# AIS-Bonn/lattice_net

Hardware: AMD Instinct MI355X
Metric: Mpoints/sec splat+conv+slice fwd+bwd on 120k-pt SemanticKITTI scan (higher is better)
Workload: dtype f32 (convolution products bf16x3-emulated)

## Files before the change

include/latticenet_hip.h:

```cpp
#ifndef LATTICENET_HIP_H
#define LATTICENET_HIP_H

#include <stddef.h>

#ifdef __cplusplus
extern "C" {
#endif

#define LN_OK 0
#define LN_ERR_ARG (-1)
#define LN_ERR_UNSUPPORTED (-2)
#define LN_ERR_LAUNCH (-3)
#define LN_ERR_WORKSPACE (-4)

#define LN_STATUS_TABLE_FULL 1
#define LN_STATUS_KEY_RANGE 2
#define LN_STATUS_BUCKET_OVERFLOW 4
#define LN_STATUS_CLOUD_BAND 8
#define LN_STATUS_CLOUD_STARTS 16

#define LN_MAX_POS_DIM 6
#define LN_SLOT_MAP_INTS 32
#define LN_KEYS_RAW 0
#define LN_KEYS_LATTICE 1
#define LN_NOT_VISITED (-2)

typedef struct LnTable {
    int capacity;
    int pos_dim;
    unsigned long long* slot_keys;
    unsigned int* slot_tok;
    int* slot_cnt;
    int* entries;
    int* keys;
    int* nr_filled;
    int* status;
    int* host_counters;
    int host_seq;
    int key_format;
    int row_limit;
    const int* slot_map;
    int bucket_slots_max;
    int batch_points;
    int batch_key_step;
    int* row_regions;
} LnTable;

#define LN_BATCH_POINT_STARTS (-1)
typedef struct LnTableClouds {
    LnTable table;
    const int* batch_point_starts;
    int batch_clouds;
} LnTableClouds;

#define LN_XCD_GROUPS 8
typedef struct LnCsr {
    int* grp_start;
    int* csr_tok;
    int* seg_desc;
    int* seg_count;
    long long seg_region;
    const int* planes;
    int dense;
} LnCsr;

const char* ln_last_error_string(void);
const char* ln_version(void);
const char* ln_abi_hash(void);

const char* ln_kernel_names(void);
int ln_profile_begin(const char* kernel_names, int max_samples);
int ln_profile_end(double* total_ms, int* launches);
int ln_profile_end_table(char* out, int out_bytes);

int ln_table_clear(const LnTable* t, float* values, long long values_elems, void* stream);

int ln_arena_init(int* arena, long long words, long long minus_begin, long long minus_end, void* stream);

int ln_table_bucket_count(int capacity);

size_t ln_build_workspace_bytes(long long tokens, int capacity);

#define LN_BUILD_WRITE_IDX 1
#define LN_BUILD_CLEAR_FIRST 2
#define LN_BUILD_ATOMIC_PATH 4
#define LN_BUILD_CANONICAL_ROWS 8
#define LN_BUILD_SORTED_CSR 16
#define LN_BUILD_OVERLAPPED 32
int ln_build_splat(const LnTable* t, const float* positions_raw, const float* sigmas_host, int n, int* idx, float* w,
                   int flags, const LnCsr* csr, void* workspace, size_t workspace_bytes, float* clear_values,
                   long long clear_values_elems, void* stream);

int ln_canonicalize(const LnTable* t, int* idx, long long tokens, const LnCsr* csr, void* workspace, size_t workspace_bytes, void* stream);

int ln_rehash(const LnTable* t, void* stream);

int ln_splat_accumulate(float* table_values, const float* vals, const int* idx, const float* w, int n, int pos_dim,
                        int val_dim, void* stream);

long long ln_csr_max_segments(long long tokens, int groups_upper);
size_t ln_csr_workspace_bytes(long long tokens, int groups_upper);
int ln_csr_build(const int* idx, long long tokens, int groups_upper, const LnCsr* csr, void* workspace, size_t workspace_bytes,
                 void* stream);
int ln_csr_reduce_rows(const LnCsr* csr, const int* grp_row, long long max_segments, const float* src, const float* w, int val_dim,
                       int src_div, int src_stride, float* dst, void* stream);
int ln_csr_sort(const LnCsr* csr, int groups_upper, void* workspace, size_t workspace_bytes, long long tokens, void* stream);

int ln_splat_accumulate_and_neighbours(const LnCsr* csr, const int* grp_row, long long max_segments, const float* src, const float* w,
                                       int val_dim, int src_div, int src_stride, float* dst, const LnTable* table, int query_rows_upper,
                                       int* nbr, void* stream);

int ln_csr_segment_max(const LnCsr* csr, const int* grp_row, long long max_segments, const float* src, int channels, int rows,
                       void* packed_ws, float* out_max, int* out_arg, void* stream);
int ln_csr_group_sizes(const LnCsr* csr, const int* grp_row, int groups_upper, int rows, int* counts, void* stream);

int ln_distribute(const LnTable* t, const float* positions_raw, const float* sigmas_host, const float* vals, int n,
                  int val_dim, int* idx, float* w, float* distributed, int flags, const LnCsr* csr, void* workspace,
                  size_t workspace_bytes, float* clear_values, long long clear_values_elems, void* stream);

int ln_coarsen(const LnTable* fine, int fine_rows_upper, const LnTable* coarse, const LnCsr* csr, void* workspace,
               size_t workspace_bytes, void* stream);

int ln_neighbours(const LnTable* query, int query_rows_upper, const LnTable* neigh, int lvl_query, int lvl_neigh,
                  int dilation, int flip, int* nbr, void* stream);

int ln_im2row(const int* nbr, const float* values_neigh, int m, int filter_extent, int val_dim, float* out, void* stream);
int ln_im2rowindices(const int* nbr, int m, int filter_extent, int val_dim, int* out, void* stream);
int ln_row2im(const int* nbr, const float* rowified, int m, int filter_extent, int val_dim, float* out, void* stream);

#define LN_CONV_FLIP_NEIGHBOURS 1
#define LN_CONV_TRANSPOSED_FILTER 2
#define LN_CONV_BANK_READY 4
#define LN_CONV_OVERLAPPED 8
int ln_conv_forward(const int* nbr, const float* values_neigh, const float* filter, int m, int filter_extent, int val_dim,
                    int nr_filters, int flags, float* out, void* stream);
size_t ln_conv_bank_workspace_bytes(int m, int filter_extent, int val_dim, int nr_filters);
size_t ln_conv_forward_workspace_bytes(int m, int filter_extent, int val_dim, int nr_filters);
int ln_conv_forward_ws(const int* nbr, const float* values_neigh, const float* filter, int m, int filter_extent, int val_dim,
                       int nr_filters, int flags, float* out, void* workspace, size_t workspace_bytes, const int* row_partition, void* stream);
size_t ln_conv_grad_filter_workspace_bytes(int m, int filter_extent, int val_dim, int nr_filters);
int ln_conv_grad_filter(const int* nbr, const float* values_neigh, const float* grad_out, int m, int filter_extent,
                        int val_dim, int nr_filters, float* grad_filter, void* workspace, size_t workspace_bytes,
                        void* stream);

int ln_slice_forward(const float* values, const int* idx, const float* w, int n, int pos_dim, int val_dim, float* out,
                     void* stream);
int ln_slice_forward_prepare_backward(const float* values, const int* idx, const float* w, int n, int pos_dim, int val_dim, float* out,
                                      float* grad_accumulator, long long grad_accumulator_elems, void* stream);
int ln_slice_forward_ordered(const LnTable* t, const LnCsr* csr, const float* values, const int* idx, const float* w, int n, int val_dim,
                             float* out, float* grad_accumulator, long long grad_accumulator_elems, void* stream);

int ln_slice_no_precomputation(const LnTable* t, const float* values, const float* positions_raw, const float* sigmas_host,
                               int n, int val_dim, float* out, int* idx, float* w, void* stream);
int ln_slice_backward(const float* grad_sliced, const int* idx, const float* w, int n, int pos_dim, int val_dim,
                      float* grad_values, void* stream);

int ln_gather_forward(const float* values, const int* idx, const float* w, int n, int pos_dim, int val_dim, float* out,
                      void* stream);
int ln_gather_backward(const float* grad_gathered, const int* idx, const float* w, int n, int pos_dim, int val_dim,
                       float* grad_values, void* stream);

int ln_slice_classify_forward(const float* values, const float* delta_w, const float* lin_w, const float* lin_b,
                              const int* idx, const float* w, int n, int pos_dim, int val_dim, int nr_classes,
                              float* logits, void* stream);
size_t ln_slice_classify_backward_workspace_bytes(int n, int pos_dim, int val_dim, int nr_classes);
int ln_slice_classify_backward(const float* grad_logits, const float* values, const float* delta_w, const float* lin_w,
                               const int* idx, const float* w, int n, int pos_dim, int val_dim, int nr_classes,
                               float* g_values, float* g_delta_w, float* g_lin_w, float* g_lin_b, float* grad_sliced,
                               float* w_eff, void* workspace, size_t workspace_bytes, void* stream);

size_t ln_conv_backward_workspace_bytes(int mq, int mn, int filter_extent, int val_dim, int nr_filters);
int ln_conv_backward(const int* nbr_q, const int* nbr_n, const float* values_neigh, const float* grad_out, const float* filter, int mq, int mn,
                     int filter_extent, int val_dim, int nr_filters, float* grad_values, float* grad_filter, void* workspace,
                     size_t workspace_bytes, const int* row_partition, void* stream);
int ln_conv_backward_flags(const int* nbr_q, const int* nbr_n, const float* values_neigh, const float* grad_out, const float* filter, int mq,
                           int mn, int filter_extent, int val_dim, int nr_filters, int flags, float* grad_values, float* grad_filter,
                           void* workspace, size_t workspace_bytes, const int* row_partition, void* stream);

int ln_csr_reduce_rows_f16(const LnCsr* csr, const int* grp_row, long long max_segments, const void* src_f16, const float* w, int val_dim,
                           int src_div, int src_stride, float* dst, void* stream);
int ln_splat_accumulate_and_neighbours_f16(const LnCsr* csr, const int* grp_row, long long max_segments, const void* src_f16, const float* w,
                                           int val_dim, int src_div, int src_stride, float* dst, const LnTable* table, int query_rows_upper,
                                           int* nbr, void* stream);
int ln_slice_forward_f16(const void* values_f16, const int* idx, const float* w, int n, int pos_dim, int val_dim, void* out_f16, void* stream);
int ln_slice_forward_f16_prepare_backward(const void* values_f16, const int* idx, const float* w, int n, int pos_dim, int val_dim, void* out_f16,
                                          float* grad_accumulator, long long grad_accumulator_elems, void* stream);

int ln_conv_forward_f16(const int* nbr, const void* values_neigh, const void* filter, int m, int filter_extent, int val_dim,
                        int nr_filters, int flags, void* out, void* stream);
size_t ln_conv_grad_filter_f16_workspace_bytes(int m, int filter_extent, int val_dim, int nr_filters);
int ln_conv_grad_filter_f16(const int* nbr, const void* values_neigh, const void* grad_out, int m, int filter_extent, int val_dim,
                            int nr_filters, float* grad_filter, void* workspace, size_t workspace_bytes, void* stream);

int ln_linear_act_forward(const float* x, const float* w, const float* b, long long rows, int cin, int cout, float slope, float* y,
                          void* stream);
size_t ln_linear_act_backward_workspace_bytes(int cin, int cout);
int ln_linear_act_backward(const float* x, const float* w, const float* y, const float* grad_y, long long rows, int cin, int cout,
                           float slope, float* grad_x, float* grad_w, float* grad_b, void* workspace, size_t workspace_bytes, void* stream);

size_t ln_group_norm_workspace_bytes(int channels);
int ln_group_norm_forward(const float* x, const float* gamma, const float* beta, int m, int channels, int groups, float eps, int relu,
                          float* y, float* mean_rstd, float* scale_shift, void* workspace, size_t workspace_bytes, void* next_workspace,
                          size_t next_workspace_bytes, void* stream);
int ln_group_norm_backward(const float* x, const float* grad_y, const float* gamma, const float* mean_rstd, const float* scale_shift, int m,
                           int channels, int groups, int relu, float* grad_x, float* grad_gamma, float* grad_beta, void* workspace,
                           size_t workspace_bytes, void* next_workspace, size_t next_workspace_bytes, void* stream);
int ln_group_norm_forward_rows(const float* x, const float* gamma, const float* beta, int m, int channels, int groups, float eps, int relu,
                               float* y, float* mean_rstd, float* scale_shift, void* workspace, size_t workspace_bytes, void* next_workspace,
                               size_t next_workspace_bytes, const int* rows_device, void* stream);
int ln_group_norm_backward_rows(const float* x, const float* grad_y, const float* gamma, const float* mean_rstd, const float* scale_shift, int m,
                                int channels, int groups, int relu, float* grad_x, float* grad_gamma, float* grad_beta, void* workspace,
                                size_t workspace_bytes, void* next_workspace, size_t next_workspace_bytes, const int* rows_device, void* stream);

int ln_cloud_row_starts(const LnTable* t, int rows_upper, int clouds, int* row_starts, int* order_flag, void* stream);
int ln_cloud_row_starts_many(const LnTable* t, int rows_upper, int clouds, int* row_starts, int* order_flag, void* stream);
size_t ln_group_norm_segments_workspace_bytes(int channels, int segments);
int ln_group_norm_forward_segments(const float* x, const float* gamma, const float* beta, int m, int channels, int groups, float eps, int relu,
                                   float* y, float* mean_rstd, float* scale_shift, void* workspace, size_t workspace_bytes, void* next_workspace,
                                   size_t next_workspace_bytes, const int* rows_device, const int* row_starts, int segments, void* stream);
int ln_group_norm_backward_segments(const float* x, const float* grad_y, const float* gamma, const float* mean_rstd, const float* scale_shift,
                                    int m, int channels, int groups, int relu, float* grad_x, float* grad_gamma, float* grad_beta, void* workspace,
                                    size_t workspace_bytes, void* next_workspace, size_t next_workspace_bytes, const int* rows_device,
                                    const int* row_starts, int segments, void* stream);
int ln_group_norm_forward_many_segments(const float* x, const float* gamma, const float* beta, int m, int channels, int groups, float eps,
                                        int relu, float* y, float* mean_rstd, float* scale_shift, void* workspace, size_t workspace_bytes,
                                        void* next_workspace, size_t next_workspace_bytes, const int* rows_device, const int* row_starts,
                                        int segments, void* stream);
int ln_group_norm_backward_many_segments(const float* x, const float* grad_y, const float* gamma, const float* mean_rstd,
                                         const float* scale_shift, int m, int channels, int groups, int relu, float* grad_x, float* grad_gamma,
                                         float* grad_beta, void* workspace, size_t workspace_bytes, void* next_workspace,
                                         size_t next_workspace_bytes, const int* rows_device, const int* row_starts, int segments, void* stream);

int ln_group_norm_forward_segments_f16(const void* x, const float* gamma, const float* beta, int m, int channels, int groups, float eps, int relu,
                                       void* y, float* mean_rstd, float* scale_shift, void* workspace, size_t workspace_bytes,
                                       void* next_workspace, size_t next_workspace_bytes, const int* rows_device, const int* row_starts,
                                       int segments, void* stream);
int ln_group_norm_backward_segments_f16(const void* x, const void* grad_y, const float* gamma, const float* mean_rstd, const float* scale_shift,
                                        int m, int channels, int groups, int relu, void* grad_x, float* grad_gamma, float* grad_beta,
                                        void* workspace, size_t workspace_bytes, void* next_workspace, size_t next_workspace_bytes,
                                        const int* rows_device, const int* row_starts, int segments, void* stream);

size_t ln_batch_norm_workspace_bytes(int channels);
int ln_batch_norm_forward(const float* x, const float* gamma, const float* beta, float* running_mean, float* running_var, int m, int channels,
                          float eps, double momentum, int training, int relu, float* y, float* mean_rstd, float* scale_shift, void* workspace,
                          size_t workspace_bytes, void* next_workspace, size_t next_workspace_bytes, const int* rows_device, void* stream);
int ln_batch_norm_backward(const float* x, const float* grad_y, const float* gamma, const float* mean_rstd, const float* scale_shift, int m,
                           int channels, int training, int relu, float* grad_x, float* grad_gamma, float* grad_beta, void* workspace,
                           size_t workspace_bytes, void* next_workspace, size_t next_workspace_bytes, const int* rows_device, void* stream);

int ln_max_centre_forward(const float* x, const float* gamma, const float* beta, long long n, int k, int c, float* out,
                          float* max_vals, unsigned char* arg_max, void* stream);
size_t ln_max_centre_backward_workspace_bytes(long long n, int k, int c);
int ln_max_centre_backward(const float* grad_out, const float* max_vals, const unsigned char* arg_max, const float* gamma,
                           long long n, int k, int c, float* grad_x, float* grad_gamma_beta, void* workspace,
                           size_t workspace_bytes, void* stream);

size_t ln_linear_backward_workspace_bytes(int rows, int cin, int cout);
int ln_linear_backward(const int* ident, const float* x, const float* grad_y, const float* w, int rows, int cin, int cout, float* grad_x,
                       float* grad_w, void* workspace, size_t workspace_bytes, void* stream);

int ln_weight_norm_forward(const float* v, const float* g, int rows, int cols, int g_dim, float* w, float* norm, void* stream);
int ln_weight_norm_backward(const float* v, const float* g, const float* grad_w, const float* norm, int rows, int cols, int g_dim,
                            float* grad_v, float* grad_g, void* stream);

int ln_distribute_centre(const float* distributed, const int* splat_idx, const float* position_sums, const int* counts, long long tokens,
                         int width, int pos_dim, float* out, void* stream);
int ln_distribute_centre_clouds(const float* distributed, const int* splat_idx, const float* position_sums, const int* counts,
                                long long tokens, int width, int pos_dim, long long tokens_per_cloud, const int* row_starts, int clouds,
                                float* out, void* stream);
int ln_distribute_centre_cloud_starts(const float* distributed, const int* splat_idx, const float* position_sums, const int* counts,
                                      long long tokens, int width, int pos_dim, int tokens_per_point, const int* point_starts,
                                      const int* row_starts, int clouds, float* out, void* stream);
int ln_distribute_centre_many_clouds(const float* distributed, const int* splat_idx, const float* position_sums, const int* counts,
                                     long long tokens, int width, int pos_dim, long long tokens_per_cloud, const int* row_starts, int clouds,
                                     float* out, void* stream);
int ln_distribute_centre_many_cloud_starts(const float* distributed, const int* splat_idx, const float* position_sums, const int* counts,
                                           long long tokens, int width, int pos_dim, int tokens_per_point, const int* point_starts,
                                           const int* row_starts, int clouds, float* out, void* stream);

size_t ln_pointnet_reduce_workspace_bytes(int rows, int channels);
int ln_pointnet_reduce_forward(const LnCsr* csr, const int* grp_row, long long max_segments, const float* src, int channels,
                               const float* bary, int bary_stride, int rows, int min_points, void* workspace, size_t workspace_bytes,
                               float* out, int* out_arg, void* stream);
int ln_pointnet_reduce_forward_clouds(const LnCsr* csr, const int* grp_row, long long max_segments, const float* src, int channels,
                                      const float* bary, int bary_stride, int rows, int min_points, void* workspace, size_t workspace_bytes,
                                      float* out, int* out_arg, const int* row_starts, int clouds, void* stream);
int ln_pointnet_reduce_forward_many_clouds(const LnCsr* csr, const int* grp_row, long long max_segments, const float* src, int channels,
                                           const float* bary, int bary_stride, int rows, int min_points, void* workspace,
                                           size_t workspace_bytes, float* out, int* out_arg, const int* row_starts, int clouds, void* stream);
int ln_pointnet_reduce_backward(const float* grad_out, int grad_stride, const int* out_arg, const int* splat_idx, long long tokens,
                                int channels, float* grad_src, void* stream);

size_t ln_nll_workspace_bytes(void);
int ln_nll_forward(const float* log_probs, const long long* target, long long n, int classes, long long ignore_index, void* workspace,
                   size_t workspace_bytes, float* loss_count, void* stream);
int ln_nll_backward(const long long* target, const float* grad_loss, const float* loss_count, long long n, int classes,
                    long long ignore_index, float* grad_log_probs, void* stream);

size_t ln_lovasz_workspace_bytes(long long n, int classes);
int ln_lovasz_forward(const float* log_probs, const long long* target, long long n, int classes, long long ignore_index, int reduction,
                      void* workspace, size_t workspace_bytes, float* loss, float* per_class, float* dloss_dlogp, void* stream);
int ln_lovasz_backward(const float* dloss_dlogp, const float* grad_loss, long long n, int classes, float* grad_log_probs, void* stream);

size_t ln_lovasz_clouds_workspace_bytes(long long n, long long points_per_cloud, int classes);
int ln_lovasz_forward_clouds(const float* log_probs, const long long* target, long long n, long long points_per_cloud, int classes,
                             long long ignore_index, int reduction, void* workspace, size_t workspace_bytes, float* loss, float* per_cloud,
                             float* per_class, float* dloss_dlogp, void* stream);

size_t ln_iou_counts_clouds_workspace_bytes(long long n, long long points_per_cloud, int classes);
int ln_iou_counts_clouds(const float* scores, const long long* target, long long n, long long points_per_cloud, int classes,
                         long long unlabeled_index, void* workspace, size_t workspace_bytes, long long* intersection, long long* union_,
                         void* stream);

size_t ln_dice_workspace_bytes(long long n, long long points_per_cloud, int classes);
int ln_dice_forward(const float* log_probs, const long long* target, long long n, long long points_per_cloud, int classes,
                    long long ignore_index, void* workspace, size_t workspace_bytes, float* loss, float* per_cloud, float* stats, float* coef,
                    void* stream);
int ln_dice_backward(const float* log_probs, const long long* target, const float* coef, const float* grad_loss, long long n,
                     long long points_per_cloud, int classes, float* grad_log_probs, void* stream);

size_t ln_nll_clouds_workspace_bytes(long long n, long long points_per_cloud);
int ln_nll_forward_clouds(const float* log_probs, const long long* target, long long n, long long points_per_cloud, int classes,
                          long long ignore_index, const float* class_weight, void* workspace, size_t workspace_bytes, float* loss,
                          float* per_cloud, float* weight_sum, void* stream);
int ln_nll_backward_clouds(const long long* target, const float* grad_loss, const float* weight_sum, long long n, long long points_per_cloud,
                           int classes, long long ignore_index, const float* class_weight, float* grad_log_probs, void* stream);

size_t ln_nll_ranges_workspace_bytes(long long n, int clouds, long long longest);
int ln_nll_forward_ranges(const float* log_probs, const long long* target, long long n, const int* point_starts, int clouds, long long longest,
                          int classes, long long ignore_index, const float* class_weight, void* workspace, size_t workspace_bytes, float* loss,
// ... 24 lines not shown
```

lattice_net_amd/_lib.py:

```python
from __future__ import annotations

import ctypes as C
import os

import torch

_PKG = os.path.dirname(os.path.abspath(__file__))
LIB_PATH = os.environ.get("LATTICE_NET_LIB") or os.path.join(_PKG, "liblatticenet_hip.so")

LN_STATUS_TABLE_FULL = 1
LN_STATUS_KEY_RANGE = 2
LN_STATUS_BUCKET_OVERFLOW = 4
LN_STATUS_CLOUD_BAND = 8
LN_STATUS_CLOUD_STARTS = 16
LN_BUILD_WRITE_IDX = 1
LN_BUILD_CLEAR_FIRST = 2
LN_BUILD_ATOMIC_PATH = 4
LN_BUILD_CANONICAL_ROWS = 8
LN_BUILD_SORTED_CSR = 16
LN_BUILD_OVERLAPPED = 32
LN_NOT_VISITED = -2
LN_CONV_FLIP_NEIGHBOURS = 1
LN_CONV_TRANSPOSED_FILTER = 2
LN_CONV_BANK_READY = 4
LN_CONV_OVERLAPPED = 8
LN_MAX_POS_DIM = 6
LN_KEYS_RAW = 0
LN_KEYS_LATTICE = 1
LN_XCD_GROUPS = 8
LN_SLOT_MAP_INTS = 32


class LnTable(C.Structure):

    _fields_ = [
        ("capacity", C.c_int),
        ("pos_dim", C.c_int),
        ("slot_keys", C.c_void_p),
        ("slot_tok", C.c_void_p),
        ("slot_cnt", C.c_void_p),
        ("entries", C.c_void_p),
        ("keys", C.c_void_p),
        ("nr_filled", C.c_void_p),
        ("status", C.c_void_p),
        ("host_counters", C.c_void_p),
        ("host_seq", C.c_int),
        ("key_format", C.c_int),
        ("row_limit", C.c_int),
        ("slot_map", C.c_void_p),
        ("bucket_slots_max", C.c_int),
        ("batch_points", C.c_int),
        ("batch_key_step", C.c_int),
        ("row_regions", C.c_void_p),
    ]


LN_BATCH_POINT_STARTS = -1


class LnTableClouds(C.Structure):

    _fields_ = [
        ("table", LnTable),
        ("batch_point_starts", C.c_void_p),
        ("batch_clouds", C.c_int),
    ]

    def __init__(self, table_fields=(), batch_point_starts=None, batch_clouds=0):
        super().__init__(LnTable(*table_fields), batch_point_starts, batch_clouds)
        self.table.batch_points = LN_BATCH_POINT_STARTS


class LnCsr(C.Structure):

    _fields_ = [
        ("grp_start", C.c_void_p),
        ("csr_tok", C.c_void_p),
        ("seg_desc", C.c_void_p),
        ("seg_count", C.c_void_p),
        ("seg_region", C.c_longlong),
        ("planes", C.c_void_p),
        ("dense", C.c_int),
    ]


class LatticeNetHipError(RuntimeError):
    pass


_vp, _i, _ll, _sz = C.c_void_p, C.c_int, C.c_longlong, C.c_size_t
_T = C.POINTER(LnTable)
_CSR = C.POINTER(LnCsr)

SIGNATURES = {
    "ln_last_error_string": (C.c_char_p, []),
    "ln_version": (C.c_char_p, []),
    "ln_abi_hash": (C.c_char_p, []),
    "ln_kernel_names": (C.c_char_p, []),
    "ln_profile_begin": (_i, [C.c_char_p, _i]),
    "ln_profile_end": (_i, [C.POINTER(C.c_double), C.POINTER(_i)]),
    "ln_profile_end_table": (_i, [C.c_char_p, _i]),
    "ln_table_clear": (_i, [_T, _vp, _ll, _vp]),
    "ln_build_workspace_bytes": (_sz, [_ll, _i]),
    "ln_table_bucket_count": (_i, [_i]),
    "ln_build_splat": (_i, [_T, _vp, _vp, _i, _vp, _vp, _i, _CSR, _vp, _sz, _vp, _ll, _vp]),
    "ln_rehash": (_i, [_T, _vp]),
    "ln_canonicalize": (_i, [_T, _vp, _ll, _CSR, _vp, _sz, _vp]),
    "ln_splat_accumulate": (_i, [_vp, _vp, _vp, _vp, _i, _i, _i, _vp]),
    "ln_csr_workspace_bytes": (_sz, [_ll, _i]),
    "ln_csr_max_segments": (_ll, [_ll, _i]),
    "ln_csr_build": (_i, [_vp, _ll, _i, _CSR, _vp, _sz, _vp]),
    "ln_csr_reduce_rows": (_i, [_CSR, _vp, _ll, _vp, _vp, _i, _i, _i, _vp, _vp]),
    "ln_csr_sort": (_i, [_CSR, _i, _vp, _sz, _ll, _vp]),
    "ln_splat_accumulate_and_neighbours": (_i, [_CSR, _vp, _ll, _vp, _vp, _i, _i, _i, _vp, _T, _i, _vp, _vp]),
    "ln_csr_segment_max": (_i, [_CSR, _vp, _ll, _vp, _i, _i, _vp, _vp, _vp, _vp]),
    "ln_csr_group_sizes": (_i, [_CSR, _vp, _i, _i, _vp, _vp]),
    "ln_distribute": (_i, [_T, _vp, _vp, _vp, _i, _i, _vp, _vp, _vp, _i, _CSR, _vp, _sz, _vp, _ll, _vp]),
    "ln_coarsen": (_i, [_T, _i, _T, _CSR, _vp, _sz, _vp]),
    "ln_neighbours": (_i, [_T, _i, _T, _i, _i, _i, _i, _vp, _vp]),
    "ln_im2row": (_i, [_vp, _vp, _i, _i, _i, _vp, _vp]),
    "ln_im2rowindices": (_i, [_vp, _i, _i, _i, _vp, _vp]),
    "ln_row2im": (_i, [_vp, _vp, _i, _i, _i, _vp, _vp]),
    "ln_conv_forward": (_i, [_vp, _vp, _vp, _i, _i, _i, _i, _i, _vp, _vp]),
    "ln_conv_forward_workspace_bytes": (_sz, [_i, _i, _i, _i]),
    "ln_conv_bank_workspace_bytes": (_sz, [_i, _i, _i, _i]),
    "ln_conv_forward_ws": (_i, [_vp, _vp, _vp, _i, _i, _i, _i, _i, _vp, _vp, _sz, _vp, _vp]),
    "ln_conv_grad_filter_workspace_bytes": (_sz, [_i, _i, _i, _i]),
    "ln_conv_grad_filter": (_i, [_vp, _vp, _vp, _i, _i, _i, _i, _vp, _vp, _sz, _vp]),
    "ln_slice_forward": (_i, [_vp, _vp, _vp, _i, _i, _i, _vp, _vp]),
    "ln_slice_forward_prepare_backward": (_i, [_vp, _vp, _vp, _i, _i, _i, _vp, _vp, _ll, _vp]),
    "ln_slice_forward_ordered": (_i, [_T, _CSR, _vp, _vp, _vp, _i, _i, _vp, _vp, _ll, _vp]),
    "ln_slice_no_precomputation": (_i, [_T, _vp, _vp, _vp, _i, _i, _vp, _vp, _vp, _vp]),
    "ln_slice_backward": (_i, [_vp, _vp, _vp, _i, _i, _i, _vp, _vp]),
    "ln_gather_forward": (_i, [_vp, _vp, _vp, _i, _i, _i, _vp, _vp]),
    "ln_gather_backward": (_i, [_vp, _vp, _vp, _i, _i, _i, _vp, _vp]),
    "ln_slice_classify_forward": (_i, [_vp, _vp, _vp, _vp, _vp, _vp, _i, _i, _i, _i, _vp, _vp]),
    "ln_csr_reduce_rows_f16": (_i, [_CSR, _vp, _ll, _vp, _vp, _i, _i, _i, _vp, _vp]),
    "ln_splat_accumulate_and_neighbours_f16": (_i, [_CSR, _vp, _ll, _vp, _vp, _i, _i, _i, _vp, _T, _i, _vp, _vp]),
    "ln_slice_forward_f16": (_i, [_vp, _vp, _vp, _i, _i, _i, _vp, _vp]),
    "ln_slice_forward_f16_prepare_backward": (_i, [_vp, _vp, _vp, _i, _i, _i, _vp, _vp, _ll, _vp]),
    "ln_conv_backward_workspace_bytes": (_sz, [_i, _i, _i, _i, _i]),
    "ln_conv_backward": (_i, [_vp, _vp, _vp, _vp, _vp, _i, _i, _i, _i, _i, _vp, _vp, _vp, _sz, _vp, _vp]),
    "ln_conv_backward_flags": (_i, [_vp, _vp, _vp, _vp, _vp, _i, _i, _i, _i, _i, _i, _vp, _vp, _vp, _sz, _vp, _vp]),
    "ln_conv_forward_f16": (_i, [_vp, _vp, _vp, _i, _i, _i, _i, _i, _vp, _vp]),
    "ln_conv_grad_filter_f16_workspace_bytes": (_sz, [_i, _i, _i, _i]),
    "ln_conv_grad_filter_f16": (_i, [_vp, _vp, _vp, _i, _i, _i, _i, _vp, _vp, _sz, _vp]),
    "ln_linear_act_forward": (_i, [_vp, _vp, _vp, _ll, _i, _i, C.c_float, _vp, _vp]),
    "ln_linear_act_backward_workspace_bytes": (_sz, [_i, _i]),
    "ln_linear_act_backward": (_i, [_vp, _vp, _vp, _vp, _ll, _i, _i, C.c_float, _vp, _vp, _vp, _vp, _sz, _vp]),
    "ln_arena_init": (_i, [_vp, _ll, _ll, _ll, _vp]),
    "ln_weight_norm_forward": (_i, [_vp, _vp, _i, _i, _i, _vp, _vp, _vp]),
    "ln_weight_norm_backward": (_i, [_vp, _vp, _vp, _vp, _i, _i, _i, _vp, _vp, _vp]),
    "ln_distribute_centre": (_i, [_vp, _vp, _vp, _vp, _ll, _i, _i, _vp, _vp]),
    "ln_distribute_centre_clouds": (_i, [_vp, _vp, _vp, _vp, _ll, _i, _i, _ll, _vp, _i, _vp, _vp]),
    "ln_distribute_centre_many_clouds": (_i, [_vp, _vp, _vp, _vp, _ll, _i, _i, _ll, _vp, _i, _vp, _vp]),
    "ln_distribute_centre_cloud_starts": (_i, [_vp, _vp, _vp, _vp, _ll, _i, _i, _i, _vp, _vp, _i, _vp, _vp]),
    "ln_distribute_centre_many_cloud_starts": (_i, [_vp, _vp, _vp, _vp, _ll, _i, _i, _i, _vp, _vp, _i, _vp, _vp]),
    "ln_pointnet_reduce_workspace_bytes": (_sz, [_i, _i]),
    "ln_pointnet_reduce_forward": (_i, [_CSR, _vp, _ll, _vp, _i, _vp, _i, _i, _i, _vp, _sz, _vp, _vp, _vp]),
    "ln_pointnet_reduce_forward_clouds": (_i, [_CSR, _vp, _ll, _vp, _i, _vp, _i, _i, _i, _vp, _sz, _vp, _vp, _vp, _i, _vp]),
    "ln_pointnet_reduce_forward_many_clouds": (_i, [_CSR, _vp, _ll, _vp, _i, _vp, _i, _i, _i, _vp, _sz, _vp, _vp, _vp, _i, _vp]),
    "ln_pointnet_reduce_backward": (_i, [_vp, _i, _vp, _vp, _ll, _i, _vp, _vp]),
    "ln_linear_backward_workspace_bytes": (_sz, [_i, _i, _i]),
    "ln_linear_backward": (_i, [_vp, _vp, _vp, _vp, _i, _i, _i, _vp, _vp, _vp, _sz, _vp]),
    "ln_nll_workspace_bytes": (_sz, []),
    "ln_nll_forward": (_i, [_vp, _vp, _ll, _i, _ll, _vp, _sz, _vp, _vp]),
    "ln_nll_backward": (_i, [_vp, _vp, _vp, _ll, _i, _ll, _vp, _vp]),
    "ln_nll_clouds_workspace_bytes": (_sz, [_ll, _ll]),
    "ln_nll_forward_clouds": (_i, [_vp, _vp, _ll, _ll, _i, _ll, _vp, _vp, _sz, _vp, _vp, _vp, _vp]),
    "ln_nll_backward_clouds": (_i, [_vp, _vp, _vp, _ll, _ll, _i, _ll, _vp, _vp, _vp]),
    "ln_lovasz_workspace_bytes": (_sz, [_ll, _i]),
    "ln_lovasz_forward": (_i, [_vp, _vp, _ll, _i, _ll, _i, _vp, _sz, _vp, _vp, _vp, _vp]),
    "ln_lovasz_backward": (_i, [_vp, _vp, _ll, _i, _vp, _vp]),
    "ln_lovasz_clouds_workspace_bytes": (_sz, [_ll, _ll, _i]),
    "ln_lovasz_forward_clouds": (_i, [_vp, _vp, _ll, _ll, _i, _ll, _i, _vp, _sz, _vp, _vp, _vp, _vp, _vp]),
    "ln_iou_counts_clouds_workspace_bytes": (_sz, [_ll, _ll, _i]),
    "ln_iou_counts_clouds": (_i, [_vp, _vp, _ll, _ll, _i, _ll, _vp, _sz, _vp, _vp, _vp]),
    "ln_dice_workspace_bytes": (_sz, [_ll, _ll, _i]),
    "ln_dice_forward": (_i, [_vp, _vp, _ll, _ll, _i, _ll, _vp, _sz, _vp, _vp, _vp, _vp, _vp]),
    "ln_dice_backward": (_i, [_vp, _vp, _vp, _vp, _ll, _ll, _i, _vp, _vp]),
    "ln_nll_ranges_workspace_bytes": (_sz, [_ll, _i, _ll]),
    "ln_nll_forward_ranges": (_i, [_vp, _vp, _ll, _vp, _i, _ll, _i, _ll, _vp, _vp, _sz, _vp, _vp, _vp, _vp]),
    "ln_nll_backward_ranges": (_i, [_vp, _vp, _vp, _ll, _vp, _i, _ll, _i, _ll, _vp, _vp, _vp]),
    "ln_dice_ranges_workspace_bytes": (_sz, [_ll, _i, _ll, _i]),
    "ln_dice_forward_ranges": (_i, [_vp, _vp, _ll, _vp, _i, _ll, _i, _ll, _vp, _sz, _vp, _vp, _vp, _vp, _vp]),
    "ln_dice_backward_ranges": (_i, [_vp, _vp, _vp, _vp, _ll, _vp, _i, _ll, _i, _vp, _vp]),
    "ln_lovasz_ranges_workspace_bytes": (_sz, [_ll, _i, _ll, _i]),
    "ln_lovasz_forward_ranges": (_i, [_vp, _vp, _ll, _vp, _i, _ll, _i, _ll, _i, _vp, _sz, _vp, _vp, _vp, _vp, _vp]),
    "ln_max_centre_forward": (_i, [_vp, _vp, _vp, _ll, _i, _i, _vp, _vp, _vp, _vp]),
    "ln_max_centre_backward_workspace_bytes": (_sz, [_ll, _i, _i]),
    "ln_max_centre_backward": (_i, [_vp, _vp, _vp, _vp, _ll, _i, _i, _vp, _vp, _vp, _sz, _vp]),
    "ln_group_norm_workspace_bytes": (_sz, [_i]),
    "ln_group_norm_forward": (_i, [_vp, _vp, _vp, _i, _i, _i, C.c_float, _i, _vp, _vp, _vp, _vp, _sz, _vp, _sz, _vp]),
    "ln_group_norm_backward": (_i, [_vp, _vp, _vp, _vp, _vp, _i, _i, _i, _i, _vp, _vp, _vp, _vp, _sz, _vp, _sz, _vp]),
    "ln_group_norm_forward_rows": (_i, [_vp, _vp, _vp, _i, _i, _i, C.c_float, _i, _vp, _vp, _vp, _vp, _sz, _vp, _sz, _vp, _vp]),
    "ln_group_norm_backward_rows": (_i, [_vp, _vp, _vp, _vp, _vp, _i, _i, _i, _i, _vp, _vp, _vp, _vp, _sz, _vp, _sz, _vp, _vp]),
    "ln_cloud_row_starts": (_i, [_T, _i, _i, _vp, _vp, _vp]),
    "ln_cloud_row_starts_many": (_i, [_T, _i, _i, _vp, _vp, _vp]),
    "ln_group_norm_segments_workspace_bytes": (_sz, [_i, _i]),
    "ln_group_norm_forward_segments": (_i, [_vp, _vp, _vp, _i, _i, _i, C.c_float, _i, _vp, _vp, _vp, _vp, _sz, _vp, _sz, _vp, _vp, _i, _vp]),
    "ln_group_norm_forward_many_segments": (_i, [_vp, _vp, _vp, _i, _i, _i, C.c_float, _i, _vp, _vp, _vp, _vp, _sz, _vp, _sz, _vp, _vp, _i, _vp]),
    "ln_group_norm_backward_segments": (_i, [_vp, _vp, _vp, _vp, _vp, _i, _i, _i, _i, _vp, _vp, _vp, _vp, _sz, _vp, _sz, _vp, _vp, _i, _vp]),
    "ln_group_norm_backward_many_segments": (_i, [_vp, _vp, _vp, _vp, _vp, _i, _i, _i, _i, _vp, _vp, _vp, _vp, _sz, _vp, _sz, _vp, _vp, _i, _vp]),
    "ln_group_norm_forward_segments_f16": (_i, [_vp, _vp, _vp, _i, _i, _i, C.c_float, _i, _vp, _vp, _vp, _vp, _sz, _vp, _sz, _vp, _vp, _i, _vp]),
    "ln_group_norm_backward_segments_f16": (_i, [_vp, _vp, _vp, _vp, _vp, _i, _i, _i, _i, _vp, _vp, _vp, _vp, _sz, _vp, _sz, _vp, _vp, _i, _vp]),
    "ln_batch_norm_workspace_bytes": (_sz, [_i]),
    "ln_batch_norm_forward": (_i, [_vp, _vp, _vp, _vp, _vp, _i, _i, C.c_float, C.c_double, _i, _i, _vp, _vp, _vp, _vp, _sz, _vp, _sz, _vp, _vp]),
    "ln_batch_norm_backward": (_i, [_vp, _vp, _vp, _vp, _vp, _i, _i, _i, _i, _vp, _vp, _vp, _vp, _sz, _vp, _sz, _vp, _vp]),
    "ln_cloud_key_extents": (_i, [_T, _vp, _vp, _i, _i, _vp, _vp, _vp]),
    "ln_cloud_point_starts_check": (_i, [_vp, _i, _i, _vp, _vp]),
    "ln_slice_classify_backward_workspace_bytes": (_sz, [_i, _i, _i, _i]),
    "ln_slice_classify_backward": (_i, [_vp, _vp, _vp, _vp, _vp, _vp, _i, _i, _i, _i, _vp, _vp, _vp, _vp, _vp, _vp, _vp, _sz, _vp]),
}

_lib = None


def load():
    global _lib
    if _lib is not None:
        return _lib
    if not os.path.exists(LIB_PATH):
        raise LatticeNetHipError(
            f"{LIB_PATH} is missing: the HIP extension is not built. Run `python -c 'import __graft_entry__ as g; g.build()'` "
            "(or `python lattice_net_amd/build_ext.py`). There is no CPU fallback."
        )
    lib = C.CDLL(LIB_PATH)
    for name, (res, args) in SIGNATURES.items():
        fn = getattr(lib, name)
        fn.restype = res
        fn.argtypes = args
    from . import build_ext
    try:
        want = build_ext.abi_hash()
    except OSError:
        want = None
    have = lib.ln_abi_hash().decode()
    if want is not None and have != want:
        raise LatticeNetHipError(f"{LIB_PATH} was built from a different include/latticenet_hip.h (library {have}, header {want}): "
                                 "rebuild it with `python lattice_net_amd/build_ext.py`")
    _lib = lib
    return lib


def check(rc: int, what: str = ""):
    if rc != 0:
        msg = load().ln_last_error_string().decode("utf-8", "replace")
        raise LatticeNetHipError(f"{what or 'latticenet_hip'} failed (code {rc}): {msg}")


def ptr(t):
    return None if t is None else t.data_ptr()


def stream_ptr(device) -> int:
    cur = torch.cuda.current_device()
    idx = device.index if device.index is not None else cur
    if idx != cur:
        raise LatticeNetHipError(f"lattice tensors live on cuda:{idx} but the current device is cuda:{cur}; wrap the call in "
                                 f"`with torch.cuda.device({idx}):` (or torch.cuda.set_device) — one process drives one GPU")
    return torch._C._cuda_getCurrentRawStream(idx)


def host_floats(values):
    arr = (C.c_float * len(values))(*[float(v) for v in values])
    return arr
```

lattice_net_amd/csrc/ln_conv.hip:

```cpp
#include "ln_common.h"
#include <stdlib.h>

#include "ln_bf16x3.h"

#include "ln_conv_plan.h"
#include <type_traits>

#ifdef LN_STAMPS
__device__ unsigned long long* g_ln_stamps_conv = nullptr;
extern "C" int ln_debug_set_stamps_conv(void* buffer) {
    unsigned long long* p = static_cast<unsigned long long*>(buffer);
    return hipMemcpyToSymbol(HIP_SYMBOL(g_ln_stamps_conv), &p, sizeof(p)) == hipSuccess ? 0 : -1;
}
#define LN_CSTAMP(slot)                                                                                                  \
    do {                                                                                                                 \
        if (g_ln_stamps_conv && threadIdx.x == 0) g_ln_stamps_conv[(size_t)blockIdx.x * 8 + (slot)] = wall_clock64(); \
    } while (0)
#else
#define LN_CSTAMP(slot) do { } while (0)
#endif

template <int KQ>
__device__ __forceinline__ void ln_load_quarter(const float* __restrict__ src, float* a) {
    if constexpr (KQ % 4 == 0) {
// ... 811 lines not shown
                }
            }
        }
    }
}

template <int V, int NT, int E, bool FLIP, bool WT>
__global__ void __launch_bounds__(256)
    k_conv_mfma_full(const int* __restrict__ nbr, const float* __restrict__ values, const float* __restrict__ filter, int m,
                     float* __restrict__ out, int conv_blocks, const float* __restrict__ slab_partial, int nslabs, int slab_total,
                     float* __restrict__ slab_out) {
    if (slab_out != nullptr && (int)blockIdx.x >= conv_blocks) {
        ln_sum_slabs_body<false>(blockIdx.x - conv_blocks, slab_partial, nslabs, slab_total, slab_total, slab_out);
        return;
    }
    constexpr int F = 16 * NT;
    constexpr int KQ = V / 4;
    static_assert(E * V * F * 4 <= 64 * 1024, "filter bank must fit 64 KiB of LDS");
    __shared__ __attribute__((aligned(16))) float s_b[E * V * F];
    const int tid = threadIdx.x;
    const int lane = tid & 63;
    const int wave = tid >> 6;
    const int i = lane & 15;
    const int q = lane >> 4;
    const int m0 = blockIdx.x * 64 + wave * 16;
    const int my_row = m0 + i;

    LN_CSTAMP(0);
    constexpr int N4 = E * V * F / 4;
    constexpr int NST = (N4 + 255) / 256;
    float4 wv[NST];
#pragma unroll
    for (int s = 0; s < NST; ++s) {
        const int x4 = tid + s * 256;
        wv[s] = (x4 < N4) ? reinterpret_cast<const float4*>(filter)[x4] : make_float4(0.f, 0.f, 0.f, 0.f);
    }
    int nb[E];
#pragma unroll
    for (int e = 0; e < E; ++e) nb[e] = (my_row < m) ? nbr[(size_t)my_row * E + ((FLIP && e < E - 1) ? (e ^ 1) : e)] : -1;
    float a[E][KQ];
#pragma unroll
    for (int e = 0; e < E; ++e) ln_load_quarter<KQ>(values + (size_t)(nb[e] >= 0 ? nb[e] : 0) * V + q * KQ, a[e]);
#pragma unroll
    for (int s = 0; s < NST; ++s) {
        const int x4 = tid + s * 256;
        if (x4 < N4) {
            const int x = x4 * 4;
            if constexpr (!WT) {
                const int ek = x / F;
                const int f = x - ek * F;
                const int e = ek / V;
                const int k = ek - e * V;
                const int qq = k / KQ;
                const int kk = k - qq * KQ;
                float* dst = s_b + (((e * KQ + kk) * NT + (f >> 4)) * 64 + qq * 16 + (f & 15));
                *reinterpret_cast<float4*>(dst) = wv[s];
            } else {
                const int ef = x / V;
                const int k0 = x - ef * V;
                const int e = ef / F;
                const int f = ef - e * F;
                const float vals4[4] = {wv[s].x, wv[s].y, wv[s].z, wv[s].w};
#pragma unroll
                for (int j = 0; j < 4; ++j) {
                    const int k = k0 + j;
                    const int qq = k / KQ;
                    const int kk = k - qq * KQ;
                    s_b[((e * KQ + kk) * NT + (f >> 4)) * 64 + qq * 16 + (f & 15)] = vals4[j];
                }
            }
        }
    }
    __syncthreads();
    LN_CSTAMP(1);
    floatx4 acc[NT];
#pragma unroll
    for (int nt = 0; nt < NT; ++nt) acc[nt] = floatx4{0.f, 0.f, 0.f, 0.f};
#pragma unroll
    for (int e = 0; e < E; ++e) {
#pragma unroll
        for (int kk = 0; kk < KQ; ++kk) {
            const float av = nb[e] >= 0 ? a[e][kk] : 0.f;
#pragma unroll
            for (int nt = 0; nt < NT; ++nt) {
                const float b = s_b[((e * KQ + kk) * NT + nt) * 64 + lane];
                acc[nt] = __builtin_amdgcn_mfma_f32_16x16x4f32(av, b, acc[nt], 0, 0, 0);
            }
        }
    }
    LN_CSTAMP(2);
#pragma unroll
    for (int nt = 0; nt < NT; ++nt) {
#pragma unroll
        for (int r = 0; r < 4; ++r) {
            const int row = m0 + q * 4 + r;
            if (row < m) out[(size_t)row * F + nt * 16 + i] = acc[nt][r];
        }
    }
    LN_CSTAMP(3);
}

__global__ void __launch_bounds__(256)
    k_conv_generic(const int* __restrict__ nbr, const float* __restrict__ values, const float* __restrict__ filter, long long work,
                   int E, int V, int F, int flip, int wt, float* __restrict__ out) {
    const long long g = (long long)blockIdx.x * blockDim.x + threadIdx.x;
    if (g >= work) return;
    const long long mrow = g / F;
    const int f = int(g - mrow * F);
    float acc = 0.0f;
    for (int e = 0; e < E; ++e) {
        const int nb = nbr[mrow * E + ((flip && e < E - 1) ? (e ^ 1) : e)];
        if (nb < 0) continue;
        const float* vr = values + (size_t)nb * V;
        if (wt) {
            const float* wr = filter + ((size_t)e * F + f) * V;
            for (int v = 0; v < V; ++v) acc = fmaf(vr[v], wr[v], acc);
        } else {
            const float* wr = filter + (size_t)e * V * F + f;
            for (int v = 0; v < V; ++v) acc = fmaf(vr[v], wr[(size_t)v * F], acc);
        }
    }
    out[g] = acc;
}

__global__ void __launch_bounds__(256) ln_k_sum_partials(const float* __restrict__ partial, int nslabs, long long total4, float* __restrict__ out) {
    const long long i = (long long)blockIdx.x * 256 + threadIdx.x;
    if (i >= total4) return;
    float4 acc = reinterpret_cast<const float4*>(partial)[i];
    for (int sl = 1; sl < nslabs; ++sl) {
        const float4 v = reinterpret_cast<const float4*>(partial)[(long long)sl * total4 + i];
        acc.x += v.x; acc.y += v.y; acc.z += v.z; acc.w += v.w;
    }
    reinterpret_cast<float4*>(out)[i] = acc;
}

static bool ln_conv_b3_enabled() {
    static int v = -1;
    if (v < 0) {
        const char* e = getenv("LN_CONV_EXACT_F32");
        v = (e && e[0] == '1') ? 0 : 1;
    }
    return v == 1;
}
static bool ln_aligned16(const void* p) { return (reinterpret_cast<uintptr_t>(p) & 15) == 0; }

extern "C" size_t ln_conv_bank_workspace_bytes(int m, int filter_extent, int val_dim, int nr_filters) {
    return ln_conv_bank_query(m, filter_extent, val_dim, nr_filters, ln_conv_b3_enabled());
}

extern "C" size_t ln_conv_forward_workspace_bytes(int m, int filter_extent, int val_dim, int nr_filters) {
    return ln_conv_forward_query(m, filter_extent, val_dim, nr_filters, ln_conv_b3_enabled());
}

template <int T>
__global__ void __launch_bounds__(256 * T) __attribute__((amdgpu_waves_per_eu(T, T)))
    k_conv_forward_b3(const int* __restrict__ nbr, const float* __restrict__ values, const float* __restrict__ filter, int m,
                      float* __restrict__ out, const int* __restrict__ row_part) {
    constexpr int V = 32, F = 32, E = 9, KQ = 8, NT = 2;
    constexpr int THREADS = 256 * T;
    constexpr int FRAG16 = E * NT * 3 * 64;
    __shared__ __attribute__((aligned(16))) unsigned char s_raw[FRAG16 * 16];
    const u32x4* s_frag = reinterpret_cast<const u32x4*>(s_raw);
    __shared__ __attribute__((aligned(16))) floatx4 s_x[4 * T][16 * 8];
    __shared__ int s_nbr[64 * T * E];
    const int tid = threadIdx.x;
    const int lane = tid & 63;
    const int i = lane & 15;
    const int q = lane >> 4;
    const int bx = ln_partition_tile(blockIdx.x, gridDim.x, row_part, 64 * T);
    const int m0 = bx * (64 * T) + (tid >> 6) * 16;
    const int my_row = m0 + i;
    constexpr int ITEMS = E * (V / 8) * F;
    constexpr int NIT = (ITEMS + THREADS - 1) / THREADS;
    float wv[NIT][8];
#pragma unroll
    for (int s = 0; s < NIT; ++s) {
        const int x = min(tid + s * THREADS, ITEMS - 1);
        const int f = x % F;
        const int ev8 = x / F;
#pragma unroll
        for (int j = 0; j < 8; ++j) wv[s][j] = filter[(ev8 * 8 + j) * F + f];
    }
    {
        const size_t g0 = (size_t)bx * (64 * T) * E, g_end = (size_t)m * E;
        for (int x = tid; x < 64 * T * E; x += THREADS) s_nbr[x] = (g0 + x < g_end) ? nbr[g0 + x] : -1;
    }
    {
        bool any = false;
        for (int x = tid; x < 64 * T * E; x += THREADS) any |= s_nbr[x] >= 0;
        if (!__syncthreads_or(any)) {
            for (int x = tid; x < 64 * T * (F / 4); x += THREADS) {
                const int row = bx * (64 * T) + x / (F / 4);
                if (row < m) *reinterpret_cast<float4*>(out + (size_t)row * F + (x % (F / 4)) * 4) = make_float4(0.f, 0.f, 0.f, 0.f);
            }
            return;
        }
    }
    const int wv_ = tid >> 6;
    const int lr = lane >> 3;
    int nb[2][E];
#pragma unroll
    for (int j = 0; j < 2; ++j)
#pragma unroll
        for (int e = 0; e < E; ++e) nb[j][e] = s_nbr[(wv_ * 16 + 8 * j + lr) * E + e];
    auto fsw = [](int r) -> int { return ((r >> 1) & 7) ^ (((r >> 2) & 1) << 1); };
    floatx4* xw[2];
#pragma unroll
    for (int j = 0; j < 2; ++j) xw[j] = &s_x[wv_][(8 * j + lr) * 8 + ((lane & 7) ^ fsw(8 * j + lr))];
    const floatx4* xr0 = &s_x[wv_][i * 8 + ((2 * q) ^ fsw(i))];
    const floatx4* xr1 = &s_x[wv_][i * 8 + ((2 * q + 1) ^ fsw(i))];
#ifndef LN_FWD_DEPTH
#define LN_FWD_DEPTH 4
#endif
    constexpr int DEPTH = LN_FWD_DEPTH;
    floatx4 a[DEPTH][2];
    auto gather = [&](int e, floatx4 (&dst)[2]) {
#pragma unroll
        for (int j = 0; j < 2; ++j)
            dst[j] = *reinterpret_cast<const floatx4*>(values + (size_t)(nb[j][e] >= 0 ? nb[j][e] : 0) * V + (lane & 7) * 4);
    };
#pragma unroll
    for (int k = 0; k < DEPTH - 1 && k < E; ++k) gather(k, a[k]);
    u32x4* s_frag_w = reinterpret_cast<u32x4*>(s_raw);
#pragma unroll
    for (int s = 0; s < NIT; ++s) {
        const int x = tid + s * THREADS;
        if (x < ITEMS) {
            const int f = x % F;
            const int ev8 = x / F;
            const int e = ev8 / (V / 8);
            const int vo = ev8 - e * (V / 8);
            unsigned int h[8], md[8], lo[8];
#pragma unroll
            for (int j = 0; j < 8; ++j) ln_split3_bits(wv[s][j], h[j], md[j], lo[j]);
            const int unit = ((e * NT + (f >> 4)) * 3) * 64 + vo * 16 + (f & 15);
            s_frag_w[unit] = u32x4{ln_pack_hi(h[0], h[1]), ln_pack_hi(h[2], h[3]), ln_pack_hi(h[4], h[5]), ln_pack_hi(h[6], h[7])};
            s_frag_w[unit + 64] = u32x4{ln_pack_hi(md[0], md[1]), ln_pack_hi(md[2], md[3]), ln_pack_hi(md[4], md[5]), ln_pack_hi(md[6], md[7])};
            s_frag_w[unit + 128] = u32x4{ln_pack_hi(lo[0], lo[1]), ln_pack_hi(lo[2], lo[3]), ln_pack_hi(lo[4], lo[5]), ln_pack_hi(lo[6], lo[7])};
        }
    }
    floatx4 acc[NT];
#pragma unroll
    for (int nt = 0; nt < NT; ++nt) acc[nt] = floatx4{0.f, 0.f, 0.f, 0.f};
    __syncthreads();
#pragma unroll
    for (int e = 0; e < E; ++e) {
        if (e + DEPTH - 1 < E) gather(e + DEPTH - 1, a[(e + DEPTH - 1) % DEPTH]);
#pragma unroll
        for (int j = 0; j < 2; ++j) *xw[j] = (nb[j][e] >= 0) ? a[e % DEPTH][j] : floatx4{0.f, 0.f, 0.f, 0.f};
        __builtin_amdgcn_fence(__ATOMIC_RELEASE, "wavefront");
        __builtin_amdgcn_wave_barrier();
        __builtin_amdgcn_fence(__ATOMIC_ACQUIRE, "wavefront");
        const floatx4 lo4 = *xr0, hi4 = *xr1;
        __builtin_amdgcn_fence(__ATOMIC_RELEASE, "wavefront");
        __builtin_amdgcn_wave_barrier();
        __builtin_amdgcn_fence(__ATOMIC_ACQUIRE, "wavefront");
        const float ae[KQ] = {lo4[0], lo4[1], lo4[2], lo4[3], hi4[0], hi4[1], hi4[2], hi4[3]};
        u32x4 p[3];
        ln_split3_pack8(ae, 0, p);
        const bf16x8 ap[3] = {__builtin_bit_cast(bf16x8, p[0]), __builtin_bit_cast(bf16x8, p[1]), __builtin_bit_cast(bf16x8, p[2])};
#pragma unroll
        for (int nt = 0; nt < NT; ++nt) {
            const u32x4* pb = s_frag + ((e * NT + nt) * 3) * 64 + lane;
            const bf16x8 bp[3] = {__builtin_bit_cast(bf16x8, pb[0]), __builtin_bit_cast(bf16x8, pb[64]), __builtin_bit_cast(bf16x8, pb[128])};
            ln_b3_mfma16(ap, bp, acc[nt]);
        }
    }
#pragma unroll
    for (int nt = 0; nt < NT; ++nt)
#pragma unroll
        for (int r = 0; r < 4; ++r) {
            const int row = m0 + q * 4 + r;
            if (row < m) out[(size_t)row * F + nt * 16 + i] = acc[nt][r];
        }
}

template <int T, int C>
__global__ void __launch_bounds__(256 * T) __attribute__((amdgpu_waves_per_eu(T, T)))
    k_conv_forward_b3_rows(const int* __restrict__ nbr, const float* __restrict__ values, const float* __restrict__ filter, int m,
                      float* __restrict__ out, const int* __restrict__ row_part) {
    constexpr int V = 32, F = 32, E = 9, KQ = 8, NT = 2;
    constexpr int THREADS = 256 * T;
    constexpr int FRAG16 = E * NT * 3 * 64;
    __shared__ __attribute__((aligned(16))) unsigned char s_raw[FRAG16 * 16];
    const u32x4* s_frag = reinterpret_cast<const u32x4*>(s_raw);
    __shared__ __attribute__((aligned(16))) floatx4 s_x[4 * T][16 * 8];
    __shared__ int s_nbr[64 * T * E];
    const int tid = threadIdx.x;
    const int lane = tid & 63;
    const int i = lane & 15;
    const int q = lane >> 4;
    const int bx0 = ln_partition_tile(blockIdx.x, gridDim.x, row_part, 64 * T * C) * C;
    const int m00 = bx0 * (64 * T) + (tid >> 6) * 16;
    constexpr int ITEMS = E * (V / 8) * F;
    constexpr int NIT = (ITEMS + THREADS - 1) / THREADS;
    float wv[NIT][8];
#pragma unroll
    for (int s = 0; s < NIT; ++s) {
        const int x = min(tid + s * THREADS, ITEMS - 1);
        const int f = x % F;
        const int ev8 = x / F;
#pragma unroll
        for (int j = 0; j < 8; ++j) wv[s][j] = filter[(ev8 * 8 + j) * F + f];
    }
    bool staged = false;
#pragma unroll
    for (int c = 0; c < C; ++c) {
    const int bx = bx0 + c;
    const int m0 = m00 + c * (64 * T);
    {
        const size_t g0 = (size_t)bx * (64 * T) * E, g_end = (size_t)m * E;
        for (int x = tid; x < 64 * T * E; x += THREADS) s_nbr[x] = (g0 + x < g_end) ? nbr[g0 + x] : -1;
    }
    {
        bool any = false;
        for (int x = tid; x < 64 * T * E; x += THREADS) any |= s_nbr[x] >= 0;
        if (!__syncthreads_or(any)) {
            for (int x = tid; x < 64 * T * (F / 4); x += THREADS) {
                const int row = bx * (64 * T) + x / (F / 4);
                if (row < m) *reinterpret_cast<float4*>(out + (size_t)row * F + (x % (F / 4)) * 4) = make_float4(0.f, 0.f, 0.f, 0.f);
            }
            if constexpr (C == 1) return;
            else continue;
        }
    }
    const int wv_ = tid >> 6;
    const int lr = lane >> 3;
    int nb[2][E];
#pragma unroll
    for (int j = 0; j < 2; ++j)
#pragma unroll
        for (int e = 0; e < E; ++e) nb[j][e] = s_nbr[(wv_ * 16 + 8 * j + lr) * E + e];
    auto fsw = [](int r) -> int { return ((r >> 1) & 7) ^ (((r >> 2) & 1) << 1); };
    floatx4* xw[2];
#pragma unroll
    for (int j = 0; j < 2; ++j) xw[j] = &s_x[wv_][(8 * j + lr) * 8 + ((lane & 7) ^ fsw(8 * j + lr))];
    const floatx4* xr0 = &s_x[wv_][i * 8 + ((2 * q) ^ fsw(i))];
    const floatx4* xr1 = &s_x[wv_][i * 8 + ((2 * q + 1) ^ fsw(i))];
#ifndef LN_FWD_DEPTH
#define LN_FWD_DEPTH 4
#endif
    constexpr int DEPTH = LN_FWD_DEPTH;
    floatx4 a[DEPTH][2];
    auto gather = [&](int e, floatx4 (&dst)[2]) {
#pragma unroll
        for (int j = 0; j < 2; ++j)
            dst[j] = *reinterpret_cast<const floatx4*>(values + (size_t)(nb[j][e] >= 0 ? nb[j][e] : 0) * V + (lane & 7) * 4);
    };
#pragma unroll
    for (int k = 0; k < DEPTH - 1 && k < E; ++k) gather(k, a[k]);
    u32x4* s_frag_w = reinterpret_cast<u32x4*>(s_raw);
    if (!staged) {
    staged = true;
#pragma unroll
    for (int s = 0; s < NIT; ++s) {
        const int x = tid + s * THREADS;
        if (x < ITEMS) {
            const int f = x % F;
            const int ev8 = x / F;
            const int e = ev8 / (V / 8);
            const int vo = ev8 - e * (V / 8);
            unsigned int h[8], md[8], lo[8];
#pragma unroll
            for (int j = 0; j < 8; ++j) ln_split3_bits(wv[s][j], h[j], md[j], lo[j]);
            const int unit = ((e * NT + (f >> 4)) * 3) * 64 + vo * 16 + (f & 15);
            s_frag_w[unit] = u32x4{ln_pack_hi(h[0], h[1]), ln_pack_hi(h[2], h[3]), ln_pack_hi(h[4], h[5]), ln_pack_hi(h[6], h[7])};
            s_frag_w[unit + 64] = u32x4{ln_pack_hi(md[0], md[1]), ln_pack_hi(md[2], md[3]), ln_pack_hi(md[4], md[5]), ln_pack_hi(md[6], md[7])};
            s_frag_w[unit + 128] = u32x4{ln_pack_hi(lo[0], lo[1]), ln_pack_hi(lo[2], lo[3]), ln_pack_hi(lo[4], lo[5]), ln_pack_hi(lo[6], lo[7])};
        }
    }
    }
    floatx4 acc[NT];
#pragma unroll
    for (int nt = 0; nt < NT; ++nt) acc[nt] = floatx4{0.f, 0.f, 0.f, 0.f};
    __syncthreads();
#pragma unroll
    for (int e = 0; e < E; ++e) {
        if (e + DEPTH - 1 < E) gather(e + DEPTH - 1, a[(e + DEPTH - 1) % DEPTH]);
#pragma unroll
        for (int j = 0; j < 2; ++j) *xw[j] = (nb[j][e] >= 0) ? a[e % DEPTH][j] : floatx4{0.f, 0.f, 0.f, 0.f};
        __builtin_amdgcn_fence(__ATOMIC_RELEASE, "wavefront");
        __builtin_amdgcn_wave_barrier();
        __builtin_amdgcn_fence(__ATOMIC_ACQUIRE, "wavefront");
        const floatx4 lo4 = *xr0, hi4 = *xr1;
        __builtin_amdgcn_fence(__ATOMIC_RELEASE, "wavefront");
        __builtin_amdgcn_wave_barrier();
        __builtin_amdgcn_fence(__ATOMIC_ACQUIRE, "wavefront");
        const float ae[KQ] = {lo4[0], lo4[1], lo4[2], lo4[3], hi4[0], hi4[1], hi4[2], hi4[3]};
        u32x4 p[3];
        ln_split3_pack8(ae, 0, p);
        const bf16x8 ap[3] = {__builtin_bit_cast(bf16x8, p[0]), __builtin_bit_cast(bf16x8, p[1]), __builtin_bit_cast(bf16x8, p[2])};
#pragma unroll
        for (int nt = 0; nt < NT; ++nt) {
            const u32x4* pb = s_frag + ((e * NT + nt) * 3) * 64 + lane;
            const bf16x8 bp[3] = {__builtin_bit_cast(bf16x8, pb[0]), __builtin_bit_cast(bf16x8, pb[64]), __builtin_bit_cast(bf16x8, pb[128])};
            ln_b3_mfma16(ap, bp, acc[nt]);
        }
    }
#pragma unroll
    for (int nt = 0; nt < NT; ++nt)
#pragma unroll
        for (int r = 0; r < 4; ++r) {
            const int row = m0 + q * 4 + r;
            if (row < m) out[(size_t)row * F + nt * 16 + i] = acc[nt][r];
        }
    }
}

template <bool FLIP, bool WT>
struct LnConvCall {
    const int* nbr;
    const float *values, *filter;
    int m, E, V, F;
    float* out;
    unsigned short* bank;
    float* dst;
    int e_per;
    LnSlabSum sum;
    const int* row_partition;
    hipStream_t st;
};

template <bool FLIP, bool WT>
static void ln_conv_launch_full(int V, int NT, dim3 grid, hipStream_t st, const int* nbr, const float* values, const float* filter, int m,
                                float* out, int conv_blocks, const float* partial, int chunks, int total, float* grad_filter) {
    auto go = [&](auto v, auto nt) {
        constexpr int VV = decltype(v)::value, NN = decltype(nt)::value;
        static_assert(ln_conv_full_shape(VV, 16 * NN), "not a small-filter shape");
        LN_LAUNCH("k_conv_mfma", (k_conv_mfma_full<VV, NN, 9, FLIP, WT>), grid, dim3(256), 0, st, nbr, values, filter, m, out, conv_blocks, partial,
                  chunks, total, grad_filter);
    };
    using std::integral_constant;
    switch (V * 16 + NT) {
        case 32 * 16 + 2: go(integral_constant<int, 32>{}, integral_constant<int, 2>{}); break;
        case 32 * 16 + 1: go(integral_constant<int, 32>{}, integral_constant<int, 1>{}); break;
        case 16 * 16 + 1: go(integral_constant<int, 16>{}, integral_constant<int, 1>{}); break;
        case 16 * 16 + 2: go(integral_constant<int, 16>{}, integral_constant<int, 2>{}); break;
        case 16 * 16 + 4: go(integral_constant<int, 16>{}, integral_constant<int, 4>{}); break;
        case 8 * 16 + 1: go(integral_constant<int, 8>{}, integral_constant<int, 1>{}); break;
        case 8 * 16 + 2: go(integral_constant<int, 8>{}, integral_constant<int, 2>{}); break;
        case 8 * 16 + 4: go(integral_constant<int, 8>{}, integral_constant<int, 4>{}); break;
        case 8 * 16 + 8: go(integral_constant<int, 8>{}, integral_constant<int, 8>{}); break;
        default: break;
    }
}

template <bool FLIP, bool WT>
struct LnConvEntry {
    const LnConvLaunch& l;
    const LnConvCall<FLIP, WT>& c;
    dim3 grid() const { return dim3(l.grid[0], l.grid[1], l.grid[2]); }
    unsigned short* bank() const { return c.bank + l.bank_off; }
    const u32x4* frags() const { return reinterpret_cast<const u32x4*>(bank()); }
    LnSlabSum ride() const { return l.carries_sum ? c.sum : LnSlabSum{nullptr, 0, 0, nullptr}; }
};
template <int V, int NT, bool FLIP, bool WT>
static void ln_conv_run_wide(const LnConvEntry<FLIP, WT>& e) {
    const LnConvLaunch& l = e.l;
    const LnConvCall<FLIP, WT>& c = e.c;
    if constexpr (ln_conv_wide_built(V, NT)) {
        if (l.kernel == LN_K_SPLIT_BANK32) {
            LN_LAUNCH("k_conv_split_bank", (k_conv_split_bank32<V, NT, WT>), e.grid(), dim3(l.block), 0, c.st, c.filter, c.F, l.f_off, e.bank(), l.split_x,
                      e.ride());
            return;
        }
        if constexpr (NT == 3) {
            if (l.kernel == LN_K_ROWS32SK) {
                LN_LAUNCH("k_conv_mfma", (k_conv_rows32sk_b3<V, NT, LN_CONV_R32SK_RT, FLIP>), e.grid(), dim3(l.block), 0, c.st, c.nbr, c.values, e.frags(),
                          c.m, c.E, c.dst, c.F, l.f_off, c.e_per);
                return;
            }
        }
        LN_LAUNCH("k_conv_mfma", (k_conv_rows32_b3<V, ln_conv_r32_ntw(NT), ln_conv_r32_ch(NT), ln_conv_r32_rt(NT), FLIP>), e.grid(), dim3(l.block), 0, c.st,
                  c.nbr, c.values, e.frags(), c.m, c.E, c.dst, c.F, l.f_off, c.e_per);
    }
}
template <int V, int NT, bool FLIP, bool WT>
static void ln_conv_run_chunk(const LnConvEntry<FLIP, WT>& e) {
    const LnConvLaunch& l = e.l;
    const LnConvCall<FLIP, WT>& c = e.c;
    if constexpr (ln_conv_chunk_fits(V, NT)) {
        if constexpr (ln_conv_chunk_b3(V, NT)) {
            if (l.kernel == LN_K_SPLIT_BANK) {
                LN_LAUNCH("k_conv_split_bank", (k_conv_split_bank<V, NT, WT>), e.grid(), dim3(l.block), 0, c.st, c.filter, c.F, l.f_off, e.bank(), l.split_x,
                          e.ride());
                return;
            }
            if (l.kernel == LN_K_MFMA_B3) {
                if (l.t == 3) {
                    if constexpr (ln_conv_b3_three_subtiles(V))
                        LN_LAUNCH("k_conv_mfma", (k_conv_mfma_b3<V, NT, FLIP, 3>), e.grid(), dim3(l.block), 0, c.st, c.nbr, c.values, e.frags(), c.m, c.E,
                                  c.dst, c.F, l.f_off, c.e_per);
                } else {
                    LN_LAUNCH("k_conv_mfma", (k_conv_mfma_b3<V, NT, FLIP, 1>), e.grid(), dim3(l.block), 0, c.st, c.nbr, c.values, e.frags(), c.m, c.E, c.dst,
                              c.F, l.f_off, c.e_per);
                }
                return;
            }
        }
        LN_LAUNCH("k_conv_mfma", (k_conv_mfma<V, NT, FLIP, WT>), e.grid(), dim3(l.block), 0, c.st, c.nbr, c.values, c.filter, c.m, c.E, c.dst, c.F, l.f_off,
                  c.e_per);
    }
}

template <int V, bool FLIP, bool WT>
static void ln_conv_run_v(const LnConvLaunch& l, const LnConvCall<FLIP, WT>& c) {
    const LnConvEntry<FLIP, WT> e = {l, c};
    if (l.kernel == LN_K_SPLIT_BANK32 || l.kernel == LN_K_ROWS32 || l.kernel == LN_K_ROWS32SK) {
        switch (l.nt) {
            case 4: ln_conv_run_wide<V, 4>(e); break;
            case 3: ln_conv_run_wide<V, 3>(e); break;
            case 2: ln_conv_run_wide<V, 2>(e); break;
            case 1: ln_conv_run_wide<V, 1>(e); break;
            default: break;
        }
    } else {
        switch (l.nt) {
            case 8: ln_conv_run_chunk<V, 8>(e); break;
            case 4: ln_conv_run_chunk<V, 4>(e); break;
            case 2: ln_conv_run_chunk<V, 2>(e); break;
            case 1: ln_conv_run_chunk<V, 1>(e); break;
            default: break;
        }
    }
}

template <bool FLIP, bool WT>
static void ln_conv_run(const LnConvPlan& p, const LnConvCall<FLIP, WT>& c) {
    for (int k = 0; k < p.n; ++k) {
        const LnConvLaunch& l = p.launch[k];
        const dim3 grid(l.grid[0], l.grid[1], l.grid[2]), block(l.block);
        switch (l.kernel) {
            case LN_K_FORWARD_B3:
                if constexpr (!FLIP && !WT) {
                    if (l.c > 1)
                        LN_LAUNCH("k_conv_mfma", (k_conv_forward_b3_rows<LN_CONV_OVL_T, LN_CONV_OVL_C>), grid, block, 0, c.st, c.nbr, c.values, c.filter, c.m, c.out,
                                  c.row_partition);
                    else if (l.t == 1) LN_LAUNCH("k_conv_mfma", (k_conv_forward_b3<1>), grid, block, 0, c.st, c.nbr, c.values, c.filter, c.m, c.out, c.row_partition);
                    else if (l.t == 2) LN_LAUNCH("k_conv_mfma", (k_conv_forward_b3<2>), grid, block, 0, c.st, c.nbr, c.values, c.filter, c.m, c.out, c.row_partition);
                    else LN_LAUNCH("k_conv_mfma", (k_conv_forward_b3<3>), grid, block, 0, c.st, c.nbr, c.values, c.filter, c.m, c.out, c.row_partition);
                }
                break;
            case LN_K_FULL:
                ln_conv_launch_full<FLIP, WT>(c.V, l.nt, grid, c.st, c.nbr, c.values, c.filter, c.m, c.out, l.grid[0], nullptr, 0, 0, nullptr);
                break;
            case LN_K_SUM_PARTIALS:
                LN_LAUNCH("k_conv_sum_partials", ln_k_sum_partials, grid, block, 0, c.st, (const float*)c.dst, p.nsplit, (long long)c.m * c.F / 4, c.out);
                break;
            case LN_K_GENERIC:
                LN_LAUNCH("k_conv_generic", k_conv_generic, grid, block, 0, c.st, c.nbr, c.values, c.filter, (long long)c.m * c.F, c.E, c.V, c.F,
                          FLIP ? 1 : 0, WT ? 1 : 0, c.out);
                break;
            default:
                switch (c.V) {
                    case 8: ln_conv_run_v<8>(l, c); break;
                    case 16: ln_conv_run_v<16>(l, c); break;
                    case 32: ln_conv_run_v<32>(l, c); break;
                    case 48: ln_conv_run_v<48>(l, c); break;
                    case 64: ln_conv_run_v<64>(l, c); break;
                    case 96: ln_conv_run_v<96>(l, c); break;
                    case 128: ln_conv_run_v<128>(l, c); break;
                    case 192: ln_conv_run_v<192>(l, c); break;
                    case 256: ln_conv_run_v<256>(l, c); break;
                    default: break;
                }
        }
    }
}

template <bool FLIP, bool WT>
static void ln_conv_plan_and_run(LnConvPlanIn in, const int* nbr, const float* values, const float* filter, float* out, void* ws,
                                 const LnSlabSum& sum, bool* sum_left, const int* row_partition, hipStream_t st) {
    in.flip = FLIP;
    in.wt = WT;
    const LnConvPlan p = ln_conv_plan(in);
    char* slabs = static_cast<char*>(ws) + p.bank_bytes;
    ln_conv_run<FLIP, WT>(p, LnConvCall<FLIP, WT>{nbr, values, filter, in.m, in.E, in.V, in.F, out, static_cast<unsigned short*>(ws),
                                                 p.nsplit > 1 ? reinterpret_cast<float*>(slabs) : out, p.e_per, sum, row_partition, st});
    *sum_left = p.sum_left;
}

static int ln_conv_forward_riding(const int* nbr, const float* values_neigh, const float* filter, int m, int filter_extent, int val_dim,
                                  int nr_filters, int flags, float* out, void* workspace, size_t workspace_bytes, const int* row_partition,
                                  void* stream, const LnSlabSum& sum) {
    hipStream_t st = (hipStream_t)stream;
    bool sum_left = sum.partial != nullptr;
    const int rc = [&]() -> int {
        LN_REQUIRE(m >= 0 && filter_extent >= 1 && val_dim >= 1 && nr_filters >= 1, LN_ERR_ARG, "ln_conv_forward: bad sizes");
        LN_REQUIRE(m == 0 || (nbr && values_neigh && filter && out), LN_ERR_ARG, "ln_conv_forward: null buffer");
        LN_REQUIRE((flags & ~15) == 0, LN_ERR_ARG, "ln_conv_forward: unknown flags %d", flags);
        if (m == 0) return LN_OK;
        LnConvPlanIn in = {};
        in.m = m, in.E = filter_extent, in.V = val_dim, in.F = nr_filters;
        in.b3_enabled = ln_conv_b3_enabled();
        in.values_aligned = ln_aligned16(values_neigh);
        in.filter_aligned = ln_aligned16(filter);
        in.ws_aligned = workspace && (reinterpret_cast<uintptr_t>(workspace) & 255) == 0;
        in.ws_bytes = workspace_bytes;
        in.bank_ready = (flags & LN_CONV_BANK_READY) != 0 && workspace != nullptr;
        in.riding_total = sum.partial ? sum.total : 0;
        in.overlapped = (flags & LN_CONV_OVERLAPPED) != 0;
        switch (flags & 3) {
            case 0: ln_conv_plan_and_run<false, false>(in, nbr, values_neigh, filter, out, workspace, sum, &sum_left, row_partition, st); break;
            case LN_CONV_FLIP_NEIGHBOURS: ln_conv_plan_and_run<true, false>(in, nbr, values_neigh, filter, out, workspace, sum, &sum_left, row_partition, st); break;
            case LN_CONV_TRANSPOSED_FILTER: ln_conv_plan_and_run<false, true>(in, nbr, values_neigh, filter, out, workspace, sum, &sum_left, row_partition, st); break;
            default: ln_conv_plan_and_run<true, true>(in, nbr, values_neigh, filter, out, workspace, sum, &sum_left, row_partition, st); break;
        }
        return ln_check_launch("ln_conv_forward");
    }();
    if (sum_left) (void)ln_reduce_slabs_async(sum.partial, sum.nslabs, sum.total, sum.out, st);
    return rc;
}

extern "C" int ln_conv_forward_ws(const int* nbr, const float* values_neigh, const float* filter, int m, int filter_extent, int val_dim,
                                  int nr_filters, int flags, float* out, void* workspace, size_t workspace_bytes, const int* row_partition,
                                  void* stream) {
    return ln_conv_forward_riding(nbr, values_neigh, filter, m, filter_extent, val_dim, nr_filters, flags, out, workspace, workspace_bytes,
                                  row_partition, stream, LnSlabSum{nullptr, 0, 0, nullptr});
}

extern "C" int ln_conv_forward(const int* nbr, const float* values_neigh, const float* filter, int m, int filter_extent,
                               int val_dim, int nr_filters, int flags, float* out, void* stream) {
    return ln_conv_forward_ws(nbr, values_neigh, filter, m, filter_extent, val_dim, nr_filters, flags, out, nullptr, 0, nullptr, stream);
}

#define LN_GF_SUB 64

template <int VT, int FT>
__global__ void __launch_bounds__(256)
    k_grad_filter_mfma(const int* __restrict__ nbr, const float* __restrict__ values, const float* __restrict__ grad_out, int m,
                       int E, float* __restrict__ partial, int v_total, int v_off, int f_total, int f_off) {
    if (gridDim.z > 1) {
        const int col_tiles = f_total / (16 * FT);
        v_off = (blockIdx.z / col_tiles) * 16 * VT;
        f_off = (blockIdx.z % col_tiles) * 16 * FT;
    }
    constexpr int V = VT * 16;
    constexpr int F = FT * 16;
    constexpr int SA = V + 16;
    constexpr int SG = F + 16;
    constexpr int TILES = VT * FT;
    constexpr int TPW = (TILES + 3) / 4;
    constexpr int A4 = LN_GF_SUB * V / 4 / 256;
    constexpr int G4 = LN_GF_SUB * F / 4 / 256;
    static_assert(A4 >= 1 && G4 >= 1, "tile too small for 256 staging threads");
    __shared__ __attribute__((aligned(16))) float s_a[LN_GF_SUB * SA];
    __shared__ __attribute__((aligned(16))) float s_g[LN_GF_SUB * SG];
    const int tid = threadIdx.x;
    const int lane = tid & 63;
    const int wave = tid >> 6;
    const int i = lane & 15;
    const int q = lane >> 4;
    const int e = blockIdx.y;
    const int chunk_begin = blockIdx.x * LN_GF_ROWS;
    const int chunk_end = min(chunk_begin + LN_GF_ROWS, m);

    floatx4 acc[TPW][2];
#pragma unroll
    for (int t = 0; t < TPW; ++t) {
        acc[t][0] = floatx4{0.f, 0.f, 0.f, 0.f};
        acc[t][1] = floatx4{0.f, 0.f, 0.f, 0.f};
    }
    float4 ra[A4], rg[G4];
    auto issue_loads = [&](int sub_begin) {
#pragma unroll
        for (int s = 0; s < A4; ++s) {
            const int x4 = tid + s * 256;
            const int r = x4 / (V / 4);
            const int c = x4 - r * (V / 4);
            const int row = sub_begin + r;
            const int nb = (row < chunk_end) ? nbr[(size_t)row * E + e] : -1;
            ra[s] = *reinterpret_cast<const float4*>(values + (size_t)(nb >= 0 ? nb : 0) * v_total + v_off + c * 4);
            if (nb < 0) ra[s] = make_float4(0.f, 0.f, 0.f, 0.f);
        }
#pragma unroll
        for (int s = 0; s < G4; ++s) {
            const int x4 = tid + s * 256;
            const int r = x4 / (F / 4);
            const int c = x4 - r * (F / 4);
            const int row = sub_begin + r;
            rg[s] = (row < chunk_end) ? *reinterpret_cast<const float4*>(grad_out + (size_t)row * f_total + f_off + c * 4)
                                      : make_float4(0.f, 0.f, 0.f, 0.f);
        }
    };
    if (chunk_begin < chunk_end) issue_loads(chunk_begin);
    for (int sub = chunk_begin; sub < chunk_end; sub += LN_GF_SUB) {
        __syncthreads();
#pragma unroll
        for (int s = 0; s < A4; ++s) {
            const int x4 = tid + s * 256;
            const int r = x4 / (V / 4);
            const int c = x4 - r * (V / 4);
            *reinterpret_cast<float4*>(s_a + r * SA + c * 4) = ra[s];
        }
#pragma unroll
        for (int s = 0; s < G4; ++s) {
            const int x4 = tid + s * 256;
            const int r = x4 / (F / 4);
            const int c = x4 - r * (F / 4);
            *reinterpret_cast<float4*>(s_g + r * SG + c * 4) = rg[s];
        }
        __syncthreads();
        if (sub + LN_GF_SUB < chunk_end) issue_loads(sub + LN_GF_SUB);
#pragma unroll
        for (int t = 0; t < TPW; ++t) {
            const int tile = wave + 4 * t;
            if (tile < TILES) {
                const int vt = tile / FT;
                const int ft = tile - vt * FT;
                const float* pa = s_a + q * SA + vt * 16 + i;
                const float* pg = s_g + q * SG + ft * 16 + i;
#pragma unroll 8
                for (int k = 0; k < LN_GF_SUB / 4; k += 2) {
                    acc[t][0] = __builtin_amdgcn_mfma_f32_16x16x4f32(pa[(k * 4) * SA], pg[(k * 4) * SG], acc[t][0], 0, 0, 0);
                    acc[t][1] = __builtin_amdgcn_mfma_f32_16x16x4f32(pa[(k * 4 + 4) * SA], pg[(k * 4 + 4) * SG], acc[t][1], 0, 0, 0);
                }
            }
        }
    }
    float* dst = partial + ((size_t)blockIdx.x * E + e) * ((size_t)v_total * f_total) + (size_t)v_off * f_total + f_off;
#pragma unroll
    for (int t = 0; t < TPW; ++t) {
        const int tile = wave + 4 * t;
        if (tile < TILES) {
            const int vt = tile / FT;
            const int ft = tile - vt * FT;
#pragma unroll
            for (int r = 0; r < 4; ++r) dst[(size_t)(vt * 16 + q * 4 + r) * f_total + ft * 16 + i] = acc[t][0][r] + acc[t][1][r];
        }
    }
}

__global__ void __launch_bounds__(256)
    k_grad_filter_generic(const int* __restrict__ nbr, const float* __restrict__ values, const float* __restrict__ grad_out, int m,
                          int E, int V, int F, float* __restrict__ grad_filter) {
    const int g = blockIdx.x * blockDim.x + threadIdx.x;
    if (g >= E * V * F) return;
    const int f = g % F;
    const int ev = g / F;
    const int v = ev % V;
    const int e = ev / V;
    float acc = 0.0f;
    for (int row = 0; row < m; ++row) {
        const int nb = nbr[(size_t)row * E + e];
        if (nb >= 0) acc = fmaf(values[(size_t)nb * V + v], grad_out[(size_t)row * F + f], acc);
    }
    grad_filter[g] = acc;
}

__global__ void __launch_bounds__(256) k_reduce_slabs4(const float* __restrict__ partial, int nslabs, int total, float* __restrict__ out) {
    ln_reduce_slabs4_block(blockIdx.x, partial, nslabs, total, out);
}

int ln_reduce_slabs_async(const float* partial, int nslabs, int total, float* out, hipStream_t st) {
    if (total % 64 == 0 && ((reinterpret_cast<uintptr_t>(out) | reinterpret_cast<uintptr_t>(partial)) & 15) == 0)
        LN_LAUNCH("k_reduce_slabs", k_reduce_slabs4, dim3(total / 64), dim3(256), 0, st, partial, nslabs, total, out);
    else
        LN_LAUNCH("k_reduce_slabs", ln_k_sum_slabs<false>, dim3(ln_div_up(total, 16)), dim3(256), 0, st, partial, nslabs, (long long)total, total, out);
    return LN_OK;
}

typedef short gf_short4 __attribute__((ext_vector_type(4)));
#ifndef LN_GFB_WAVES
#define LN_GFB_WAVES 2
#endif
template <int VT, int FT, int E, int WV, int WF>
__global__ void __launch_bounds__(64 * WV * WF, (WV * WF) > 8 ? 1 : LN_GFB_WAVES)
    k_grad_filter_b3(const int* __restrict__ nbr, const float* __restrict__ values, const float* __restrict__ grad_out, int m, int rows_per_wg,
                     float* __restrict__ partial, int v_total, int f_total) {
    constexpr int V = VT * 16, F = FT * 16;
    constexpr int EG = LN_GFB_EG;
// ... 217 lines not shown
extern "C" int ln_conv_grad_filter(const int* nbr, const float* values_neigh, const float* grad_out, int m, int filter_extent,
                                   int val_dim, int nr_filters, float* grad_filter, void* workspace, size_t workspace_bytes,
                                   void* stream) {
    return ln_conv_grad_filter_impl(nbr, values_neigh, grad_out, m, filter_extent, val_dim, nr_filters, grad_filter, workspace, workspace_bytes,
                                    stream, nullptr);
}

template <int V, int F, int E, int T>
__global__ void __launch_bounds__(256 * T) __attribute__((amdgpu_waves_per_eu(T, T)))
    k_conv_backward_fused(const int* __restrict__ nbr, const float* __restrict__ values, const float* __restrict__ grad_out,
                          const float* __restrict__ filter, int m, float* __restrict__ grad_values, float* __restrict__ slabs) {
    constexpr int KQ = F / 4;
    constexpr int NT = V / 16;
    constexpr int VT = V / 16, FT = F / 16;
    static_assert(VT * FT == 4, "one filter-gradient tile per wave of a sub-tile");
    static_assert(E * V * F * 4 <= 64 * 1024, "filter bank must fit 64 KiB of LDS");
    constexpr int SG = F + 16;
    constexpr int THREADS = 256 * T;
    constexpr int BANK = E * V * F;
    constexpr int STAGE = 2 * 64 * SG;
    constexpr int LDS_FLOATS = (BANK + T * STAGE) > (T - 1) * BANK ? (BANK + T * STAGE) : (T - 1) * BANK;
    __shared__ __attribute__((aligned(16))) float s_all[LDS_FLOATS];
    float* s_b = s_all;
    const int tid = threadIdx.x;
    const int sub = tid >> 8;
    const int t256 = tid & 255;
    const int lane = tid & 63;
    const int wave = t256 >> 6;
    const int i = lane & 15;
    const int q = lane >> 4;
    const int sub0 = blockIdx.x * (64 * T) + sub * 64;
    const int m0 = sub0 + wave * 16;
    const int my_row = m0 + i;

    LN_CSTAMP(0);
    constexpr int N4 = E * V * F / 4;
    constexpr int NST = (N4 + THREADS - 1) / THREADS;
    float4 wv[NST];
#pragma unroll
    for (int s = 0; s < NST; ++s) {
        const int x4 = tid + s * THREADS;
        wv[s] = (x4 < N4) ? reinterpret_cast<const float4*>(filter)[x4] : make_float4(0.f, 0.f, 0.f, 0.f);
    }
    int nb[E];
#pragma unroll
    for (int e = 0; e < E; ++e) nb[e] = (my_row < m) ? nbr[(size_t)my_row * E + (e < E - 1 ? (e ^ 1) : e)] : -1;
    const int vt = wave / FT, ft = wave % FT;
    float vT[16];
#pragma unroll
    for (int st = 0; st < 16; ++st) {
        const int row = sub0 + 4 * st + q;
        vT[st] = (row < m) ? values[(size_t)row * V + vt * 16 + i] : 0.f;
    }
    constexpr int DEPTH = 3;
    auto slot_of = [](int k) { return k == 0 ? E - 1 : k - 1; };
    float a[DEPTH + 1][KQ];
    ln_load_quarter<KQ>(grad_out + (size_t)(my_row < m ? my_row : 0) * F + q * KQ, a[0]);
#pragma unroll
    for (int k = 1; k < DEPTH && k < E; ++k)
        ln_load_quarter<KQ>(grad_out + (size_t)(nb[slot_of(k)] >= 0 ? nb[slot_of(k)] : 0) * F + q * KQ, a[k % (DEPTH + 1)]);
#pragma unroll
    for (int s = 0; s < NST; ++s) {
        const int x4 = tid + s * THREADS;
        if (x4 < N4) {
            const int x = x4 * 4;
            const int ev = x / F;
            const int k0 = x - ev * F;
            const int e = ev / V;
            const int v = ev - e * V;
            const float vals4[4] = {wv[s].x, wv[s].y, wv[s].z, wv[s].w};
#pragma unroll
            for (int j = 0; j < 4; ++j) {
                const int k = k0 + j;
                const int qq = k / KQ;
                const int kk = k - qq * KQ;
                s_b[((e * KQ + kk) * NT + (v >> 4)) * 64 + qq * 16 + (v & 15)] = vals4[j];
            }
        }
    }
    floatx4 acc_v[NT];
#pragma unroll
    for (int nt = 0; nt < NT; ++nt) acc_v[nt] = floatx4{0.f, 0.f, 0.f, 0.f};
    floatx4 acc_w[E];
#pragma unroll
    for (int e = 0; e < E; ++e) acc_w[e] = floatx4{0.f, 0.f, 0.f, 0.f};
#pragma unroll
    for (int k = 0; k < E; ++k) {
        const int e = slot_of(k);
        float* sg = s_all + BANK + sub * STAGE + (k & 1) * (64 * SG);
        float (&ae)[KQ] = a[k % (DEPTH + 1)];
        if (k + DEPTH < E)
            ln_load_quarter<KQ>(grad_out + (size_t)(nb[slot_of(k + DEPTH)] >= 0 ? nb[slot_of(k + DEPTH)] : 0) * F + q * KQ, a[(k + DEPTH) % (DEPTH + 1)]);
        {
            float* dst = sg + (wave * 16 + i) * SG + q * KQ;
#pragma unroll
            for (int c = 0; c < KQ; c += 4)
                *reinterpret_cast<float4*>(dst + c) = nb[e] >= 0 ? make_float4(ae[c], ae[c + 1], ae[c + 2], ae[c + 3]) : make_float4(0.f, 0.f, 0.f, 0.f);
        }
        __syncthreads();
        if (k == 0) LN_CSTAMP(1);
        if (k == 1) LN_CSTAMP(4);
        if (k == 8) LN_CSTAMP(5);
#pragma unroll
        for (int kk = 0; kk < KQ; ++kk) {
            const float av = nb[e] >= 0 ? ae[kk] : 0.f;
#pragma unroll
            for (int nt = 0; nt < NT; ++nt)
                acc_v[nt] = __builtin_amdgcn_mfma_f32_16x16x4f32(av, s_b[((e * KQ + kk) * NT + nt) * 64 + lane], acc_v[nt], 0, 0, 0);
        }
        const float* pg = sg + q * SG + ft * 16 + i;
        floatx4 w0 = floatx4{0.f, 0.f, 0.f, 0.f}, w1 = floatx4{0.f, 0.f, 0.f, 0.f};
#pragma unroll
        for (int st = 0; st < 16; st += 2) {
            w0 = __builtin_amdgcn_mfma_f32_16x16x4f32(vT[st], pg[(4 * st) * SG], w0, 0, 0, 0);
            w1 = __builtin_amdgcn_mfma_f32_16x16x4f32(vT[st + 1], pg[(4 * st + 4) * SG], w1, 0, 0, 0);
        }
        acc_w[e] = w0 + w1;
    }
    LN_CSTAMP(2);
#pragma unroll
    for (int nt = 0; nt < NT; ++nt) {
#pragma unroll
        for (int r = 0; r < 4; ++r) {
            const int row = m0 + q * 4 + r;
            if (row < m) grad_values[(size_t)row * V + nt * 16 + i] = acc_v[nt][r];
        }
    }
    __syncthreads();
    if (sub > 0) {
        float* park = s_all + (size_t)(sub - 1) * BANK;
#pragma unroll
        for (int e = 0; e < E; ++e)
#pragma unroll
            for (int r = 0; r < 4; ++r) park[(e * V + vt * 16 + q * 4 + r) * F + ft * 16 + i] = acc_w[e][r];
    }
    if constexpr (T > 1) __syncthreads();
    if (sub == 0) {
        float* dst = slabs + (size_t)blockIdx.x * BANK;
#pragma unroll
        for (int e = 0; e < E; ++e)
#pragma unroll
            for (int r = 0; r < 4; ++r) {
                const int o = (e * V + vt * 16 + q * 4 + r) * F + ft * 16 + i;
                float sum = acc_w[e][r];
#pragma unroll
                for (int k = 1; k < T; ++k) sum += s_all[(size_t)(k - 1) * BANK + o];
                dst[o] = sum;
            }
    }
    LN_CSTAMP(3);
}

typedef short short4v __attribute__((ext_vector_type(4)));
template <int T>
__global__ void __launch_bounds__(256 * T) __attribute__((amdgpu_waves_per_eu(T, T)))
    k_conv_backward_fused_b3(const int* __restrict__ nbr, const float* __restrict__ values, const float* __restrict__ grad_out,
                             const float* __restrict__ filter, int m, float* __restrict__ grad_values, float* __restrict__ slabs,
                             const int* __restrict__ row_part) {
    constexpr int V = 32, F = 32, E = 9, KQ = 8, NT = 2, FT = 2;
    constexpr int THREADS = 256 * T;
    constexpr int BANK = E * V * F;
    constexpr int FRAG16 = E * NT * 3 * 64;
    constexpr int RS = 32;
    auto swz = [](int r) { return (0x78 >> (2 * ((r >> 2) & 3))) & 3; };
    constexpr int PART = 64 * RS;
    constexpr int STAGE = 2 * 3 * PART;
    constexpr int LDS_BYTES_A = FRAG16 * 16 + T * STAGE * 2;
    constexpr int LDS_BYTES_B = (T - 1) * BANK * 4;
    constexpr int LDS_BYTES = LDS_BYTES_A > LDS_BYTES_B ? LDS_BYTES_A : LDS_BYTES_B;
    __shared__ __attribute__((aligned(16))) unsigned char s_raw[LDS_BYTES];
    u32x4* s_frag = reinterpret_cast<u32x4*>(s_raw);
    unsigned short* s_fh = reinterpret_cast<unsigned short*>(s_raw);
    unsigned short* s_stage = reinterpret_cast<unsigned short*>(s_raw + FRAG16 * 16);
    const int tid = threadIdx.x;
    const int sub = tid >> 8;
    const int t256 = tid & 255;
    const int lane = tid & 63;
    const int wave = t256 >> 6;
    const int i = lane & 15;
    const int q = lane >> 4;
    const int bx = ln_partition_tile(blockIdx.x, gridDim.x, row_part, 64 * T);
    const int sub0 = bx * (64 * T) + sub * 64;
    const int m0 = sub0 + wave * 16;
    const int my_row = m0 + i;

    constexpr int N4 = E * V * F / 4;
    constexpr int NST = (N4 + THREADS - 1) / THREADS;
    float4 wv[NST];
#pragma unroll
    for (int s = 0; s < NST; ++s) {
        const int x4 = tid + s * THREADS;
        wv[s] = (N4 % THREADS == 0 || x4 < N4) ? reinterpret_cast<const float4*>(filter)[x4] : make_float4(0.f, 0.f, 0.f, 0.f);
    }
    const int vt = wave / FT, ft = wave % FT;
    u32x4 va[2][3];
#pragma unroll
    for (int st = 0; st < 2; ++st) {
        float x[8];
#pragma unroll
        for (int j = 0; j < 8; ++j) {
            const int row = sub0 + 32 * st + 8 * q + j;
            const float xv = values[(size_t)min(row, m - 1) * V + vt * 16 + i];
            x[j] = (row < m) ? xv : 0.f;
        }
#pragma unroll
        for (int j = 0; j < 4; ++j) {
            unsigned int h0, m0_, l0, h1, m1_, l1;
            ln_split3_bits(x[2 * j], h0, m0_, l0);
            ln_split3_bits(x[2 * j + 1], h1, m1_, l1);
            va[st][0][j] = ln_pack_hi(h0, h1);
            va[st][1][j] = ln_pack_hi(m0_, m1_);
            va[st][2][j] = ln_pack_hi(l0, l1);
        }
    }
#ifndef LN_BWD_DEPTH
#define LN_BWD_DEPTH 2
#endif
    constexpr int DEPTH = LN_BWD_DEPTH;
    auto slot_of = [](int k) { return k == 0 ? E - 1 : k - 1; };
    const int lr = lane >> 3, c8 = lane & 7;
    int nb2[2][E];
#pragma unroll
    for (int j = 0; j < 2; ++j)
#pragma unroll
        for (int e = 0; e < E; ++e) {
            const int id = nbr[(size_t)min(m0 + 8 * j + lr, m - 1) * E + (e < E - 1 ? (e ^ 1) : e)];
            nb2[j][e] = (m0 + 8 * j + lr < m) ? id : -1;
        }
    floatx4 a[DEPTH + 1][2];
    auto gather = [&](int e, floatx4 (&dst)[2]) {
#pragma unroll
        for (int j = 0; j < 2; ++j) dst[j] = *reinterpret_cast<const floatx4*>(grad_out + (size_t)(nb2[j][e] >= 0 ? nb2[j][e] : 0) * F + c8 * 4);
    };
#pragma unroll
    for (int j = 0; j < 2; ++j)
        a[0][j] = *reinterpret_cast<const floatx4*>(grad_out + (size_t)(m0 + 8 * j + lr < m ? m0 + 8 * j + lr : 0) * F + c8 * 4);
#pragma unroll
    for (int k = 1; k < DEPTH && k < E; ++k) gather(slot_of(k), a[k % (DEPTH + 1)]);
#pragma unroll
    for (int s = 0; s < NST; ++s) {
        const int x4 = tid + s * THREADS;
        if (N4 % THREADS == 0 || x4 < N4) {
            const int x = x4 * 4;
            const int ev = x / F;
            const int f0 = x - ev * F;
            const int e = ev / V;
            const int v = ev - e * V;
            const float v4[4] = {wv[s].x, wv[s].y, wv[s].z, wv[s].w};
            unsigned int h[4], md[4], lo[4];
#pragma unroll
            for (int j = 0; j < 4; ++j) ln_split3_bits(v4[j], h[j], md[j], lo[j]);
            const int fr = (((e * NT + (v >> 4)) * 3) * 64 + (f0 >> 3) * 16 + ((v & 15) ^ (2 * (f0 >> 3)))) * 8 + (f0 & 7);
            *reinterpret_cast<uint2*>(s_fh + fr) = make_uint2(ln_pack_hi(h[0], h[1]), ln_pack_hi(h[2], h[3]));
            *reinterpret_cast<uint2*>(s_fh + fr + 64 * 8) = make_uint2(ln_pack_hi(md[0], md[1]), ln_pack_hi(md[2], md[3]));
            *reinterpret_cast<uint2*>(s_fh + fr + 2 * 64 * 8) = make_uint2(ln_pack_hi(lo[0], lo[1]), ln_pack_hi(lo[2], lo[3]));
        }
    }
    floatx4 acc_v[NT];
#pragma unroll
    for (int nt = 0; nt < NT; ++nt) acc_v[nt] = floatx4{0.f, 0.f, 0.f, 0.f};
    floatx4 acc_w[E];
#pragma unroll
    for (int e = 0; e < E; ++e) acc_w[e] = floatx4{0.f, 0.f, 0.f, 0.f};
#pragma unroll
    for (int k = 0; k < E; ++k) {
        const int e = slot_of(k);
        unsigned short* sg = s_stage + (size_t)sub * STAGE + (k & 1) * (3 * PART);
        if (k + DEPTH < E) gather(slot_of(k + DEPTH), a[(k + DEPTH) % (DEPTH + 1)]);
#pragma unroll
        for (int j = 0; j < 2; ++j) {
            const floatx4 x = a[k % (DEPTH + 1)][j];
            const bool there = nb2[j][e] >= 0;
            unsigned int h[4], md[4], lo[4];
#pragma unroll
            for (int c = 0; c < 4; ++c) ln_split3_bits(there ? x[c] : 0.f, h[c], md[c], lo[c]);
            const int row = wave * 16 + 8 * j + lr;
            unsigned short* dst = sg + row * RS + (((c8 >> 1) ^ swz(row)) * 8 + (c8 & 1) * 4);
            *reinterpret_cast<uint2*>(dst) = make_uint2(ln_pack_hi(h[0], h[1]), ln_pack_hi(h[2], h[3]));
            *reinterpret_cast<uint2*>(dst + PART) = make_uint2(ln_pack_hi(md[0], md[1]), ln_pack_hi(md[2], md[3]));
            *reinterpret_cast<uint2*>(dst + 2 * PART) = make_uint2(ln_pack_hi(lo[0], lo[1]), ln_pack_hi(lo[2], lo[3]));
        }
        __syncthreads();
        u32x4 p1, p2, p3;
        {
            const unsigned short* src = sg + (wave * 16 + i) * RS + ((q ^ swz(wave * 16 + i)) * KQ);
            p1 = *reinterpret_cast<const u32x4*>(src);
            p2 = *reinterpret_cast<const u32x4*>(src + PART);
            p3 = *reinterpret_cast<const u32x4*>(src + 2 * PART);
        }
        const bf16x8 a1 = __builtin_bit_cast(bf16x8, p1), a2 = __builtin_bit_cast(bf16x8, p2), a3 = __builtin_bit_cast(bf16x8, p3);
#pragma unroll
        for (int nt = 0; nt < NT; ++nt) {
            const u32x4* pb = s_frag + ((e * NT + nt) * 3) * 64 + q * 16 + (i ^ (2 * q));
            const bf16x8 b1 = __builtin_bit_cast(bf16x8, pb[0]), b2 = __builtin_bit_cast(bf16x8, pb[64]), b3 = __builtin_bit_cast(bf16x8, pb[128]);
            acc_v[nt] = __builtin_amdgcn_mfma_f32_16x16x32_bf16(a3, b1, acc_v[nt], 0, 0, 0);
            acc_v[nt] = __builtin_amdgcn_mfma_f32_16x16x32_bf16(a1, b3, acc_v[nt], 0, 0, 0);
            acc_v[nt] = __builtin_amdgcn_mfma_f32_16x16x32_bf16(a2, b2, acc_v[nt], 0, 0, 0);
            acc_v[nt] = __builtin_amdgcn_mfma_f32_16x16x32_bf16(a2, b1, acc_v[nt], 0, 0, 0);
            acc_v[nt] = __builtin_amdgcn_mfma_f32_16x16x32_bf16(a1, b2, acc_v[nt], 0, 0, 0);
            acc_v[nt] = __builtin_amdgcn_mfma_f32_16x16x32_bf16(a1, b1, acc_v[nt], 0, 0, 0);
        }
        floatx4 w0 = floatx4{0.f, 0.f, 0.f, 0.f}, w1 = floatx4{0.f, 0.f, 0.f, 0.f};
#pragma unroll
        for (int st = 0; st < 2; ++st) {
            bf16x8 b[3];
#pragma unroll
            for (int part = 0; part < 3; ++part) {
                const int r_lo = 32 * st + 8 * q + (i >> 2), r_hi = r_lo + 4;
                const int piece = ft * 2 + ((i & 3) >> 1), inner = (i & 1) * 4;
                const unsigned short* base = sg + part * PART + r_lo * RS + (piece ^ swz(r_lo)) * 8 + inner;
                const unsigned short* base_hi = sg + part * PART + r_hi * RS + (piece ^ swz(r_hi)) * 8 + inner;
                const short4v lo4 = __builtin_amdgcn_ds_read_tr16_b64_v4i16((short4v __attribute__((address_space(3)))*)(base));
                const short4v hi4 = __builtin_amdgcn_ds_read_tr16_b64_v4i16((short4v __attribute__((address_space(3)))*)(base_hi));
                u32x4 packed;
                packed[0] = (unsigned int)(unsigned short)lo4[0] | ((unsigned int)(unsigned short)lo4[1] << 16);
                packed[1] = (unsigned int)(unsigned short)lo4[2] | ((unsigned int)(unsigned short)lo4[3] << 16);
                packed[2] = (unsigned int)(unsigned short)hi4[0] | ((unsigned int)(unsigned short)hi4[1] << 16);
                packed[3] = (unsigned int)(unsigned short)hi4[2] | ((unsigned int)(unsigned short)hi4[3] << 16);
                b[part] = __builtin_bit_cast(bf16x8, packed);
            }
            const bf16x8 v1 = __builtin_bit_cast(bf16x8, va[st][0]), v2 = __builtin_bit_cast(bf16x8, va[st][1]), v3 = __builtin_bit_cast(bf16x8, va[st][2]);
            floatx4& acc = st ? w1 : w0;
            acc = __builtin_amdgcn_mfma_f32_16x16x32_bf16(v3, b[0], acc, 0, 0, 0);
            acc = __builtin_amdgcn_mfma_f32_16x16x32_bf16(v1, b[2], acc, 0, 0, 0);
            acc = __builtin_amdgcn_mfma_f32_16x16x32_bf16(v2, b[1], acc, 0, 0, 0);
            acc = __builtin_amdgcn_mfma_f32_16x16x32_bf16(v2, b[0], acc, 0, 0, 0);
            acc = __builtin_amdgcn_mfma_f32_16x16x32_bf16(v1, b[1], acc, 0, 0, 0);
            acc = __builtin_amdgcn_mfma_f32_16x16x32_bf16(v1, b[0], acc, 0, 0, 0);
        }
        acc_w[e] = w0 + w1;
    }
#pragma unroll
    for (int nt = 0; nt < NT; ++nt) {
#pragma unroll
        for (int r = 0; r < 4; ++r) {
            const int row = m0 + q * 4 + r;
            if (row < m) grad_values[(size_t)row * V + nt * 16 + i] = acc_v[nt][r];
        }
    }
    __syncthreads();
    float* park_all = reinterpret_cast<float*>(s_raw);
    const int colp = (ft * 16 + i) ^ ((q & 1) << 4);
    if (sub > 0) {
        float* park = park_all + (size_t)(sub - 1) * BANK;
#pragma unroll
        for (int e = 0; e < E; ++e)
#pragma unroll
            for (int r = 0; r < 4; ++r) park[(e * V + vt * 16 + q * 4 + r) * F + colp] = acc_w[e][r];
    }
    if constexpr (T > 1) __syncthreads();
    if (sub == 0) {
        float* dst = slabs + (size_t)blockIdx.x * BANK;
#pragma unroll
        for (int e = 0; e < E; ++e)
#pragma unroll
            for (int r = 0; r < 4; ++r) {
                const int o = (e * V + vt * 16 + q * 4 + r) * F + ft * 16 + i;
                float sum = acc_w[e][r];
#pragma unroll
                for (int k2 = 1; k2 < T; ++k2) sum += park_all[(k2 - 1) * BANK + (e * V + vt * 16 + q * 4 + r) * F + colp];
                dst[o] = sum;
            }
    }
}

template <int T, int C>
__global__ void __launch_bounds__(256 * T) __attribute__((amdgpu_waves_per_eu(T, T)))
    k_conv_backward_fused_b3_rows(const int* __restrict__ nbr, const float* __restrict__ values, const float* __restrict__ grad_out,
                             const float* __restrict__ filter, int m, float* __restrict__ grad_values, float* __restrict__ slabs,
                             const int* __restrict__ row_part) {
    constexpr int V = 32, F = 32, E = 9, KQ = 8, NT = 2, FT = 2;
    constexpr int THREADS = 256 * T;
    constexpr int BANK = E * V * F;
    constexpr int FRAG16 = E * NT * 3 * 64;
    constexpr int RS = 32;
    auto swz = [](int r) { return (0x78 >> (2 * ((r >> 2) & 3))) & 3; };
    constexpr int PART = 64 * RS;
    constexpr int STAGE = 2 * 3 * PART;
    constexpr int LDS_BYTES_A = FRAG16 * 16 + T * STAGE * 2;
    constexpr int LDS_BYTES_B = (T - 1) * BANK * 4;
    constexpr int LDS_BYTES = LDS_BYTES_A > LDS_BYTES_B ? LDS_BYTES_A : LDS_BYTES_B;
    __shared__ __attribute__((aligned(16))) unsigned char s_raw[LDS_BYTES];
    u32x4* s_frag = reinterpret_cast<u32x4*>(s_raw);
    unsigned short* s_fh = reinterpret_cast<unsigned short*>(s_raw);
    unsigned short* s_stage = reinterpret_cast<unsigned short*>(s_raw + FRAG16 * 16);
    const int tid = threadIdx.x;
    const int sub = tid >> 8;
    const int t256 = tid & 255;
    const int lane = tid & 63;
    const int wave = t256 >> 6;
    const int i = lane & 15;
    const int q = lane >> 4;
    const int bx0 = ln_partition_tile(blockIdx.x, gridDim.x, row_part, 64 * T * C) * C;
    const int sub00 = bx0 * (64 * T) + sub * 64;
    const int m00 = sub00 + wave * 16;

    constexpr int N4 = E * V * F / 4;
    constexpr int NST = (N4 + THREADS - 1) / THREADS;
    float4 wv[NST];
#pragma unroll
    for (int s = 0; s < NST; ++s) {
        const int x4 = tid + s * THREADS;
        wv[s] = (N4 % THREADS == 0 || x4 < N4) ? reinterpret_cast<const float4*>(filter)[x4] : make_float4(0.f, 0.f, 0.f, 0.f);
    }
    const int vt = wave / FT, ft = wave % FT;
    floatx4 acc_w[E];
#pragma unroll
    for (int c = 0; c < C; ++c) {
    const int sub0 = sub00 + c * (64 * T);
    const int m0 = m00 + c * (64 * T);
    if (c > 0 && (bx0 + c) * (64 * T) >= m) break;
    u32x4 va[2][3];
#pragma unroll
    for (int st = 0; st < 2; ++st) {
        float x[8];
#pragma unroll
        for (int j = 0; j < 8; ++j) {
            const int row = sub0 + 32 * st + 8 * q + j;
            const float xv = values[(size_t)min(row, m - 1) * V + vt * 16 + i];
            x[j] = (row < m) ? xv : 0.f;
        }
#pragma unroll
        for (int j = 0; j < 4; ++j) {
            unsigned int h0, m0_, l0, h1, m1_, l1;
            ln_split3_bits(x[2 * j], h0, m0_, l0);
            ln_split3_bits(x[2 * j + 1], h1, m1_, l1);
            va[st][0][j] = ln_pack_hi(h0, h1);
            va[st][1][j] = ln_pack_hi(m0_, m1_);
            va[st][2][j] = ln_pack_hi(l0, l1);
        }
    }
#ifndef LN_BWD_DEPTH
#define LN_BWD_DEPTH 2
#endif
    constexpr int DEPTH = LN_BWD_DEPTH;
    auto slot_of = [](int k) { return k == 0 ? E - 1 : k - 1; };
    const int lr = lane >> 3, c8 = lane & 7;
    int nb2[2][E];
#pragma unroll
    for (int j = 0; j < 2; ++j)
#pragma unroll
        for (int e = 0; e < E; ++e) {
            const int id = nbr[(size_t)min(m0 + 8 * j + lr, m - 1) * E + (e < E - 1 ? (e ^ 1) : e)];
            nb2[j][e] = (m0 + 8 * j + lr < m) ? id : -1;
        }
    floatx4 a[DEPTH + 1][2];
    auto gather = [&](int e, floatx4 (&dst)[2]) {
#pragma unroll
        for (int j = 0; j < 2; ++j) dst[j] = *reinterpret_cast<const floatx4*>(grad_out + (size_t)(nb2[j][e] >= 0 ? nb2[j][e] : 0) * F + c8 * 4);
    };
#pragma unroll
    for (int j = 0; j < 2; ++j)
        a[0][j] = *reinterpret_cast<const floatx4*>(grad_out + (size_t)(m0 + 8 * j + lr < m ? m0 + 8 * j + lr : 0) * F + c8 * 4);
#pragma unroll
    for (int k = 1; k < DEPTH && k < E; ++k) gather(slot_of(k), a[k % (DEPTH + 1)]);
    if (c == 0) {
#pragma unroll
    for (int s = 0; s < NST; ++s) {
        const int x4 = tid + s * THREADS;
        if (N4 % THREADS == 0 || x4 < N4) {
            const int x = x4 * 4;
            const int ev = x / F;
            const int f0 = x - ev * F;
            const int e = ev / V;
            const int v = ev - e * V;
            const float v4[4] = {wv[s].x, wv[s].y, wv[s].z, wv[s].w};
            unsigned int h[4], md[4], lo[4];
#pragma unroll
            for (int j = 0; j < 4; ++j) ln_split3_bits(v4[j], h[j], md[j], lo[j]);
            const int fr = (((e * NT + (v >> 4)) * 3) * 64 + (f0 >> 3) * 16 + ((v & 15) ^ (2 * (f0 >> 3)))) * 8 + (f0 & 7);
            *reinterpret_cast<uint2*>(s_fh + fr) = make_uint2(ln_pack_hi(h[0], h[1]), ln_pack_hi(h[2], h[3]));
            *reinterpret_cast<uint2*>(s_fh + fr + 64 * 8) = make_uint2(ln_pack_hi(md[0], md[1]), ln_pack_hi(md[2], md[3]));
            *reinterpret_cast<uint2*>(s_fh + fr + 2 * 64 * 8) = make_uint2(ln_pack_hi(lo[0], lo[1]), ln_pack_hi(lo[2], lo[3]));
        }
    }
    }
    floatx4 acc_v[NT];
#pragma unroll
    for (int nt = 0; nt < NT; ++nt) acc_v[nt] = floatx4{0.f, 0.f, 0.f, 0.f};
#pragma unroll
    for (int k = 0; k < E; ++k) {
        const int e = slot_of(k);
        unsigned short* sg = s_stage + (size_t)sub * STAGE + ((c * E + k) & 1) * (3 * PART);
        if (k + DEPTH < E) gather(slot_of(k + DEPTH), a[(k + DEPTH) % (DEPTH + 1)]);
#pragma unroll
        for (int j = 0; j < 2; ++j) {
            const floatx4 x = a[k % (DEPTH + 1)][j];
            const bool there = nb2[j][e] >= 0;
            unsigned int h[4], md[4], lo[4];
#pragma unroll
            for (int cc = 0; cc < 4; ++cc) ln_split3_bits(there ? x[cc] : 0.f, h[cc], md[cc], lo[cc]);
            const int row = wave * 16 + 8 * j + lr;
            unsigned short* dst = sg + row * RS + (((c8 >> 1) ^ swz(row)) * 8 + (c8 & 1) * 4);
            *reinterpret_cast<uint2*>(dst) = make_uint2(ln_pack_hi(h[0], h[1]), ln_pack_hi(h[2], h[3]));
            *reinterpret_cast<uint2*>(dst + PART) = make_uint2(ln_pack_hi(md[0], md[1]), ln_pack_hi(md[2], md[3]));
            *reinterpret_cast<uint2*>(dst + 2 * PART) = make_uint2(ln_pack_hi(lo[0], lo[1]), ln_pack_hi(lo[2], lo[3]));
        }
        __syncthreads();
        u32x4 p1, p2, p3;
        {
            const unsigned short* src = sg + (wave * 16 + i) * RS + ((q ^ swz(wave * 16 + i)) * KQ);
            p1 = *reinterpret_cast<const u32x4*>(src);
            p2 = *reinterpret_cast<const u32x4*>(src + PART);
            p3 = *reinterpret_cast<const u32x4*>(src + 2 * PART);
        }
        const bf16x8 a1 = __builtin_bit_cast(bf16x8, p1), a2 = __builtin_bit_cast(bf16x8, p2), a3 = __builtin_bit_cast(bf16x8, p3);
#pragma unroll
        for (int nt = 0; nt < NT; ++nt) {
            const u32x4* pb = s_frag + ((e * NT + nt) * 3) * 64 + q * 16 + (i ^ (2 * q));
            const bf16x8 b1 = __builtin_bit_cast(bf16x8, pb[0]), b2 = __builtin_bit_cast(bf16x8, pb[64]), b3 = __builtin_bit_cast(bf16x8, pb[128]);
            acc_v[nt] = __builtin_amdgcn_mfma_f32_16x16x32_bf16(a3, b1, acc_v[nt], 0, 0, 0);
            acc_v[nt] = __builtin_amdgcn_mfma_f32_16x16x32_bf16(a1, b3, acc_v[nt], 0, 0, 0);
            acc_v[nt] = __builtin_amdgcn_mfma_f32_16x16x32_bf16(a2, b2, acc_v[nt], 0, 0, 0);
            acc_v[nt] = __builtin_amdgcn_mfma_f32_16x16x32_bf16(a2, b1, acc_v[nt], 0, 0, 0);
            acc_v[nt] = __builtin_amdgcn_mfma_f32_16x16x32_bf16(a1, b2, acc_v[nt], 0, 0, 0);
            acc_v[nt] = __builtin_amdgcn_mfma_f32_16x16x32_bf16(a1, b1, acc_v[nt], 0, 0, 0);
        }
        floatx4 w0 = floatx4{0.f, 0.f, 0.f, 0.f}, w1 = floatx4{0.f, 0.f, 0.f, 0.f};
#pragma unroll
        for (int st = 0; st < 2; ++st) {
            bf16x8 b[3];
#pragma unroll
            for (int part = 0; part < 3; ++part) {
                const int r_lo = 32 * st + 8 * q + (i >> 2), r_hi = r_lo + 4;
                const int piece = ft * 2 + ((i & 3) >> 1), inner = (i & 1) * 4;
                const unsigned short* base = sg + part * PART + r_lo * RS + (piece ^ swz(r_lo)) * 8 + inner;
                const unsigned short* base_hi = sg + part * PART + r_hi * RS + (piece ^ swz(r_hi)) * 8 + inner;
                const short4v lo4 = __builtin_amdgcn_ds_read_tr16_b64_v4i16((short4v __attribute__((address_space(3)))*)(base));
                const short4v hi4 = __builtin_amdgcn_ds_read_tr16_b64_v4i16((short4v __attribute__((address_space(3)))*)(base_hi));
                u32x4 packed;
                packed[0] = (unsigned int)(unsigned short)lo4[0] | ((unsigned int)(unsigned short)lo4[1] << 16);
                packed[1] = (unsigned int)(unsigned short)lo4[2] | ((unsigned int)(unsigned short)lo4[3] << 16);
                packed[2] = (unsigned int)(unsigned short)hi4[0] | ((unsigned int)(unsigned short)hi4[1] << 16);
                packed[3] = (unsigned int)(unsigned short)hi4[2] | ((unsigned int)(unsigned short)hi4[3] << 16);
                b[part] = __builtin_bit_cast(bf16x8, packed);
            }
            const bf16x8 v1 = __builtin_bit_cast(bf16x8, va[st][0]), v2 = __builtin_bit_cast(bf16x8, va[st][1]), v3 = __builtin_bit_cast(bf16x8, va[st][2]);
            floatx4& acc = st ? w1 : w0;
            acc = __builtin_amdgcn_mfma_f32_16x16x32_bf16(v3, b[0], acc, 0, 0, 0);
            acc = __builtin_amdgcn_mfma_f32_16x16x32_bf16(v1, b[2], acc, 0, 0, 0);
            acc = __builtin_amdgcn_mfma_f32_16x16x32_bf16(v2, b[1], acc, 0, 0, 0);
            acc = __builtin_amdgcn_mfma_f32_16x16x32_bf16(v2, b[0], acc, 0, 0, 0);
            acc = __builtin_amdgcn_mfma_f32_16x16x32_bf16(v1, b[1], acc, 0, 0, 0);
            acc = __builtin_amdgcn_mfma_f32_16x16x32_bf16(v1, b[0], acc, 0, 0, 0);
        }
        if (c == 0) acc_w[e] = w0 + w1;
        else acc_w[e] += w0 + w1;
    }
#pragma unroll
    for (int nt = 0; nt < NT; ++nt) {
#pragma unroll
        for (int r = 0; r < 4; ++r) {
            const int row = m0 + q * 4 + r;
            if (row < m) grad_values[(size_t)row * V + nt * 16 + i] = acc_v[nt][r];
        }
    }
    }
    __syncthreads();
    float* park_all = reinterpret_cast<float*>(s_raw);
    const int colp = (ft * 16 + i) ^ ((q & 1) << 4);
    if (sub > 0) {
        float* park = park_all + (size_t)(sub - 1) * BANK;
#pragma unroll
        for (int e = 0; e < E; ++e)
#pragma unroll
            for (int r = 0; r < 4; ++r) park[(e * V + vt * 16 + q * 4 + r) * F + colp] = acc_w[e][r];
    }
    if constexpr (T > 1) __syncthreads();
    if (sub == 0) {
        float* dst = slabs + (size_t)blockIdx.x * BANK;
#pragma unroll
        for (int e = 0; e < E; ++e)
#pragma unroll
            for (int r = 0; r < 4; ++r) {
                const int o = (e * V + vt * 16 + q * 4 + r) * F + ft * 16 + i;
                float sum = acc_w[e][r];
#pragma unroll
                for (int k2 = 1; k2 < T; ++k2) sum += park_all[(k2 - 1) * BANK + (e * V + vt * 16 + q * 4 + r) * F + colp];
                dst[o] = sum;
            }
    }
}

template <int T>
static void ln_bwd_launch_fused(const LnBwdPlan& p, const int* nbr, const float* values, const float* grad_out, const float* filter, int m,
                                float* grad_values, float* partial, const int* row_partition, hipStream_t st) {
    if constexpr (T <= LN_BWD_B3_MAX_T) {
        if (p.form == LN_BWD_FUSED_B3) {
            if constexpr (T == LN_CONV_OVL_T) {
                if (p.c > 1) {
                    LN_LAUNCH("k_conv_backward_fused", (k_conv_backward_fused_b3_rows<T, LN_CONV_OVL_C>), dim3(p.grid), dim3(p.block), 0, st, nbr, values, grad_out,
                              filter, m, grad_values, partial, row_partition);
                    return;
                }
            }
            LN_LAUNCH("k_conv_backward_fused", (k_conv_backward_fused_b3<T>), dim3(p.grid), dim3(p.block), 0, st, nbr, values, grad_out, filter, m,
                      grad_values, partial, row_partition);
            return;
        }
    }
    LN_LAUNCH("k_conv_backward_fused", (k_conv_backward_fused<32, 32, 9, T>), dim3(p.grid), dim3(p.block), 0, st, nbr, values, grad_out, filter, m,
              grad_values, partial);
}

extern "C" size_t ln_conv_backward_workspace_bytes(int mq, int mn, int filter_extent, int val_dim, int nr_filters) {
    return ln_conv_backward_query(mq, mn, filter_extent, val_dim, nr_filters, ln_conv_b3_enabled());
}

extern "C" int ln_conv_backward_flags(const int* nbr_q, const int* nbr_n, const float* values_neigh, const float* grad_out, const float* filter,
                                      int mq, int mn, int filter_extent, int val_dim, int nr_filters, int flags, float* grad_values,
                                      float* grad_filter, void* workspace, size_t workspace_bytes, const int* row_partition, void* stream) {
    hipStream_t st = (hipStream_t)stream;
    LN_REQUIRE((flags & ~LN_CONV_OVERLAPPED) == 0, LN_ERR_ARG, "ln_conv_backward: unknown flags %d", flags);
    const LnBwdPlan p = ln_conv_backward_plan(LnBwdPlanIn{
        mq, mn, filter_extent, val_dim, nr_filters, nbr_q == nbr_n,
        nbr_q && nbr_n && values_neigh && grad_out && filter && grad_values && grad_filter, workspace ? workspace_bytes : 0,
        ln_aligned16(values_neigh) && ln_aligned16(grad_out) && ln_aligned16(filter), ln_conv_b3_enabled(), (flags & LN_CONV_OVERLAPPED) != 0});
    float* partial = static_cast<float*>(workspace);
    const int total = filter_extent * val_dim * nr_filters;
    if (p.form == LN_BWD_FUSED_B3 || p.form == LN_BWD_FUSED_F32) {
        switch (p.t) {
            case 1: ln_bwd_launch_fused<1>(p, nbr_n, values_neigh, grad_out, filter, mn, grad_values, partial, row_partition, st); break;
            case 2: ln_bwd_launch_fused<2>(p, nbr_n, values_neigh, grad_out, filter, mn, grad_values, partial, row_partition, st); break;
            case 3: ln_bwd_launch_fused<3>(p, nbr_n, values_neigh, grad_out, filter, mn, grad_values, partial, row_partition, st); break;
            default: ln_bwd_launch_fused<4>(p, nbr_n, values_neigh, grad_out, filter, mn, grad_values, partial, row_partition, st); break;
        }
        (void)ln_reduce_slabs_async(partial, p.grid, total, grad_filter, st);
        return ln_check_launch("ln_conv_backward");
    }
    if (p.form == LN_BWD_FULL_SUM) {
        const LnGfPlan gf = ln_gf_plan(mq, filter_extent, val_dim, nr_filters, ln_conv_b3_enabled());
        ln_gf_launch_partials(gf, nbr_q, values_neigh, grad_out, mq, filter_extent, val_dim, nr_filters, partial, st);
        ln_conv_launch_full<true, true>(nr_filters, val_dim / 16, dim3(p.grid), st, nbr_n, grad_out, filter, mn, grad_values, p.conv_blocks,
                                        (const float*)partial, gf.chunks, total, grad_filter);
        return ln_check_launch("ln_conv_backward");
    }
    LnSlabSum sum = {nullptr, 0, 0, nullptr};
    int rc = ln_conv_grad_filter_impl(nbr_q, values_neigh, grad_out, mq, filter_extent, val_dim, nr_filters, grad_filter, workspace, workspace_bytes,
                                      stream, &sum);
    if (rc) return rc;
    const size_t gf_bytes = ln_bwd_gf_bytes(mq, filter_extent, val_dim, nr_filters, ln_conv_b3_enabled());
    char* conv_ws = (workspace && workspace_bytes > gf_bytes) ? static_cast<char*>(workspace) + gf_bytes : nullptr;
    rc = ln_conv_forward_riding(nbr_n, grad_out, filter, mn, filter_extent, nr_filters, val_dim, LN_CONV_FLIP_NEIGHBOURS | LN_CONV_TRANSPOSED_FILTER,
                                grad_values, conv_ws, conv_ws ? workspace_bytes - gf_bytes : 0, row_partition, stream, sum);
    return rc ? rc : ln_check_launch("ln_conv_backward");
}

extern "C" int ln_conv_backward(const int* nbr_q, const int* nbr_n, const float* values_neigh, const float* grad_out, const float* filter, int mq,
                                int mn, int filter_extent, int val_dim, int nr_filters, float* grad_values, float* grad_filter,
                                void* workspace, size_t workspace_bytes, const int* row_partition, void* stream) {
    return ln_conv_backward_flags(nbr_q, nbr_n, values_neigh, grad_out, filter, mq, mn, filter_extent, val_dim, nr_filters, 0, grad_values,
                                  grad_filter, workspace, workspace_bytes, row_partition, stream);
}

extern "C" size_t ln_linear_backward_workspace_bytes(int rows, int cin, int cout) {
    return ln_linear_backward_query(rows, cin, cout, ln_conv_b3_enabled());
}

extern "C" int ln_linear_backward(const int* ident, const float* x, const float* grad_y, const float* w, int rows, int cin, int cout,
                                  float* grad_x, float* grad_w, void* workspace, size_t workspace_bytes, void* stream) {
    LN_REQUIRE(rows >= 0 && cin >= 1 && cout >= 1 && grad_w, LN_ERR_ARG, "ln_linear_backward: bad sizes / null output");
    LN_REQUIRE(workspace && workspace_bytes >= ln_linear_backward_workspace_bytes(rows, cin, cout), LN_ERR_WORKSPACE,
               "ln_linear_backward: workspace too small");
    const size_t gf_bytes = ln_bwd_gf_bytes(rows, 1, cout, cin, ln_conv_b3_enabled());
    const bool conv = grad_x && rows > 0;
    LnSlabSum sum = {nullptr, 0, 0, nullptr};
    int rc = ln_conv_grad_filter_impl(ident, grad_y, x, rows, 1, cout, cin, grad_w, workspace, gf_bytes, stream, conv ? &sum : nullptr);
    if (rc) return rc;
    if (conv)
        rc = ln_conv_forward_riding(ident, grad_y, w, rows, 1, cout, cin, 0, grad_x, static_cast<char*>(workspace) + gf_bytes,
                                    workspace_bytes - gf_bytes, nullptr, stream, sum);
    return rc ? rc : ln_check_launch("ln_linear_backward");
}
```

lattice_net_amd/csrc/ln_conv_plan.h:

```cpp
#pragma once
#include <stddef.h>
#include <stdint.h>

#define LN_BWD_MAX_SUBTILES 4
#define LN_BWD_CUS 256
#ifndef LN_BWD_B3_MAX_T
#define LN_BWD_B3_MAX_T 3
#endif
#ifndef LN_CONV_LDS_E
#define LN_CONV_LDS_E 16
#endif
#define LN_CONV_B3_WAVES(V) ((V) <= 128 ? 3 : 2)
#ifndef LN_CONV_SPLIT_TILES
#define LN_CONV_SPLIT_TILES 512
#endif
#ifndef LN_CONV_WIDE_SPLIT_MIN_V
#define LN_CONV_WIDE_SPLIT_MIN_V 128
#endif
#ifndef LN_CONV_B3_MIN_ROWS
#define LN_CONV_B3_MIN_ROWS 4096
#endif
#ifndef LN_GF_ROWS
#define LN_GF_ROWS 320
#endif
#ifndef LN_GFB_SUB
#define LN_GFB_SUB 64
#endif
#ifndef LN_GFB_EG
#define LN_GFB_EG 3
#endif
#ifndef LN_GFB_W128F
#define LN_GFB_W128F 2
#endif
#define LN_GFB_SLAB_BYTES (24ll << 20)

constexpr int ln_cdiv(long long a, long long b) { return int((a + b - 1) / b); }

constexpr bool ln_conv_per_slot_v(int V) {
    return V == 8 || V == 16 || V == 32 || V == 48 || V == 64 || V == 96 || V == 128 || V == 192 || V == 256;
}
constexpr int ln_conv_nt_max(int V) { return (V * 16 * 8 * 4 <= 32 * 1024) ? 8 : ((V * 16 * 4 * 4 <= 48 * 1024) ? 4 : 2); }
constexpr bool ln_conv_chunk_fits(int V, int NT) { return (NT == 8 || NT == 4 || NT == 2 || NT == 1) && NT <= ln_conv_nt_max(V); }
constexpr bool ln_conv_chunk_b3_spills(int V, int NT) { return V >= 256 && NT > 1; }
constexpr bool ln_conv_chunk_b3(int V, int NT) { return V % 32 == 0 && V * 16 * NT * 6 <= 64 * 1024 && !ln_conv_chunk_b3_spills(V, NT); }
constexpr bool ln_conv_b3_three_subtiles(int V) { return LN_CONV_B3_WAVES(V) == 3; }
constexpr int ln_conv_b3_subtiles(int V, int m, int chunks) {
    return ln_conv_b3_three_subtiles(V) && (long long)ln_cdiv(m, 192) * chunks >= LN_BWD_CUS * 3 / 4 ? 3 : 1;
}
constexpr bool ln_conv_wide_built(int V, int NT) { return V % 32 == 0 && NT >= 1 && NT <= 4; }
constexpr bool ln_conv_wide_shape(int V, int F) { return V % 32 == 0 && V >= 96 && F % 32 == 0; }
constexpr int ln_conv_r32_ntw(int NT) { return NT == 4 ? 2 : (NT == 3 ? 3 : 1); }
constexpr int ln_conv_r32_ch(int NT) { return NT % 2 == 0 ? 2 : 1; }
constexpr int ln_conv_r32_rt(int NT) { return NT % 2 == 0 ? 6 : 4; }
constexpr int LN_CONV_R32SK_RT = 6;
constexpr bool ln_conv_full_shape(int V, int F) {
    return (V == 8 || V == 16 || V == 32) && (F == 16 || F == 32 || F == 64 || F == 128) && V * F <= 1024;
}
constexpr bool ln_conv_small_filter(int E, int V, int F) { return E == 9 && (size_t)E * V * F * 4 <= 64 * 1024 && V <= 32; }
constexpr bool ln_bwd_fused_shape(int E, int V, int F) { return E == 9 && V == 32 && F == 32; }

constexpr int LN_CONV_OVL_T = 2;
constexpr int LN_CONV_OVL_C = 2;
constexpr int LN_CONV_OVL_MAX_ROWS = 2 * 64 * LN_BWD_B3_MAX_T * LN_BWD_CUS;
constexpr bool ln_bwd_narrow(int m, bool b3_enabled, bool overlapped) {
    return overlapped && b3_enabled && m >= LN_CONV_B3_MIN_ROWS && m <= LN_CONV_OVL_MAX_ROWS;
}
constexpr int ln_bwd_subtiles(int m, bool b3_enabled, bool overlapped = false) {
    if (ln_bwd_narrow(m, b3_enabled, overlapped)) return LN_CONV_OVL_T;
    const int max_t = b3_enabled ? LN_BWD_B3_MAX_T : LN_BWD_MAX_SUBTILES;
    const int s = (m + 63) / 64;
    int best = 1, best_cost = 1 << 30;
    for (int t = 1; t <= max_t; ++t) {
        const int wgs = (s + t - 1) / t;
        const int cost = ((wgs + LN_BWD_CUS - 1) / LN_BWD_CUS) * (t + 1);
        if (cost <= best_cost) {
            best = t;
            best_cost = cost;
        }
    }
    return best;
}
constexpr int ln_bwd_chunks(int m, bool b3_enabled, bool overlapped = false) { return ln_bwd_narrow(m, b3_enabled, overlapped) ? LN_CONV_OVL_C : 1; }
static_assert(LN_CONV_OVL_T * LN_CONV_OVL_C >= LN_BWD_B3_MAX_T, "the narrow form would write more slabs than the workspace queries report");
constexpr int ln_bwd_workgroups(int m, bool b3_enabled, bool overlapped = false) {
    return ln_cdiv(m, 64 * ln_bwd_subtiles(m, b3_enabled, overlapped) * ln_bwd_chunks(m, b3_enabled, overlapped));
}

constexpr size_t ln_conv_bank_bytes(int m, int E, int V, int F, bool b3_enabled) {
    if (V % 32 != 0 || F % 16 != 0 || m < LN_CONV_B3_MIN_ROWS || E > LN_CONV_LDS_E || !b3_enabled) return 0;
    return (((size_t)E * V * F * 3 * sizeof(unsigned short)) + 255) & ~size_t(255);
}
constexpr int ln_conv_slots_per_split(int V, int m, int E, int F) {
    if (!ln_conv_per_slot_v(V)) return E;
    const long long tiles = (long long)ln_cdiv(m, 64) * ln_cdiv(F, 16 * ln_conv_nt_max(V));
    if (tiles * 2 > LN_CONV_SPLIT_TILES || E < 2) return E;
    int nsplit = int((LN_CONV_SPLIT_TILES + tiles - 1) / tiles);
    if (nsplit > E) nsplit = E;
    return (E + nsplit - 1) / nsplit;
}
constexpr bool ln_conv_wide_fills_chip(int m, int F) { return (long long)ln_cdiv(m, 192) * ln_cdiv(F, 128) >= LN_BWD_CUS / 2; }
constexpr int ln_conv_wide_split(int V, int m, int E, int F, bool have_bank) {
    if (!have_bank || !ln_conv_per_slot_v(V) || V % 32 != 0 || V < LN_CONV_WIDE_SPLIT_MIN_V || F % 32 != 0 || E < 3 || m < LN_CONV_B3_MIN_ROWS)
        return 0;
    if (ln_conv_wide_fills_chip(m, F)) return 0;
    const long long wgs = (long long)ln_cdiv(m, 192) * (F >= 128 ? F / 128 : 1);
    int best = 1;
    long long best_cost = 1ll << 60;
    for (int n = 2; n <= E; ++n) {
        const long long cost = ((wgs * n + LN_BWD_CUS - 1) / LN_BWD_CUS) * ((E + n - 1) / n);
        if (cost < best_cost) {
            best = n;
            best_cost = cost;
        }
    }
    return best;
}
struct LnConvLayout {
    size_t bank_bytes;
    int wide_split;
    int nsplit, e_per;
};
constexpr LnConvLayout ln_conv_layout(int m, int E, int V, int F, bool b3_enabled, bool have_bank) {
    LnConvLayout l = {ln_conv_bank_bytes(m, E, V, F, b3_enabled), 0, 1, ln_conv_slots_per_split(V, m, E, F)};
    l.wide_split = ln_conv_wide_split(V, m, E, F, l.bank_bytes > 0 && have_bank);
    if (l.wide_split > 1) l.e_per = (E + l.wide_split - 1) / l.wide_split;
    l.nsplit = (E + l.e_per - 1) / l.e_per;
    return l;
}
constexpr size_t ln_conv_slab_bytes(int nsplit, int m, int F) { return nsplit > 1 ? (size_t)nsplit * m * F * sizeof(float) : 0; }
constexpr size_t ln_conv_bank_query(int m, int E, int V, int F, bool b3_enabled) {
    if (m <= 0 || F % 16 != 0 || ln_conv_small_filter(E, V, F)) return 0;
    return ln_conv_bank_bytes(m, E, V, F, b3_enabled);
}
constexpr size_t ln_conv_forward_query(int m, int E, int V, int F, bool b3_enabled) {
    if (m <= 0 || F % 16 != 0) return 256;
    return ln_conv_bank_query(m, E, V, F, b3_enabled) + ln_conv_slab_bytes(ln_conv_layout(m, E, V, F, b3_enabled, true).nsplit, m, F) + 256;
}

enum LnConvKernel : uint8_t {
    LN_K_FORWARD_B3,
    LN_K_FULL,
    LN_K_SPLIT_BANK32,
    LN_K_ROWS32,
    LN_K_ROWS32SK,
    LN_K_SPLIT_BANK,
    LN_K_MFMA_B3,
    LN_K_MFMA,
    LN_K_SUM_PARTIALS,
    LN_K_GENERIC,
};
struct LnConvLaunch {
    uint8_t kernel;
    uint8_t nt, t;
    uint8_t c;
    bool carries_sum;
    int grid[3], block;
    int f_off, cols;
    int split_x;
    size_t bank_off;
    size_t bank_elems;
};
#define LN_CONV_MAX_LAUNCHES 10
struct LnConvPlanIn {
    int m, E, V, F;
    bool flip, wt;
    bool b3_enabled;
    bool values_aligned, filter_aligned;
    bool ws_aligned;
    size_t ws_bytes;
    bool bank_ready;
    int riding_total;
    bool overlapped = false;
};
struct LnConvPlan {
    size_t bank_bytes, slab_bytes;
    int nsplit, e_per;
    bool sum_left;
    int n;
    LnConvLaunch launch[LN_CONV_MAX_LAUNCHES];
};

inline LnConvLaunch* ln_plan_add(LnConvPlan& p, LnConvKernel k, int nt, int t, int gx, int gy, int gz, int block, int f_off, int cols) {
    LnConvLaunch& l = p.launch[p.n++];
    l = LnConvLaunch{uint8_t(k), uint8_t(nt), uint8_t(t), 1, false, {gx, gy, gz}, block, f_off, cols, 0, 0, 0};
    return &l;
}

inline LnConvPlan ln_conv_plan(const LnConvPlanIn& in) {
    const int m = in.m, E = in.E, V = in.V, F = in.F;
    LnConvPlan p = {};
    p.nsplit = 1;
    p.e_per = E;
    p.sum_left = in.riding_total > 0;
    if (E == 9 && in.filter_aligned) {
        if (!in.flip && !in.wt && V == 32 && F == 32 && m >= LN_CONV_B3_MIN_ROWS && in.b3_enabled && in.values_aligned) {
            const int bt = ln_bwd_subtiles(m, true, in.overlapped), t = bt < 3 ? bt : 3, c = ln_bwd_chunks(m, true, in.overlapped);
            ln_plan_add(p, LN_K_FORWARD_B3, 2, t, ln_cdiv(m, 64 * t * c), 1, 1, 256 * t, 0, F)->c = uint8_t(c);
            return p;
        }
        if (ln_conv_full_shape(V, F)) {
            ln_plan_add(p, LN_K_FULL, F / 16, 1, ln_cdiv(m, 64), 1, 1, 256, 0, F);
            return p;
        }
    }
    if (!(F % 16 == 0 && in.values_aligned && in.filter_aligned && ln_conv_per_slot_v(V))) {
        ln_plan_add(p, LN_K_GENERIC, 0, 0, ln_cdiv((long long)m * F, 256), 1, 1, 256, 0, F);
        return p;
    }
    const size_t bank_bytes = ln_conv_bank_bytes(m, E, V, F, in.b3_enabled);
    const bool b3 = bank_bytes > 0 && in.ws_aligned && in.ws_bytes >= bank_bytes;
    const LnConvLayout lay = ln_conv_layout(m, E, V, F, in.b3_enabled, b3);
    p.bank_bytes = b3 ? bank_bytes : 0;
    p.nsplit = lay.nsplit;
    p.e_per = lay.e_per;
    if (p.nsplit > 1 && (!in.ws_aligned || in.ws_bytes - p.bank_bytes < ln_conv_slab_bytes(p.nsplit, m, F))) {
        p.e_per = E;
        p.nsplit = 1;
    }
    p.slab_bytes = ln_conv_slab_bytes(p.nsplit, m, F);
    const int nsplit = p.nsplit;
    int f_off = 0;
    size_t bank_off = 0;
    auto split = [&](LnConvKernel k, int nt, int cnt, int cols_per_chunk) {
        if (in.bank_ready) return;
        const int sx = ln_cdiv(V * cols_per_chunk, 256);
        LnConvLaunch* l = ln_plan_add(p, k, nt, 1, sx, E, cnt, 256, f_off, cnt * cols_per_chunk);
        l->split_x = sx;
        l->bank_off = bank_off;
        l->bank_elems = (size_t)E * cnt * V * cols_per_chunk * 3;
        if (p.sum_left) {
            l->carries_sum = true;
            l->grid[0] += ln_cdiv(in.riding_total / 64, E * cnt);
            p.sum_left = false;
        }
    };
    auto conv = [&](LnConvKernel k, int nt, int t, int rows, int block, int cnt, int cols_per_chunk, bool banked) {
        LnConvLaunch* l = ln_plan_add(p, k, nt, t, ln_cdiv(m, rows), cnt, nsplit, block, f_off, cnt * cols_per_chunk);
        if (banked) {
// ... 162 lines not shown
```

lattice_net_amd/lattice.py:

```python
from __future__ import annotations

import ctypes as C
import itertools
import os
import re
import weakref
from typing import Optional, Sequence

import torch
import torch.utils.weak

from . import _lib

__all__ = ["Lattice", "HashTable", "set_row_order", "get_row_order", "set_hash_capacity_policy", "set_slot_order", "set_bank_cache", "set_deterministic"]


_SIZE_CACHE = {}
_FORCE_ATOMIC_BUILD = os.environ.get("LATTICE_BUILD_PATH", "") == "atomic"

_ROW_ORDER = [os.environ.get("LATTICE_ROW_ORDER", "slot")]


_HASH_POLICY = [os.environ.get("LATTICE_HASH_CAPACITY", "tokens")]
_STATIC_SLOTS_PER_ROW = float(os.environ.get("LATTICE_STATIC_SLOTS_PER_ROW", "2.3"))
# ... 932 lines not shown
            nh.m_values_tensor = torch.zeros((oh.capacity(), oh.val_dim() or v), dtype=torch.float32, device=dev)
            nh._zero_beyond = (weakref.ref(nh.m_values_tensor), 0)
            nh._counters = nh._storage.fresh_counters
            nh.clear(lazy=True)
        else:
            nh._storage = oh._storage.clone()
            nh.m_values_tensor = torch.zeros_like(oh.m_values_tensor)
            nh._counters = oh._counters.clone()
        idx, w = new._build(positions_raw, True, vals=values, distributed=distributed)
        new._after_build(lambda: new._prefetch_neighbours(n * (d + 1)))
        new._trace_level()
        return new, distributed, idx, w

    def expand(self, positions_raw: torch.Tensor, point_multiplier: int, noise_stddev: float, expand_values: bool):
        self._check_positions(positions_raw)
        d = positions_raw.shape[1]
        self._ensure_table(d, 1, positions_raw)
        pos = positions_raw.repeat(point_multiplier, 1)
        pos = pos + torch.randn_like(pos) * noise_stddev
        new = Lattice._clone_of(self)
        new.m_name = "expanded_lattice"
        oh, nh = self.m_hash_table, new.m_hash_table
        nh._storage = oh._storage.clone()
        nh.m_values_tensor = torch.zeros((1, self.val_dim()), dtype=torch.float32, device=self._dev())
        nh._counters = oh._counters.clone()
        new.just_create_verts(pos.contiguous(), False)
        if expand_values:
            diff = new.nr_lattice_vertices() - self.nr_lattice_vertices()
            if diff < 0:
                raise _lib.LatticeNetHipError("expand produced fewer vertices than the source lattice")
            new.set_values(torch.nn.functional.pad(self.values()[: self.nr_lattice_vertices()], (0, 0, 0, diff)))
        return new

    def _accumulate_and_prefetch(self, values, idx, w, dst, val_dim, src_div, tokens):
        ht = self.m_hash_table
        st = ht._storage
        rows_upper = min(ht.capacity(), tokens)
        _, csr, max_seg, grp_row, _ = self._csr(idx)
        if rows_upper <= 0 or max_seg <= 0 or not self.prefetch_neighbours:
            return self._scatter_rows(values, idx, w, dst, val_dim, src_div, val_dim)
        lib = _lib.load()
        nbr = torch.empty((rows_upper, self.get_filter_extent(1)), dtype=torch.int32, device=self._dev())
        t = ht.c_table()
        fn, what = (lib.ln_splat_accumulate_and_neighbours_f16, "ln_splat_accumulate_and_neighbours_f16") if values.dtype == torch.float16 \
            else (lib.ln_splat_accumulate_and_neighbours, "ln_splat_accumulate_and_neighbours")
        csr.dense = self._dense_hint(tokens)
        _lib.check(fn(C.byref(csr), _lib.ptr(grp_row), max_seg, _lib.ptr(values), _lib.ptr(w), val_dim, src_div, val_dim, _lib.ptr(dst),
                      C.byref(t), rows_upper, _lib.ptr(nbr), self._stream()), what)
        st.nbr_cache[("prefetch", st.uid, st.version, self.m_lvl)] = (nbr,)

    def _prefetch_neighbours(self, tokens: int):
        ht = self.m_hash_table
        st = ht._storage
        rows_upper = min(ht.capacity(), tokens)
        if rows_upper <= 0:
            return
        lib = _lib.load()
        E = self.get_filter_extent(1)
        nbr = torch.empty((rows_upper, E), dtype=torch.int32, device=self._dev())
        t = ht.c_table()
        _lib.check(lib.ln_neighbours(C.byref(t), rows_upper, C.byref(t), self.m_lvl, self.m_lvl, 1, 0, _lib.ptr(nbr), self._stream()),
                   "ln_neighbours")
        st.nbr_cache[("prefetch", st.uid, st.version, self.m_lvl)] = (nbr,)


    def neighbours(self, lattice_neighbours: Optional["Lattice"], dilation: int, flip_neighbours: bool) -> torch.Tensor:
        nb = lattice_neighbours if lattice_neighbours is not None else self
        if abs(self.m_lvl - nb.m_lvl) > 1:
            raise ValueError(f"query lvl {self.m_lvl} and neighbours lvl {nb.m_lvl} must differ by at most 1")
        m = self.nr_lattice_vertices()
        if m == 0:
            raise _lib.LatticeNetHipError("this lattice has zero vertices")
        sq, sn = self.m_hash_table._storage, nb.m_hash_table._storage
        key = (sn.uid, sn.version, self.m_lvl, nb.m_lvl, int(dilation), bool(flip_neighbours), m)
        hit = sq.nbr_cache.get(key)
        if hit is not None:
            return hit[0]
        E = self.get_filter_extent(1)
        pre = sq.nbr_cache.get(("prefetch", sn.uid, sn.version, self.m_lvl)) if (sn is sq and not flip_neighbours and dilation == 1 and
                                                                                  nb.m_lvl == self.m_lvl) else None
        if pre is not None and pre[0].shape[0] >= m:
            nbr = pre[0][:m]
            sq.nbr_cache[key] = (nbr,)
            return nbr
        if flip_neighbours:
            base = self.neighbours(nb, dilation, False)
            perm = [e ^ 1 for e in range(E - 1)] + [E - 1]
            nbr = base[:, perm].contiguous()
        else:
            lib = _lib.load()
            nbr = torch.empty((m, E), dtype=torch.int32, device=self._dev())
            tq, tn = self.m_hash_table.c_table(), nb.m_hash_table.c_table()
            _lib.check(lib.ln_neighbours(C.byref(tq), m, C.byref(tn), self.m_lvl, nb.m_lvl, int(dilation), 0, _lib.ptr(nbr),
                                         self._stream()), "ln_neighbours")
        sq.nbr_cache[key] = (nbr,)
        return nbr

    def _row_partition(self):
        st = self.m_hash_table._storage
        if st is None or not st.rows_follow_space or st.row_regions is None:
            return None
        return st.row_regions.data_ptr()

    def _check_filter_extent(self, filter_extent: int):
        if filter_extent != self.get_filter_extent(1):
            raise ValueError(f"filter extent should be {self.get_filter_extent(1)} (1-hop neighbourhood + centre), got {filter_extent}")

    def convolve_im2row_standalone(self, filter_bank: torch.Tensor, dilation: int, lattice_neighbours: Optional["Lattice"],
                                   flip_neighbours: bool, filter_is_transposed: bool = False) -> "Lattice":
        nb = lattice_neighbours if lattice_neighbours is not None else self
        if filter_bank is None or filter_bank.dim() != 2:
            raise ValueError("filter bank should be 2-D: (filter_extent * val_dim) x nr_filters")
        filter_bank = filter_bank.contiguous()
        v = nb.val_dim()
        E = self.get_filter_extent(1)
        if filter_is_transposed:
            if filter_bank.shape[1] != v or filter_bank.shape[0] % E != 0:
                raise ValueError(f"transposed filter bank should be (filter_extent * nr_filters) x val_dim={v}, got {tuple(filter_bank.shape)}")
            nr_filters = int(filter_bank.shape[0]) // E
            filter_extent = E
        else:
            nr_filters = int(filter_bank.shape[1])
            filter_extent = filter_bank.shape[0] // v
            self._check_filter_extent(filter_extent)
            if filter_bank.shape[0] != filter_extent * v:
                raise ValueError("filter bank rows must be filter_extent * val_dim")
        nbr = self.neighbours(nb, dilation, False)
        m = nbr.shape[0]
        vals = nb.values()
        half = vals.dtype == torch.float16
        if filter_bank.dtype != vals.dtype:
            raise ValueError(f"filter bank is {filter_bank.dtype}, lattice values are {vals.dtype}")
        out = torch.empty((m, nr_filters), dtype=vals.dtype, device=self._dev())
        flags = (_lib.LN_CONV_FLIP_NEIGHBOURS if flip_neighbours else 0) | (_lib.LN_CONV_TRANSPOSED_FILTER if filter_is_transposed else 0)
        lib = _lib.load()
        if not half and _SCANS_IN_FLIGHT[0] > 1:
            flags |= _lib.LN_CONV_OVERLAPPED
        if half:
            _lib.check(lib.ln_conv_forward_f16(_lib.ptr(nbr), _lib.ptr(vals), _lib.ptr(filter_bank), m, filter_extent, v, nr_filters, flags,
                                               _lib.ptr(out), self._stream()), "ln_conv_forward_f16")
        else:
            wsb = int(lib.ln_conv_forward_workspace_bytes(m, filter_extent, v, nr_filters))
            ws = None
            key = None
            bank_b = int(lib.ln_conv_bank_workspace_bytes(m, filter_extent, v, nr_filters))
            if bank_b > 0 and wsb == bank_b + 256 and _BANK_CACHE[0] and not filter_bank.requires_grad and \
                    not torch.cuda.is_current_stream_capturing():
                key = (filter_bank.data_ptr(), filter_bank._version, m, filter_extent, v, nr_filters, flags, self._stream())
                hit = _BANK_ENTRIES.get(filter_bank)
                if hit is not None and hit[0] == key:
                    ws, flags = hit[1], flags | _lib.LN_CONV_BANK_READY
            if ws is None and wsb > 256:
                ws = torch.empty((wsb,), dtype=torch.uint8, device=self._dev())
            _lib.check(lib.ln_conv_forward_ws(_lib.ptr(nbr), _lib.ptr(vals), _lib.ptr(filter_bank), m, filter_extent, v, nr_filters, flags,
                                              _lib.ptr(out), _lib.ptr(ws), 0 if ws is None else ws.numel(), self._row_partition(),
                                              self._stream()), "ln_conv_forward")
            if key is not None and not (flags & _lib.LN_CONV_BANK_READY):
                try:
                    _BANK_ENTRIES[filter_bank] = (key, ws)
                except TypeError:
                    pass
        conv = Lattice._clone_of(self)
        conv.m_name = "convolved_lattice"
        conv.m_hash_table.set_values(out)
        return conv

    def convolve_im2row_backward(self, grad_out: torch.Tensor, filter_bank: torch.Tensor, dilation: int,
                                 query: Optional["Lattice"], neighbours: Optional["Lattice"], filter_grad_fp32: bool = False):
        q = query if query is not None else self
        nb = neighbours if neighbours is not None else self
        lib = _lib.load()
        main = self._stream()
        E = q.get_filter_extent(1)
        grad_out = grad_out.contiguous()
        filter_bank = filter_bank.contiguous()
        v = nb.val_dim()
        f = int(filter_bank.shape[1])
        if filter_bank.shape[0] != E * v or grad_out.shape[1] != f:
            raise ValueError("filter bank / gradient shapes do not match the forward convolution")
        nbr_q = q.neighbours(nb, dilation, False)
        mq = nbr_q.shape[0]
        if grad_out.shape[0] != mq:
            raise ValueError(f"grad_out has {grad_out.shape[0]} rows, the query lattice has {mq} vertices")
        dev = self._dev()
        half = grad_out.dtype == torch.float16
        if filter_bank.dtype != grad_out.dtype or nb.values().dtype != grad_out.dtype:
            raise ValueError("grad_out, filter bank and lattice values must share one dtype (float32 or float16)")
        gf = torch.empty((E * v, f), dtype=torch.float32, device=dev)
        ws_bytes = int(lib.ln_conv_grad_filter_f16_workspace_bytes(mq, E, v, f) if half else
                       lib.ln_conv_backward_workspace_bytes(mq, int(nb.nr_lattice_vertices()), E, v, f))
        ws = torch.empty((max(ws_bytes, 256),), dtype=torch.uint8, device=dev)
        nbr_n = nb.neighbours(q, dilation, False)
        mn = nbr_n.shape[0]
        gvals = torch.empty((mn, v), dtype=grad_out.dtype, device=dev)
        if half:
            _lib.check(lib.ln_conv_grad_filter_f16(_lib.ptr(nbr_q), _lib.ptr(nb.values()), _lib.ptr(grad_out), mq, E, v, f, _lib.ptr(gf),
                                                   _lib.ptr(ws), ws.numel(), main), "ln_conv_grad_filter_f16")
            flags = _lib.LN_CONV_FLIP_NEIGHBOURS | _lib.LN_CONV_TRANSPOSED_FILTER
            _lib.check(lib.ln_conv_forward_f16(_lib.ptr(nbr_n), _lib.ptr(grad_out), _lib.ptr(filter_bank), mn, E, f, v, flags, _lib.ptr(gvals),
                                               main), "ln_conv_forward_f16")
            return gvals, (gf if filter_grad_fp32 else gf.to(torch.float16))
        part = nb._row_partition() if q.m_hash_table._storage is nb.m_hash_table._storage else None
        flags = _lib.LN_CONV_OVERLAPPED if _SCANS_IN_FLIGHT[0] > 1 else 0
        _lib.check(lib.ln_conv_backward_flags(_lib.ptr(nbr_q), _lib.ptr(nbr_n), _lib.ptr(nb.values()), _lib.ptr(grad_out), _lib.ptr(filter_bank),
                                              mq, mn, E, v, f, flags, _lib.ptr(gvals), _lib.ptr(gf), _lib.ptr(ws), ws.numel(), part, main),
                   "ln_conv_backward")
        return gvals, gf

    def convolve_im2row_grad_filter(self, grad_out: torch.Tensor, dilation: int, lattice_neighbours: Optional["Lattice"],
                                    filter_extent: int) -> torch.Tensor:
        nb = lattice_neighbours if lattice_neighbours is not None else self
        self._check_filter_extent(filter_extent)
        grad_out = grad_out.contiguous()
        nbr = self.neighbours(nb, dilation, False)
        m = nbr.shape[0]
        v = nb.val_dim()
        f = int(grad_out.shape[1])
        if grad_out.shape[0] != m:
            raise ValueError(f"grad_out has {grad_out.shape[0]} rows, lattice has {m} vertices")
        lib = _lib.load()
        gf = torch.empty((filter_extent * v, f), dtype=torch.float32, device=self._dev())
        ws = self._workspace(lib.ln_conv_grad_filter_workspace_bytes(m, filter_extent, v, f))
        _lib.check(lib.ln_conv_grad_filter(_lib.ptr(nbr), _lib.ptr(nb.values()), _lib.ptr(grad_out), m, filter_extent, v, f,
                                           _lib.ptr(gf), _lib.ptr(ws), ws.numel(), self._stream()), "ln_conv_grad_filter")
        return gf

    def im2row(self, lattice_neighbours: Optional["Lattice"], filter_extent: int, dilation: int, flip_neighbours: bool):
        nb = lattice_neighbours if lattice_neighbours is not None else self
        self._check_filter_extent(filter_extent)
        nbr = self.neighbours(nb, dilation, flip_neighbours)
        m = nbr.shape[0]
        v = nb.val_dim()
        out = torch.empty((m, filter_extent * v), dtype=torch.float32, device=self._dev())
        lib = _lib.load()
        _lib.check(lib.ln_im2row(_lib.ptr(nbr), _lib.ptr(nb.values()), m, filter_extent, v, _lib.ptr(out), self._stream()), "ln_im2row")
        return out

    def im2rowindices(self, lattice_neighbours: Optional["Lattice"], filter_extent: int, dilation: int, flip_neighbours: bool):
        nb = lattice_neighbours if lattice_neighbours is not None else self
        self._check_filter_extent(filter_extent)
        nbr = self.neighbours(nb, dilation, flip_neighbours)
        m = nbr.shape[0]
        v = nb.val_dim()
        out = torch.empty((m, filter_extent * v), dtype=torch.int32, device=self._dev())
        lib = _lib.load()
        _lib.check(lib.ln_im2rowindices(_lib.ptr(nbr), m, filter_extent, v, _lib.ptr(out), self._stream()), "ln_im2rowindices")
        return out

    def row2im(self, lattice_rowified: torch.Tensor, dilation: int, filter_extent: int, nr_filters: int,
               lattice_neighbours: Optional["Lattice"]):
        nb = lattice_neighbours if lattice_neighbours is not None else self
        if not lattice_rowified.is_contiguous():
            raise ValueError("lattice rowified is not contiguous, call .contiguous() on it")
        v = lattice_rowified.shape[1] // filter_extent
        if v != self.val_dim():
            raise ValueError(f"each rowified row should be val_dim*filter_extent long: row {lattice_rowified.shape[1]}, val_dim {self.val_dim()}")
        nbr = self.neighbours(nb, dilation, False)
        m = nbr.shape[0]
        out = torch.empty((m, v), dtype=torch.float32, device=self._dev())
        lib = _lib.load()
        _lib.check(lib.ln_row2im(_lib.ptr(nbr), _lib.ptr(lattice_rowified), m, filter_extent, v, _lib.ptr(out), self._stream()), "ln_row2im")
        self.m_hash_table.m_values_tensor = out
        return out

    def _new_coarse(self) -> "Lattice":
        capacity = self.m_hash_table.capacity()
        d = self.pos_dim()
        dev = self._dev()
        coarse = Lattice._clone_of(self)
        coarse.m_name = "coarse_lattice"
        coarse.m_lvl = self.m_lvl + 1
        coarse.m_sigmas = [s * 2.0 for s in self.m_sigmas]
        coarse._sigmas_tensor = None
        ht = HashTable(capacity)
        bp, step = self.m_hash_table._batch
        ht._batch = (bp, (step // (2 * (d + 1))) * (d + 1)) if bp else (0, 0)
        ht._cloud_lengths, ht._cloud_starts = self.m_hash_table._cloud_lengths, self.m_hash_table._cloud_starts
        ht._per_cloud_norm = self.m_hash_table._per_cloud_norm
        ht._per_cloud_invalid_vertex = self.m_hash_table._per_cloud_invalid_vertex
        ht._many_clouds = self.m_hash_table._many_clouds
        ht._band = self.m_hash_table._band
        ht._storage = _TableStorage(capacity, d, dev, spare_row_width=self.val_dim())
        ht.m_values_tensor = ht._storage.fresh_row if ht._storage.fresh_row is not None else torch.zeros((1, self.val_dim()), dtype=torch.float32, device=dev)
        ht._counters = ht._storage.fresh_counters
        levels = getattr(self.m_hash_table, "_static_levels", None)
        if self.m_hash_table._static_rows is not None:
            if not levels or coarse.m_lvl not in levels:
                raise _lib.LatticeNetHipError(f"static-rows mode: no row bound for lattice level {coarse.m_lvl} "
                                              "(set_static_rows(bound, coarse_bounds=[...]))")
            ht._static_rows = min(int(levels[coarse.m_lvl]), capacity)
        ht._static_levels = levels
        coarse.m_hash_table = ht
        ht.clear(lazy=True)
        return coarse

    def create_coarse_verts(self) -> "Lattice":
        coarse = self._new_coarse()
        coarse.m_hash_table._storage.key_format = _lib.LN_KEYS_RAW
        lib = _lib.load()
        m = self.nr_lattice_vertices()
        tokens = m * (2 * (self.pos_dim() + 1) + 1)
        coarse._choose_hash_capacity(tokens, fresh=True)
        cap = coarse.m_hash_table._storage.hashed()
        ws = self._workspace(_build_sizes(tokens, cap)[0])
        csr_buf, csr, _ = self._alloc_csr(tokens, cap)
        tf, tc = self.m_hash_table.c_table(), coarse.m_hash_table.c_table()
        _lib.check(lib.ln_coarsen(C.byref(tf), m, C.byref(tc), C.byref(csr), _lib.ptr(ws), ws.numel(), self._stream()), "ln_coarsen")
        coarse.m_hash_table._storage.touch()
        coarse.m_hash_table.m_nr_filled_is_dirty = True
        nr = coarse.nr_lattice_vertices()
        coarse.m_hash_table.m_values_tensor = torch.zeros((nr, self.val_dim()), dtype=torch.float32, device=self._dev())
        coarse._trace_level()
        return coarse

    def create_coarse_verts_naive(self, positions_raw: torch.Tensor) -> "Lattice":
        self._check_positions(positions_raw)
        coarse = self._new_coarse()
        coarse.just_create_verts(positions_raw, False)
        coarse._trace_level()
        return coarse

    def _check_slice_inputs(self, positions_raw, idx, w):
        self._check_positions(positions_raw)
        if self.val_dim() <= 0:
            raise ValueError("val_dim is 0: splat something first")
        if positions_raw.shape[1] != self.pos_dim():
            raise ValueError("position dimension does not match the lattice")
        n = positions_raw.shape[0]
        expect = n * (self.pos_dim() + 1)
        if idx is None or w is None or idx.numel() != expect or w.numel() != expect:
            raise ValueError(f"indices / weights must have {expect} elements")
        return n

    def slice_standalone_with_precomputation(self, positions_raw, splatting_indices_tensor, splatting_weights_tensor,
                                             grad_accumulator: Optional[torch.Tensor] = None):
        idx, w = splatting_indices_tensor.contiguous(), splatting_weights_tensor.contiguous()
        n = self._check_slice_inputs(positions_raw, idx, w)
        vals = self.values()
        lib = _lib.load()
        if vals.dtype == torch.float16:
            out = torch.empty((n, self.val_dim()), dtype=torch.float16, device=self._dev())
            if grad_accumulator is None:
                _lib.check(lib.ln_slice_forward_f16(_lib.ptr(vals), _lib.ptr(idx), _lib.ptr(w), n, self.pos_dim(), self.val_dim(), _lib.ptr(out),
                                                    self._stream()), "ln_slice_forward_f16")
            else:
                _lib.check(lib.ln_slice_forward_f16_prepare_backward(_lib.ptr(vals), _lib.ptr(idx), _lib.ptr(w), n, self.pos_dim(), self.val_dim(),
                                                                     _lib.ptr(out), _lib.ptr(grad_accumulator), grad_accumulator.numel(),
                                                                     self._stream()), "ln_slice_forward_f16_prepare_backward")
            return out
        out = torch.empty((n, self.val_dim()), dtype=torch.float32, device=self._dev())
        st = self.m_hash_table._storage
        hit = st.csr_cache.get((idx.data_ptr(), idx._version, idx.numel())) if (st is not None and st.rows_follow_space and _ORDERED_SLICE[0]) else None
        if hit is not None and hit[3] is not None:
            t = self.m_hash_table.c_table()
            _lib.check(lib.ln_slice_forward_ordered(C.byref(t), C.byref(hit[1]), _lib.ptr(vals), _lib.ptr(idx), _lib.ptr(w), n, self.val_dim(),
                                                    _lib.ptr(out), _lib.ptr(grad_accumulator),
                                                    0 if grad_accumulator is None else grad_accumulator.numel(), self._stream()),
                       "ln_slice_forward_ordered")
# ... 472 lines not shown
```

Measured before the change: 1506.

## Skip dead row tiles in b3 conv kernels using device-side live row count

Passes a device-resident count of live lattice rows into the bf16x3 forward and fused backward conv kernels. Workgroups whose tile starts past that count only zero their output rows, and their filter-gradient slab when needed, then exit instead of running the MFMA pipeline. When no row partition is in use, a new slab reducer sums only the slabs that belong to live workgroups. This targets the wasted compute from sizing grids to the hash-table capacity rather than the real vertex count, at the cost of extra template variants and a dependency on the live count being correct.

```diff
diff --git a/include/latticenet_hip.h b/include/latticenet_hip.h
--- a/include/latticenet_hip.h
+++ b/include/latticenet_hip.h
@@ -138,6 +138,9 @@
 size_t ln_conv_forward_workspace_bytes(int m, int filter_extent, int val_dim, int nr_filters);
 int ln_conv_forward_ws(const int* nbr, const float* values_neigh, const float* filter, int m, int filter_extent, int val_dim,
                        int nr_filters, int flags, float* out, void* workspace, size_t workspace_bytes, const int* row_partition, void* stream);
+int ln_conv_forward_ws_rows(const int* nbr, const float* values_neigh, const float* filter, int m, int filter_extent, int val_dim,
+                            int nr_filters, int flags, float* out, void* workspace, size_t workspace_bytes, const int* row_partition,
+                            const int* rows_device, void* stream);
 size_t ln_conv_grad_filter_workspace_bytes(int m, int filter_extent, int val_dim, int nr_filters);
 int ln_conv_grad_filter(const int* nbr, const float* values_neigh, const float* grad_out, int m, int filter_extent,
                         int val_dim, int nr_filters, float* grad_filter, void* workspace, size_t workspace_bytes,
@@ -176,6 +179,9 @@
 int ln_conv_backward_flags(const int* nbr_q, const int* nbr_n, const float* values_neigh, const float* grad_out, const float* filter, int mq,
                            int mn, int filter_extent, int val_dim, int nr_filters, int flags, float* grad_values, float* grad_filter,
                            void* workspace, size_t workspace_bytes, const int* row_partition, void* stream);
+int ln_conv_backward_rows(const int* nbr_q, const int* nbr_n, const float* values_neigh, const float* grad_out, const float* filter, int mq,
+                          int mn, int filter_extent, int val_dim, int nr_filters, int flags, float* grad_values, float* grad_filter,
+                          void* workspace, size_t workspace_bytes, const int* row_partition, const int* rows_device, void* stream);
 
 int ln_csr_reduce_rows_f16(const LnCsr* csr, const int* grp_row, long long max_segments, const void* src_f16, const float* w, int val_dim,
                            int src_div, int src_stride, float* dst, void* stream);
diff --git a/lattice_net_amd/_lib.py b/lattice_net_amd/_lib.py
--- a/lattice_net_amd/_lib.py
+++ b/lattice_net_amd/_lib.py
@@ -125,6 +125,7 @@
     "ln_conv_forward_workspace_bytes": (_sz, [_i, _i, _i, _i]),
     "ln_conv_bank_workspace_bytes": (_sz, [_i, _i, _i, _i]),
     "ln_conv_forward_ws": (_i, [_vp, _vp, _vp, _i, _i, _i, _i, _i, _vp, _vp, _sz, _vp, _vp]),
+    "ln_conv_forward_ws_rows": (_i, [_vp, _vp, _vp, _i, _i, _i, _i, _i, _vp, _vp, _sz, _vp, _vp, _vp]),
     "ln_conv_grad_filter_workspace_bytes": (_sz, [_i, _i, _i, _i]),
     "ln_conv_grad_filter": (_i, [_vp, _vp, _vp, _i, _i, _i, _i, _vp, _vp, _sz, _vp]),
     "ln_slice_forward": (_i, [_vp, _vp, _vp, _i, _i, _i, _vp, _vp]),
@@ -142,6 +143,7 @@
     "ln_conv_backward_workspace_bytes": (_sz, [_i, _i, _i, _i, _i]),
     "ln_conv_backward": (_i, [_vp, _vp, _vp, _vp, _vp, _i, _i, _i, _i, _i, _vp, _vp, _vp, _sz, _vp, _vp]),
     "ln_conv_backward_flags": (_i, [_vp, _vp, _vp, _vp, _vp, _i, _i, _i, _i, _i, _i, _vp, _vp, _vp, _sz, _vp, _vp]),
+    "ln_conv_backward_rows": (_i, [_vp, _vp, _vp, _vp, _vp, _i, _i, _i, _i, _i, _i, _vp, _vp, _vp, _sz, _vp, _vp, _vp]),
     "ln_conv_forward_f16": (_i, [_vp, _vp, _vp, _i, _i, _i, _i, _i, _vp, _vp]),
     "ln_conv_grad_filter_f16_workspace_bytes": (_sz, [_i, _i, _i, _i]),
     "ln_conv_grad_filter_f16": (_i, [_vp, _vp, _vp, _i, _i, _i, _i, _vp, _vp, _sz, _vp]),
diff --git a/lattice_net_amd/csrc/ln_conv.hip b/lattice_net_amd/csrc/ln_conv.hip
--- a/lattice_net_amd/csrc/ln_conv.hip
+++ b/lattice_net_amd/csrc/ln_conv.hip
@@ -987,10 +987,17 @@
     return ln_conv_forward_query(m, filter_extent, val_dim, nr_filters, ln_conv_b3_enabled());
 }
 
-template <int T>
+__device__ __forceinline__ int ln_conv_live_rows(int m, const int* __restrict__ rows_dev) { return max(0, min(m, *rows_dev)); }
+template <int THREADS>
+__device__ __forceinline__ void ln_conv_zero_rows32(float* __restrict__ out, int r0, int rows, int m) {
+    const int n4 = (min(r0 + rows, m) - r0) * 8;
+    for (int x = threadIdx.x; x < n4; x += THREADS) reinterpret_cast<float4*>(out + (size_t)r0 * 32)[x] = make_float4(0.f, 0.f, 0.f, 0.f);
+}
+
+template <int T, bool LIVE>
 __global__ void __launch_bounds__(256 * T) __attribute__((amdgpu_waves_per_eu(T, T)))
     k_conv_forward_b3(const int* __restrict__ nbr, const float* __restrict__ values, const float* __restrict__ filter, int m,
-                      float* __restrict__ out, const int* __restrict__ row_part) {
+                      float* __restrict__ out, const int* __restrict__ row_part, const int* __restrict__ rows_dev) {
     constexpr int V = 32, F = 32, E = 9, KQ = 8, NT = 2;
     constexpr int THREADS = 256 * T;
     constexpr int FRAG16 = E * NT * 3 * 64;
@@ -1005,6 +1012,12 @@
     const int bx = ln_partition_tile(blockIdx.x, gridDim.x, row_part, 64 * T);
     const int m0 = bx * (64 * T) + (tid >> 6) * 16;
     const int my_row = m0 + i;
+    if constexpr (LIVE) {
+        if (bx * (64 * T) >= ln_conv_live_rows(m, rows_dev)) {
+            ln_conv_zero_rows32<THREADS>(out, bx * (64 * T), 64 * T, m);
+            return;
+        }
+    }
     constexpr int ITEMS = E * (V / 8) * F;
     constexpr int NIT = (ITEMS + THREADS - 1) / THREADS;
     float wv[NIT][8];
@@ -1110,10 +1123,10 @@
         }
 }
 
-template <int T, int C>
+template <int T, int C, bool LIVE>
 __global__ void __launch_bounds__(256 * T) __attribute__((amdgpu_waves_per_eu(T, T)))
     k_conv_forward_b3_rows(const int* __restrict__ nbr, const float* __restrict__ values, const float* __restrict__ filter, int m,
-                      float* __restrict__ out, const int* __restrict__ row_part) {
+                      float* __restrict__ out, const int* __restrict__ row_part, const int* __restrict__ rows_dev) {
     constexpr int V = 32, F = 32, E = 9, KQ = 8, NT = 2;
     constexpr int THREADS = 256 * T;
     constexpr int FRAG16 = E * NT * 3 * 64;
@@ -1127,6 +1140,14 @@
     const int q = lane >> 4;
     const int bx0 = ln_partition_tile(blockIdx.x, gridDim.x, row_part, 64 * T * C) * C;
     const int m00 = bx0 * (64 * T) + (tid >> 6) * 16;
+    int live = m;
+    if constexpr (LIVE) {
+        live = ln_conv_live_rows(m, rows_dev);
+        if (bx0 * (64 * T) >= live) {
+            ln_conv_zero_rows32<THREADS>(out, bx0 * (64 * T), 64 * T * C, m);
+            return;
+        }
+    }
     constexpr int ITEMS = E * (V / 8) * F;
     constexpr int NIT = (ITEMS + THREADS - 1) / THREADS;
     float wv[NIT][8];
@@ -1143,6 +1164,12 @@
     for (int c = 0; c < C; ++c) {
     const int bx = bx0 + c;
     const int m0 = m00 + c * (64 * T);
+    if constexpr (LIVE) {
+        if (c > 0 && bx * (64 * T) >= live) {
+            ln_conv_zero_rows32<THREADS>(out, bx * (64 * T), 64 * T, m);
+            continue;
+        }
+    }
     {
         const size_t g0 = (size_t)bx * (64 * T) * E, g_end = (size_t)m * E;
         for (int x = tid; x < 64 * T * E; x += THREADS) s_nbr[x] = (g0 + x < g_end) ? nbr[g0 + x] : -1;
@@ -1253,6 +1280,7 @@
     int e_per;
     LnSlabSum sum;
     const int* row_partition;
+    const int* rows_dev;
     hipStream_t st;
 };
 
@@ -1368,12 +1396,21 @@
         switch (l.kernel) {
             case LN_K_FORWARD_B3:
                 if constexpr (!FLIP && !WT) {
+                    if (c.rows_dev && ln_aligned16(c.out)) {
+                        if (l.c > 1)
+                            LN_LAUNCH("k_conv_mfma", (k_conv_forward_b3_rows<LN_CONV_OVL_T, LN_CONV_OVL_C, true>), grid, block, 0, c.st, c.nbr, c.values, c.filter, c.m,
+                                      c.out, c.row_partition, c.rows_dev);
+                        else if (l.t == 1) LN_LAUNCH("k_conv_mfma", (k_conv_forward_b3<1, true>), grid, block, 0, c.st, c.nbr, c.values, c.filter, c.m, c.out, c.row_partition, c.rows_dev);
+                        else if (l.t == 2) LN_LAUNCH("k_conv_mfma", (k_conv_forward_b3<2, true>), grid, block, 0, c.st, c.nbr, c.values, c.filter, c.m, c.out, c.row_partition, c.rows_dev);
+                        else LN_LAUNCH("k_conv_mfma", (k_conv_forward_b3<3, true>), grid, block, 0, c.st, c.nbr, c.values, c.filter, c.m, c.out, c.row_partition, c.rows_dev);
+                        break;
+                    }
                     if (l.c > 1)
-                        LN_LAUNCH("k_conv_mfma", (k_conv_forward_b3_rows<LN_CONV_OVL_T, LN_CONV_OVL_C>), grid, block, 0, c.st, c.nbr, c.values, c.filter, c.m, c.out,
-                                  c.row_partition);
-                    else if (l.t == 1) LN_LAUNCH("k_conv_mfma", (k_conv_forward_b3<1>), grid, block, 0, c.st, c.nbr, c.values, c.filter, c.m, c.out, c.row_partition);
-                    else if (l.t == 2) LN_LAUNCH("k_conv_mfma", (k_conv_forward_b3<2>), grid, block, 0, c.st, c.nbr, c.values, c.filter, c.m, c.out, c.row_partition);
-                    else LN_LAUNCH("k_conv_mfma", (k_conv_forward_b3<3>), grid, block, 0, c.st, c.nbr, c.values, c.filter, c.m, c.out, c.row_partition);
+                        LN_LAUNCH("k_conv_mfma", (k_conv_forward_b3_rows<LN_CONV_OVL_T, LN_CONV_OVL_C, false>), grid, block, 0, c.st, c.nbr, c.values, c.filter, c.m, c.out,
+                                  c.row_partition, (const int*)nullptr);
+                    else if (l.t == 1) LN_LAUNCH("k_conv_mfma", (k_conv_forward_b3<1, false>), grid, block, 0, c.st, c.nbr, c.values, c.filter, c.m, c.out, c.row_partition, (const int*)nullptr);
+                    else if (l.t == 2) LN_LAUNCH("k_conv_mfma", (k_conv_forward_b3<2, false>), grid, block, 0, c.st, c.nbr, c.values, c.filter, c.m, c.out, c.row_partition, (const int*)nullptr);
+                    else LN_LAUNCH("k_conv_mfma", (k_conv_forward_b3<3, false>), grid, block, 0, c.st, c.nbr, c.values, c.filter, c.m, c.out, c.row_partition, (const int*)nullptr);
                 }
                 break;
             case LN_K_FULL:
@@ -1405,19 +1442,19 @@
 
 template <bool FLIP, bool WT>
 static void ln_conv_plan_and_run(LnConvPlanIn in, const int* nbr, const float* values, const float* filter, float* out, void* ws,
-                                 const LnSlabSum& sum, bool* sum_left, const int* row_partition, hipStream_t st) {
+                                 const LnSlabSum& sum, bool* sum_left, const int* row_partition, const int* rows_dev, hipStream_t st) {
     in.flip = FLIP;
     in.wt = WT;
     const LnConvPlan p = ln_conv_plan(in);
     char* slabs = static_cast<char*>(ws) + p.bank_bytes;
     ln_conv_run<FLIP, WT>(p, LnConvCall<FLIP, WT>{nbr, values, filter, in.m, in.E, in.V, in.F, out, static_cast<unsigned short*>(ws),
-                                                 p.nsplit > 1 ? reinterpret_cast<float*>(slabs) : out, p.e_per, sum, row_partition, st});
+                                                 p.nsplit > 1 ? reinterpret_cast<float*>(slabs) : out, p.e_per, sum, row_partition, rows_dev, st});
     *sum_left = p.sum_left;
 }
 
 static int ln_conv_forward_riding(const int* nbr, const float* values_neigh, const float* filter, int m, int filter_extent, int val_dim,
                                   int nr_filters, int flags, float* out, void* workspace, size_t workspace_bytes, const int* row_partition,
-                                  void* stream, const LnSlabSum& sum) {
+                                  void* stream, const LnSlabSum& sum, const int* rows_dev = nullptr) {
     hipStream_t st = (hipStream_t)stream;
     bool sum_left = sum.partial != nullptr;
     const int rc = [&]() -> int {
@@ -1436,10 +1473,10 @@
         in.riding_total = sum.partial ? sum.total : 0;
         in.overlapped = (flags & LN_CONV_OVERLAPPED) != 0;
         switch (flags & 3) {
-            case 0: ln_conv_plan_and_run<false, false>(in, nbr, values_neigh, filter, out, workspace, sum, &sum_left, row_partition, st); break;
-            case LN_CONV_FLIP_NEIGHBOURS: ln_conv_plan_and_run<true, false>(in, nbr, values_neigh, filter, out, workspace, sum, &sum_left, row_partition, st); break;
-            case LN_CONV_TRANSPOSED_FILTER: ln_conv_plan_and_run<false, true>(in, nbr, values_neigh, filter, out, workspace, sum, &sum_left, row_partition, st); break;
-            default: ln_conv_plan_and_run<true, true>(in, nbr, values_neigh, filter, out, workspace, sum, &sum_left, row_partition, st); break;
+            case 0: ln_conv_plan_and_run<false, false>(in, nbr, values_neigh, filter, out, workspace, sum, &sum_left, row_partition, rows_dev, st); break;
+            case LN_CONV_FLIP_NEIGHBOURS: ln_conv_plan_and_run<true, false>(in, nbr, values_neigh, filter, out, workspace, sum, &sum_left, row_partition, rows_dev, st); break;
+            case LN_CONV_TRANSPOSED_FILTER: ln_conv_plan_and_run<false, true>(in, nbr, values_neigh, filter, out, workspace, sum, &sum_left, row_partition, rows_dev, st); break;
+            default: ln_conv_plan_and_run<true, true>(in, nbr, values_neigh, filter, out, workspace, sum, &sum_left, row_partition, rows_dev, st); break;
         }
         return ln_check_launch("ln_conv_forward");
     }();
@@ -1452,6 +1489,13 @@
                                   void* stream) {
     return ln_conv_forward_riding(nbr, values_neigh, filter, m, filter_extent, val_dim, nr_filters, flags, out, workspace, workspace_bytes,
                                   row_partition, stream, LnSlabSum{nullptr, 0, 0, nullptr});
+}
+
+extern "C" int ln_conv_forward_ws_rows(const int* nbr, const float* values_neigh, const float* filter, int m, int filter_extent, int val_dim,
+                                       int nr_filters, int flags, float* out, void* workspace, size_t workspace_bytes, const int* row_partition,
+                                       const int* rows_device, void* stream) {
+    return ln_conv_forward_riding(nbr, values_neigh, filter, m, filter_extent, val_dim, nr_filters, flags, out, workspace, workspace_bytes,
+                                  row_partition, stream, LnSlabSum{nullptr, 0, 0, nullptr}, rows_device);
 }
 
 extern "C" int ln_conv_forward(const int* nbr, const float* values_neigh, const float* filter, int m, int filter_extent,
@@ -1975,11 +2019,17 @@
 }
 
 typedef short short4v __attribute__((ext_vector_type(4)));
-template <int T>
+template <int THREADS>
+__device__ __forceinline__ void ln_bwd_dead_workgroup(float* __restrict__ grad_values, int r0, int rows, int m, float* __restrict__ slab, int zero_slab) {
+    ln_conv_zero_rows32<THREADS>(grad_values, r0, rows, m);
+    if (zero_slab)
+        for (int x = threadIdx.x; x < 9 * 32 * 32 / 4; x += THREADS) reinterpret_cast<float4*>(slab)[x] = make_float4(0.f, 0.f, 0.f, 0.f);
+}
+template <int T, bool LIVE>
 __global__ void __launch_bounds__(256 * T) __attribute__((amdgpu_waves_per_eu(T, T)))
     k_conv_backward_fused_b3(const int* __restrict__ nbr, const float* __restrict__ values, const float* __restrict__ grad_out,
                              const float* __restrict__ filter, int m, float* __restrict__ grad_values, float* __restrict__ slabs,
-                             const int* __restrict__ row_part) {
+                             const int* __restrict__ row_part, const int* __restrict__ rows_dev, int zero_slab) {
     constexpr int V = 32, F = 32, E = 9, KQ = 8, NT = 2, FT = 2;
     constexpr int THREADS = 256 * T;
     constexpr int BANK = E * V * F;
@@ -2006,6 +2056,12 @@
     const int sub0 = bx * (64 * T) + sub * 64;
     const int m0 = sub0 + wave * 16;
     const int my_row = m0 + i;
+    if constexpr (LIVE) {
+        if (bx * (64 * T) >= ln_conv_live_rows(m, rows_dev)) {
+            ln_bwd_dead_workgroup<THREADS>(grad_values, bx * (64 * T), 64 * T, m, slabs + (size_t)blockIdx.x * BANK, zero_slab);
+            return;
+        }
+    }
 
     constexpr int N4 = E * V * F / 4;
     constexpr int NST = (N4 + THREADS - 1) / THREADS;
@@ -2187,11 +2243,12 @@
     }
 }
 
-template <int T, int C>
+
+template <int T, int C, bool LIVE>
 __global__ void __launch_bounds__(256 * T) __attribute__((amdgpu_waves_per_eu(T, T)))
     k_conv_backward_fused_b3_rows(const int* __restrict__ nbr, const float* __restrict__ values, const float* __restrict__ grad_out,
                              const float* __restrict__ filter, int m, float* __restrict__ grad_values, float* __restrict__ slabs,
-                             const int* __restrict__ row_part) {
+                             const int* __restrict__ row_part, const int* __restrict__ rows_dev, int zero_slab) {
     constexpr int V = 32, F = 32, E = 9, KQ = 8, NT = 2, FT = 2;
     constexpr int THREADS = 256 * T;
     constexpr int BANK = E * V * F;
@@ -2217,6 +2274,14 @@
     const int bx0 = ln_partition_tile(blockIdx.x, gridDim.x, row_part, 64 * T * C) * C;
     const int sub00 = bx0 * (64 * T) + sub * 64;
     const int m00 = sub00 + wave * 16;
+    int live = m;
+    if constexpr (LIVE) {
+        live = ln_conv_live_rows(m, rows_dev);
+        if (bx0 * (64 * T) >= live) {
+            ln_bwd_dead_workgroup<THREADS>(grad_values, bx0 * (64 * T), 64 * T * C, m, slabs + (size_t)blockIdx.x * BANK, zero_slab);
+            return;
+        }
+    }
 
     constexpr int N4 = E * V * F / 4;
     constexpr int NST = (N4 + THREADS - 1) / THREADS;
@@ -2233,6 +2298,12 @@
     const int sub0 = sub00 + c * (64 * T);
     const int m0 = m00 + c * (64 * T);
     if (c > 0 && (bx0 + c) * (64 * T) >= m) break;
+    if constexpr (LIVE) {
+        if (c > 0 && (bx0 + c) * (64 * T) >= live) {
+            ln_conv_zero_rows32<THREADS>(grad_values, (bx0 + c) * (64 * T), 64 * T * (C - c), m);
+            break;
+        }
+    }
     u32x4 va[2][3];
 #pragma unroll
     for (int st = 0; st < 2; ++st) {
@@ -2405,20 +2476,37 @@
     }
 }
 
+__global__ void __launch_bounds__(256) k_reduce_slabs4_live(const float* __restrict__ partial, int nslabs, int total, float* __restrict__ out,
+                                                            const int* __restrict__ rows_dev, int m, int rows_per_slab) {
+    ln_reduce_slabs4_block(blockIdx.x, partial, ln_live_slabs(ln_conv_live_rows(m, rows_dev), rows_per_slab, nslabs), total, out);
+}
+
 template <int T>
 static void ln_bwd_launch_fused(const LnBwdPlan& p, const int* nbr, const float* values, const float* grad_out, const float* filter, int m,
-                                float* grad_values, float* partial, const int* row_partition, hipStream_t st) {
+                                float* grad_values, float* partial, const int* row_partition, hipStream_t st, const int* rows_dev, int zero_slab) {
     if constexpr (T <= LN_BWD_B3_MAX_T) {
+        if (p.form == LN_BWD_FUSED_B3 && rows_dev) {
+            if constexpr (T == LN_CONV_OVL_T) {
+                if (p.c > 1) {
+                    LN_LAUNCH("k_conv_backward_fused", (k_conv_backward_fused_b3_rows<T, LN_CONV_OVL_C, true>), dim3(p.grid), dim3(p.block), 0, st, nbr, values,
+                              grad_out, filter, m, grad_values, partial, row_partition, rows_dev, zero_slab);
+                    return;
+                }
+            }
+            LN_LAUNCH("k_conv_backward_fused", (k_conv_backward_fused_b3<T, true>), dim3(p.grid), dim3(p.block), 0, st, nbr, values, grad_out, filter, m,
+                      grad_values, partial, row_partition, rows_dev, zero_slab);
+            return;
+        }
         if (p.form == LN_BWD_FUSED_B3) {
             if constexpr (T == LN_CONV_OVL_T) {
                 if (p.c > 1) {
-                    LN_LAUNCH("k_conv_backward_fused", (k_conv_backward_fused_b3_rows<T, LN_CONV_OVL_C>), dim3(p.grid), dim3(p.block), 0, st, nbr, values, grad_out,
-                              filter, m, grad_values, partial, row_partition);
+                    LN_LAUNCH("k_conv_backward_fused", (k_conv_backward_fused_b3_rows<T, LN_CONV_OVL_C, false>), dim3(p.grid), dim3(p.block), 0, st, nbr, values, grad_out,
+                              filter, m, grad_values, partial, row_partition, (const int*)nullptr, 0);
                     return;
                 }
             }
-            LN_LAUNCH("k_conv_backward_fused", (k_conv_backward_fused_b3<T>), dim3(p.grid), dim3(p.block), 0, st, nbr, values, grad_out, filter, m,
-                      grad_values, partial, row_partition);
+            LN_LAUNCH("k_conv_backward_fused", (k_conv_backward_fused_b3<T, false>), dim3(p.grid), dim3(p.block), 0, st, nbr, values, grad_out, filter, m,
+                      grad_values, partial, row_partition, (const int*)nullptr, 0);
             return;
         }
     }
@@ -2430,9 +2518,10 @@
     return ln_conv_backward_query(mq, mn, filter_extent, val_dim, nr_filters, ln_conv_b3_enabled());
 }
 
-extern "C" int ln_conv_backward_flags(const int* nbr_q, const int* nbr_n, const float* values_neigh, const float* grad_out, const float* filter,
-                                      int mq, int mn, int filter_extent, int val_dim, int nr_filters, int flags, float* grad_values,
-                                      float* grad_filter, void* workspace, size_t workspace_bytes, const int* row_partition, void* stream) {
+extern "C" int ln_conv_backward_rows(const int* nbr_q, const int* nbr_n, const float* values_neigh, const float* grad_out, const float* filter,
+                                     int mq, int mn, int filter_extent, int val_dim, int nr_filters, int flags, float* grad_values,
+                                     float* grad_filter, void* workspace, size_t workspace_bytes, const int* row_partition,
+                                     const int* rows_device, void* stream) {
     hipStream_t st = (hipStream_t)stream;
     LN_REQUIRE((flags & ~LN_CONV_OVERLAPPED) == 0, LN_ERR_ARG, "ln_conv_backward: unknown flags %d", flags);
     const LnBwdPlan p = ln_conv_backward_plan(LnBwdPlanIn{
@@ -2442,13 +2531,20 @@
     float* partial = static_cast<float*>(workspace);
     const int total = filter_extent * val_dim * nr_filters;
     if (p.form == LN_BWD_FUSED_B3 || p.form == LN_BWD_FUSED_F32) {
+        const int* rows_dev = (p.form == LN_BWD_FUSED_B3 && ln_aligned16(grad_values) && ln_aligned16(partial)) ? rows_device : nullptr;
+        const bool count_slabs = rows_dev && !row_partition && total % 64 == 0 && ln_aligned16(grad_filter);
+        const int zero_slab = count_slabs ? 0 : 1;
         switch (p.t) {
-            case 1: ln_bwd_launch_fused<1>(p, nbr_n, values_neigh, grad_out, filter, mn, grad_values, partial, row_partition, st); break;
-            case 2: ln_bwd_launch_fused<2>(p, nbr_n, values_neigh, grad_out, filter, mn, grad_values, partial, row_partition, st); break;
-            case 3: ln_bwd_launch_fused<3>(p, nbr_n, values_neigh, grad_out, filter, mn, grad_values, partial, row_partition, st); break;
-            default: ln_bwd_launch_fused<4>(p, nbr_n, values_neigh, grad_out, filter, mn, grad_values, partial, row_partition, st); break;
-        }
-        (void)ln_reduce_slabs_async(partial, p.grid, total, grad_filter, st);
+            case 1: ln_bwd_launch_fused<1>(p, nbr_n, values_neigh, grad_out, filter, mn, grad_values, partial, row_partition, st, rows_dev, zero_slab); break;
+            case 2: ln_bwd_launch_fused<2>(p, nbr_n, values_neigh, grad_out, filter, mn, grad_values, partial, row_partition, st, rows_dev, zero_slab); break;
+            case 3: ln_bwd_launch_fused<3>(p, nbr_n, values_neigh, grad_out, filter, mn, grad_values, partial, row_partition, st, rows_dev, zero_slab); break;
+            default: ln_bwd_launch_fused<4>(p, nbr_n, values_neigh, grad_out, filter, mn, grad_values, partial, row_partition, st, rows_dev, zero_slab); break;
+        }
+        if (count_slabs)
+            LN_LAUNCH("k_reduce_slabs", k_reduce_slabs4_live, dim3(total / 64), dim3(256), 0, st, (const float*)partial, p.grid, total, grad_filter, rows_dev, mn,
+                      64 * p.t * p.c);
+        else
+            (void)ln_reduce_slabs_async(partial, p.grid, total, grad_filter, st);
         return ln_check_launch("ln_conv_backward");
     }
     if (p.form == LN_BWD_FULL_SUM) {
@@ -2467,6 +2563,13 @@
     rc = ln_conv_forward_riding(nbr_n, grad_out, filter, mn, filter_extent, nr_filters, val_dim, LN_CONV_FLIP_NEIGHBOURS | LN_CONV_TRANSPOSED_FILTER,
                                 grad_values, conv_ws, conv_ws ? workspace_bytes - gf_bytes : 0, row_partition, stream, sum);
     return rc ? rc : ln_check_launch("ln_conv_backward");
+}
+
+extern "C" int ln_conv_backward_flags(const int* nbr_q, const int* nbr_n, const float* values_neigh, const float* grad_out, const float* filter,
+                                      int mq, int mn, int filter_extent, int val_dim, int nr_filters, int flags, float* grad_values,
+                                      float* grad_filter, void* workspace, size_t workspace_bytes, const int* row_partition, void* stream) {
+    return ln_conv_backward_rows(nbr_q, nbr_n, values_neigh, grad_out, filter, mq, mn, filter_extent, val_dim, nr_filters, flags, grad_values,
+                                 grad_filter, workspace, workspace_bytes, row_partition, nullptr, stream);
 }
 
 extern "C" int ln_conv_backward(const int* nbr_q, const int* nbr_n, const float* values_neigh, const float* grad_out, const float* filter, int mq,
diff --git a/lattice_net_amd/csrc/ln_conv_plan.h b/lattice_net_amd/csrc/ln_conv_plan.h
--- a/lattice_net_amd/csrc/ln_conv_plan.h
+++ b/lattice_net_amd/csrc/ln_conv_plan.h
@@ -84,6 +84,14 @@
 static_assert(LN_CONV_OVL_T * LN_CONV_OVL_C >= LN_BWD_B3_MAX_T, "the narrow form would write more slabs than the workspace queries report");
 constexpr int ln_bwd_workgroups(int m, bool b3_enabled, bool overlapped = false) {
     return ln_cdiv(m, 64 * ln_bwd_subtiles(m, b3_enabled, overlapped) * ln_bwd_chunks(m, b3_enabled, overlapped));
+}
+constexpr int ln_live_slabs(int live, int rows_per_slab, int nslabs) {
+    return ln_cdiv(live, rows_per_slab) < nslabs ? ln_cdiv(live, rows_per_slab) : nslabs;
+}
+constexpr int ln_bwd_slabs_summed(int live, int m, bool b3_enabled, bool overlapped, bool partitioned) {
+    const int nslabs = ln_bwd_workgroups(m, b3_enabled, overlapped);
+    const int clamped = live < 0 ? 0 : (live > m ? m : live);
+    return partitioned ? nslabs : ln_live_slabs(clamped, 64 * ln_bwd_subtiles(m, b3_enabled, overlapped) * ln_bwd_chunks(m, b3_enabled, overlapped), nslabs);
 }
 
 constexpr size_t ln_conv_bank_bytes(int m, int E, int V, int F, bool b3_enabled) {
diff --git a/lattice_net_amd/lattice.py b/lattice_net_amd/lattice.py
--- a/lattice_net_amd/lattice.py
+++ b/lattice_net_amd/lattice.py
@@ -1108,9 +1108,9 @@
                     ws, flags = hit[1], flags | _lib.LN_CONV_BANK_READY
             if ws is None and wsb > 256:
                 ws = torch.empty((wsb,), dtype=torch.uint8, device=self._dev())
-            _lib.check(lib.ln_conv_forward_ws(_lib.ptr(nbr), _lib.ptr(vals), _lib.ptr(filter_bank), m, filter_extent, v, nr_filters, flags,
-                                              _lib.ptr(out), _lib.ptr(ws), 0 if ws is None else ws.numel(), self._row_partition(),
-                                              self._stream()), "ln_conv_forward")
+            _lib.check(lib.ln_conv_forward_ws_rows(_lib.ptr(nbr), _lib.ptr(vals), _lib.ptr(filter_bank), m, filter_extent, v, nr_filters, flags,
+                                                   _lib.ptr(out), _lib.ptr(ws), 0 if ws is None else ws.numel(), self._row_partition(),
+                                                   _lib.ptr(self.rows_device()), self._stream()), "ln_conv_forward")
             if key is not None and not (flags & _lib.LN_CONV_BANK_READY):
                 try:
                     _BANK_ENTRIES[filter_bank] = (key, ws)
@@ -1156,10 +1156,13 @@
             _lib.check(lib.ln_conv_forward_f16(_lib.ptr(nbr_n), _lib.ptr(grad_out), _lib.ptr(filter_bank), mn, E, f, v, flags, _lib.ptr(gvals),
                                                main), "ln_conv_forward_f16")
             return gvals, (gf if filter_grad_fp32 else gf.to(torch.float16))
-        part = nb._row_partition() if q.m_hash_table._storage is nb.m_hash_table._storage else None
+        same = q.m_hash_table._storage is nb.m_hash_table._storage
+        part = nb._row_partition() if same else None
+        rows_dev = nb.rows_device() if same else None
         flags = _lib.LN_CONV_OVERLAPPED if _SCANS_IN_FLIGHT[0] > 1 else 0
-        _lib.check(lib.ln_conv_backward_flags(_lib.ptr(nbr_q), _lib.ptr(nbr_n), _lib.ptr(nb.values()), _lib.ptr(grad_out), _lib.ptr(filter_bank),
-                                              mq, mn, E, v, f, flags, _lib.ptr(gvals), _lib.ptr(gf), _lib.ptr(ws), ws.numel(), part, main),
+        _lib.check(lib.ln_conv_backward_rows(_lib.ptr(nbr_q), _lib.ptr(nbr_n), _lib.ptr(nb.values()), _lib.ptr(grad_out), _lib.ptr(filter_bank),
+                                             mq, mn, E, v, f, flags, _lib.ptr(gvals), _lib.ptr(gf), _lib.ptr(ws), ws.numel(), part,
+                                             _lib.ptr(rows_dev), main),
                    "ln_conv_backward")
         return gvals, gf
 
```

Result: no change. 1506 (median of 2 runs) (+0.0%).
